# xxayt/MGSV

Hardware: AMD Instinct MI355X
Metric: video-music pairs/s fwd+bwd at B=64 (full training step); sub-objects: retrieval sim-matrix GB/s, eval forward pairs/s (higher is better)
Workload: dtype bf16; 1 GPU; BASELINE.json configs[2]: B=64/GPU, T_v=30, T_a=512, D=512, train mode (dropout on), f32 master weights + Adam, f32 gradient accumulation; global_batch=64, launch=tape

## Files before the change

include/made_hip.h:

```cpp
#ifndef MADE_HIP_H
#define MADE_HIP_H

#include <stdint.h>

#ifdef __cplusplus
extern "C" {
#endif

#define MADE_ABI_VERSION 8

enum MadeDtype { MADE_F32 = 0, MADE_BF16 = 1 };

enum MadeAct {
    MADE_ACT_NONE = 0,
    MADE_ACT_RELU = 1,
    MADE_ACT_GELU = 2,
    MADE_ACT_QUICKGELU = 3,
    MADE_ACT_SIGMOID = 4
};

enum MadeGate {
    MADE_GATE_NONE = 0,
    MADE_GATE_RELU_OUT = 1,
    MADE_GATE_GELU_Z = 2,
// ... 147 lines not shown

int made_splitk_finish(const MadeFinishArgs* args, void* stream);

typedef struct MadeAttnArgs {
    const void* Q; const void* K; const void* V; void* O;
    int32_t dtype; int32_t hd;
    int64_t B, H, Lq, Lk;
    int64_t q_bs, ldq, k_bs, ldk, v_bs, ldv, o_bs, ldo;
    const float* key_mask; const float* q_mask;
    float scale; int32_t _pad;
    const float* q_skip_mask;
    float*      lse;
    MadeDropout drop;
    const int32_t* batch_order;
    uint32_t* keep_bits;
    int64_t ld_bits;
} MadeAttnArgs;

int made_attention(const MadeAttnArgs* args, void* stream);

typedef struct MadeWideAttnArgs {
    const void* Q; const void* K; const void* Kadd; const void* V; void* O;
    const float* key_mask;
    int32_t dtype; int32_t o_dtype;
    int64_t B, NQ1, NQ2, L, D;
    int64_t q_bs, q_s1, q_s2, k_bs, ldk, kadd_bs, ldkadd, v_bs, ldv, o_bs, o_s1, o_s2;
    float scale; int32_t _pad;
    int64_t n_split;
    float*  part_o;
    float*  part_ml;
    MadeDropout drop;
    float*  sum_out;
    float*  lse_out;
} MadeWideAttnArgs;

int made_attention_wide(const MadeWideAttnArgs* args, void* stream);

typedef struct MadeWideAttnBwdArgs {
    const void *Q, *dO, *O, *K, *V;
    const float* key_mask;
    const float *lse, *ssum;
    const float* extra;
    const void* dattc; int64_t ld_dattc; const float* vbias; int64_t hd;
    void *Pd, *dS; int64_t p_bs, ld_p;
    void* dQ; int64_t dq_bs, ld_dq;
    int64_t B, NQ, L, D;
    int64_t q_bs, ld_q, do_bs, ld_do, o_bs, ld_o, k_bs, ldk, v_bs, ldv;
    float scale; int32_t _pad;
    int64_t n_split; float* part_dq;
    MadeDropout drop;
} MadeWideAttnBwdArgs;
int made_attention_wide_bwd(const MadeWideAttnBwdArgs* args, void* stream);

int made_tape_begin(void);
int made_tape_end(uint64_t* handle);
int made_tape_replay(uint64_t handle);
int made_tape_free(uint64_t handle);
int made_tape_interleave(uint64_t handle, int32_t main_weight);
int made_tape_count(uint64_t handle, int64_t* kernels, int64_t* waits, int64_t* others);
int made_tape_replay_range(uint64_t handle, int64_t first, int64_t count);
int made_tape_op(uint64_t handle, int64_t index, int32_t* kind, uint64_t* function, uint64_t* stream, uint32_t* grid3);
int made_stream_wait(void* src_stream, void* dst_stream);
typedef int (*MadeTapeCallback)(void* user);
int made_tape_callback(MadeTapeCallback fn, void* user);
int made_tape_event(int32_t op_kind, int32_t slot, void* stream);
int made_memset_async(void* dst, int32_t value, int64_t nbytes, void* stream);
int made_copy_async(void* dst, const void* src, int64_t nbytes, void* stream);
int made_store_words(void* dst, const uint32_t* words, int32_t n_words, void* stream);


int made_layernorm(const void* x, int32_t x_dtype, int64_t ldx, int64_t x_rows_per_batch, int64_t x_batch_stride,
                   const float* gamma, const float* beta,
                   void* y, int32_t y_dtype, int64_t ldy, int64_t rows, int64_t D, float eps,
                   const float* row_skip , void* stream);

int made_layernorm_add(const void* x, int32_t x_dtype, int64_t ldx, const float* gamma, const float* beta,
                       void* y, int32_t y_dtype, int64_t ldy, const void* add, int32_t add_dtype, int64_t ld_add,
                       void* y2, int64_t ldy2, int64_t rows, int64_t D, float eps, const float* row_skip, void* stream);

int made_pack_music_records(const void* seg, int32_t seg_dtype, int64_t seg_bs, const float* mask, int64_t ld_mask, const float* music, int64_t ld_music,
                            void* out, int32_t pack_dtype, int64_t rec_bytes, int64_t n, int64_t n_pad, int64_t S, int64_t D, void* stream);

int made_cast_mask_rows(const float* x, int64_t ldx, const float* mask, void* y, int32_t y_dtype, int64_t ldy,
                        int64_t rows, int64_t D, void* stream);

int made_masked_mean(const void* x, int32_t x_dtype, int64_t x_bs, int64_t ldx, const float* mask,
                     float* out, int64_t B, int64_t T, int64_t D, void* stream);

int made_l2norm_rows(const void* x, int32_t x_dtype, int64_t ldx, float* y_f32, void* y_alt, int32_t y_alt_dtype,
                     int64_t ldy, int64_t rows, int64_t D, float eps, void* stream);

int made_sine_pe(const float* mask, const float* dim_t, void* out, int32_t out_dtype,
                 int64_t B, int64_t L, int64_t D, void* stream);

int made_masked_softmax(const float* logits, int64_t ld_logits, const float* mask, int64_t ld_mask,
                        void* probs, int32_t out_dtype, int64_t ldp,
                        int64_t M_outer, int64_t R, int64_t S, int64_t S_pad, float scale, void* stream);

typedef struct MadeXpoolFusedArgs {
    const void* Q; int64_t ldq;
    const void* K; const void* U; int64_t k_bs, ldk, u_bs, ldu;
    const float* key_mask;
    const float* ln2_g; const float* ln2_b;
    const void* Wl; int64_t ldw; const float* bl;
    const float* ln3_g; const float* ln3_b;
    const float* vn; int64_t ldvn;
// ... 300 lines not shown
```

mgsv_amd/_lib.py:

```python
from __future__ import annotations

import ctypes as C
import os

_HERE = os.path.dirname(os.path.abspath(__file__))


def variant_env(name: str, default: str = "") -> str:
    if os.environ.get("MADE_DEBUG_VARIANTS", "0") in ("", "0"):
        return default
    return os.environ.get(name, default)


LIB_PATH = os.environ.get("MADE_LIB_PATH") or os.path.join(_HERE, "libmade_hip.so")
ABI_VERSION = 8

F32, BF16 = 0, 1
ACT_NONE, ACT_RELU, ACT_GELU, ACT_QUICKGELU, ACT_SIGMOID = 0, 1, 2, 3, 4
GATE_NONE, GATE_RELU_OUT, GATE_GELU_Z, GATE_QUICKGELU_Z, GATE_SIGMOID_OUT = 0, 1, 2, 3, 4

vp, i64, i32, f32 = C.c_void_p, C.c_int64, C.c_int32, C.c_float


class MadeDropout(C.Structure):
    _fields_ = [("seed", C.c_uint64), ("site", C.c_uint32), ("p", f32), ("seed_device", vp)]


class MadeLinearSeg(C.Structure):
    _fields_ = [("col_begin", i64), ("out", vp), ("out_dtype", i32), ("transposed", i32), ("ldo", i64),
                ("rows_per_batch", i64), ("out_batch_stride", i64), ("out_z_stride", i64),
                ("use_a2", i32), ("_pad", i32)]


class MadeLinearArgs(C.Structure):
    _fields_ = [("A", vp), ("a_dtype", i32), ("w_dtype", i32), ("lda", i64),
                ("A2", vp), ("lda2", i64), ("a2_row_mod", i64),
                ("a2_replace", i32), ("drop_col_div", i32),
                ("a_row_mask", vp),
                ("W", vp), ("ldw", i64),
                ("bias", vp),
                ("M", i64), ("N", i64), ("K", i64),
                ("batch", i64), ("a_z_stride", i64), ("w_z_stride", i64),
                ("act", i32), ("r_dtype", i32),
                ("R", vp), ("ldr", i64), ("r_row_mod", i64),
                ("out_row_mask", vp),
                ("tile_skip_mask", vp),
                ("nseg", i32), ("split_k", i32),
                ("split_ws", vp),
                ("seg", MadeLinearSeg * 4),
                ("G", vp), ("g_dtype", i32), ("gate", i32), ("ldg", i64), ("gate_scale", f32), ("z_dtype", i32),
                ("Zout", vp), ("ldz", i64), ("drop", MadeDropout), ("drop_ld", i64), ("row_index", vp), ("n_rows", vp),
                ("bias_row_scale", vp), ("bias_z_stride", i64)]


class MadeFinishArgs(C.Structure):
    _fields_ = [("ws", vp), ("split_k", i64), ("M", i64), ("N", i64),
                ("bias", vp), ("act", i32), ("r_dtype", i32),
                ("R", vp), ("ldr", i64), ("r_row_mod", i64),
                ("out", vp), ("out_dtype", i32), ("_pad0", i32), ("ldo", i64),
                ("ln1_g", vp), ("ln1_b", vp), ("ln1_out", vp), ("ln1_dtype", i32), ("_pad1", i32), ("ln1_ld", i64),
                ("ln2_g", vp), ("ln2_b", vp), ("ln2_out", vp), ("ln2_dtype", i32), ("_pad2", i32), ("ln2_ld", i64),
                ("eps", f32), ("_pad3", i32)]


class MadeDecStageArgs(C.Structure):
    _fields_ = [("Zin", vp), ("ldz", i64), ("ln_g", vp), ("ln_b", vp),
                ("ln2_g", vp), ("ln2_b", vp), ("x2_out", vp), ("ldx2", i64),
                ("add", vp), ("add_row_mod", i64), ("x_out", vp), ("ldx", i64),
                ("W", vp), ("ldw", i64), ("bias", vp), ("R", vp), ("ldr", i64), ("out", vp), ("ldo", i64),
                ("out_dtype", i32), ("act", i32), ("res_from_x", i32), ("eps", f32),
                ("M", i64), ("N", i64), ("K", i64),
                ("zin_dtype", i32), ("drop_col_div", i32), ("a_out", vp), ("lda_out", i64), ("drop", MadeDropout), ("drop_ld", i64)]


# ... 95 lines not shown

class MadeAdamGroup(C.Structure):
    _fields_ = [("begin", i64), ("end", i64), ("lr", f32), ("max_norm", f32)]


class MadeAdamDeviceState(C.Structure):
    _fields_ = [("step", i64), ("lr", f32 * 4), ("bc1", f32), ("bc2_sqrt", f32)]


class MadeRepackDesc(C.Structure):
    _fields_ = [("src", vp), ("w", vp), ("wt", vp), ("rows", i64), ("cols", i64), ("wt_ld", i64), ("tile_begin", i64),
                ("dtype", i32), ("_pad", i32)]


class MadeFrameDesc(C.Structure):
    _fields_ = [("offset", i64), ("coef", i64), ("H", i32), ("W", i32), ("kh", i32), ("kv", i32)]


class MadeResampleDesc(C.Structure):
    _fields_ = [("offset", i64), ("n", i64), ("taps", i64), ("o", i32), ("m", i32), ("width", i32), ("_pad", i32)]


class MadeAudioSegDesc(C.Structure):
    _fields_ = [("first", i64), ("count", i64)]


SIGNATURES = {
    "made_abi_version": (C.c_int, []),
    "made_set_f32_products": (C.c_int, [C.c_int]),
    "made_get_f32_products": (C.c_int, []),
    "made_last_error": (C.c_char_p, []),
    "made_device_info": (C.c_int, [C.c_char_p, C.c_int, C.POINTER(C.c_int), C.POINTER(C.c_int)]),
    "made_tape_begin": (C.c_int, []),
    "made_tape_end": (C.c_int, [C.POINTER(C.c_uint64)]),
    "made_tape_replay": (C.c_int, [C.c_uint64]),
    "made_tape_free": (C.c_int, [C.c_uint64]),
    "made_tape_interleave": (C.c_int, [C.c_uint64, i32]),
    "made_tape_count": (C.c_int, [C.c_uint64, C.POINTER(i64), C.POINTER(i64), C.POINTER(i64)]),
    "made_tape_replay_range": (C.c_int, [C.c_uint64, i64, i64]),
    "made_tape_op": (C.c_int, [C.c_uint64, i64, C.POINTER(i32), C.POINTER(C.c_uint64), C.POINTER(C.c_uint64), C.POINTER(C.c_uint32)]),
    "made_stream_wait": (C.c_int, [vp, vp]),
    "made_tape_event": (C.c_int, [i32, i32, vp]),
    "made_tape_callback": (C.c_int, [C.CFUNCTYPE(C.c_int, vp), vp]),
    "made_memset_async": (C.c_int, [vp, i32, i64, vp]),
    "made_copy_async": (C.c_int, [vp, vp, i64, vp]),
    "made_store_words": (C.c_int, [vp, vp, i32, vp]),
    "made_linear": (C.c_int, [C.POINTER(MadeLinearArgs), vp]),
    "made_splitk_finish": (C.c_int, [C.POINTER(MadeFinishArgs), vp]),
    "made_dec_stage": (C.c_int, [C.POINTER(MadeDecStageArgs), vp]),
    "made_dec_stage_bwd": (C.c_int, [C.POINTER(MadeDecStageBwdArgs), vp]),
    "made_attention": (C.c_int, [C.POINTER(MadeAttnArgs), vp]),
    "made_attention_wide": (C.c_int, [C.POINTER(MadeWideAttnArgs), vp]),
    "made_attention_wide_bwd": (C.c_int, [C.POINTER(MadeWideAttnBwdArgs), vp]),
    "made_layernorm": (C.c_int, [vp, i32, i64, i64, i64, vp, vp, vp, i32, i64, i64, i64, f32, vp, vp]),
    "made_layernorm_add": (C.c_int, [vp, i32, i64, vp, vp, vp, i32, i64, vp, i32, i64, vp, i64, i64, i64, f32, vp, vp]),
    "made_cast_mask_rows": (C.c_int, [vp, i64, vp, vp, i32, i64, i64, i64, vp]),
    "made_pack_music_records": (C.c_int, [vp, i32, i64, vp, i64, vp, i64, vp, i32, i64, i64, i64, i64, i64, vp]),
    "made_masked_mean": (C.c_int, [vp, i32, i64, i64, vp, vp, i64, i64, i64, vp]),
    "made_l2norm_rows": (C.c_int, [vp, i32, i64, vp, vp, i32, i64, i64, i64, f32, vp]),
    "made_sine_pe": (C.c_int, [vp, vp, vp, i32, i64, i64, i64, vp]),
    "made_masked_softmax": (C.c_int, [vp, i64, vp, i64, vp, i32, i64, i64, i64, i64, i64, f32, vp]),
    "made_xpool_tail": (C.c_int, [vp, i32, i64, vp, vp, vp, i64, vp, vp, i64, i64, i64, i64, f32, vp]),
    "made_clip_loss": (C.c_int, [vp, i64, i64, vp, f32, i32, vp, vp, vp]),
    "made_hungarian_match": (C.c_int, [vp, vp, vp, i64, i64, i64, i64, i32, f32, f32, f32, vp, i32, vp, vp, vp, vp, vp]),
    "made_attention_bwd": (C.c_int, [C.POINTER(MadeAttnBwdArgs), vp]),
    "made_layernorm_bwd": (C.c_int, [vp, i32, i64, i64, i64, vp, vp, i32, i64, vp, i32, i64, vp, i32, i64, vp, i64,
                                     C.POINTER(MadeDropout), i64, vp, vp, i64, i64, f32, vp, vp]),
    "made_layernorm_bwd2": (C.c_int, [vp, vp, i64, vp, vp, i64, vp, i64, vp, i64, vp, i64, vp, i64, C.POINTER(MadeDropout), i64, i32,
                                      vp, vp, vp, vp, i64, i64, f32, vp]),
    "made_pool_bwd": (C.c_int, [vp, vp, vp, vp, i32, i64, i64, vp, i32, i64, i64, vp, i32, i64, i64, i64, i64, i64, f32, vp]),
    "made_l2norm_bwd": (C.c_int, [vp, i32, i64, vp, i64, i64, vp, i64, i32, vp, i32, i64, i64, i64, f32, vp]),
    "made_clip_loss_bwd": (C.c_int, [vp, i64, i64, vp, f32, vp, vp, vp, vp, i32, vp, vp, vp]),
    "made_xpool_tail_bwd": (C.c_int, [vp, i32, i64, vp, vp, vp, i64, vp, i64, vp, i32, i64, vp, C.POINTER(MadeDropout),
                                      vp, vp, vp, i64, vp, i64, f32, i64, i64, i64, f32, vp]),
    "made_softmax_bwd": (C.c_int, [vp, i64, vp, i64, vp, i64, vp, f32, C.POINTER(MadeDropout), vp, vp, vp, i32, i64, i64,
                                   i64, i64, i64, i64, i64, vp]),
    "made_head_bias": (C.c_int, [vp, i32, i64, vp, vp, i64, i64, i64, vp]),
    "made_head_bias_bwd": (C.c_int, [vp, i32, i64, vp, vp, vp, vp, i64, i64, i64, vp]),
    "made_add3": (C.c_int, [vp, i32, vp, i32, vp, i32, vp, i32, i64, i64, vp]),
    "made_colsum": (C.c_int, [vp, i32, i64, i64, i64, vp, vp]),
    "made_posbn_relu_fwd": (C.c_int, [vp, i32, i64, vp, vp, vp, vp, C.c_float, C.c_float, i32, vp, vp, vp, i32, i64, i64, i64, i64, vp]),
    "made_posbn_relu_bwd": (C.c_int, [vp, i32, i64, vp, i32, i64, vp, i32, i64, vp, vp, vp, i32, vp, i32, i64, vp, vp, i64, i64, i64, vp]),
    "made_set_criterion_bwd": (C.c_int, [vp, vp, vp, vp, vp, vp, vp, vp, vp, i64, i64, i64, i64, i64, i32, f32, vp, vp,
                                         vp, vp, i64, i32, vp, vp, vp]),
    "made_adam_step": (C.c_int, [vp, vp, vp, vp, i64, C.POINTER(MadeAdamGroup), i32, f32, f32, f32, i64, f32, vp, vp]),
    "made_adam_step_device": (C.c_int, [vp, vp, vp, vp, i64, C.POINTER(MadeAdamGroup), i32, f32, f32, f32, vp, i32, f32, vp, vp]),
    "made_repack": (C.c_int, [vp, i32, i64, vp]),
    "made_row_groups": (C.c_int, [vp, i64, vp, vp]),
    "made_row_index": (C.c_int, [vp, i64, vp, vp, vp]),
    "made_linear_variant": (C.c_int, [C.POINTER(MadeLinearArgs)]),
    "made_row_affine": (C.c_int, [vp, i32, i64, vp, vp, i64, i32, vp, i32, i64, i64, i64, vp]),
    "made_gate_rows": (C.c_int, [vp, i32, i64, vp, i32, i64, i32, f32, vp, i64, i64, vp, i32, i64, vp, i64, i64, vp]),
    "made_xpool_fused": (C.c_int, [C.POINTER(MadeXpoolFusedArgs), vp]),
    "made_xpool_attention": (C.c_int, [C.POINTER(MadeXpoolAttnArgs), vp]),
    "made_xpool_sims": (C.c_int, [C.POINTER(MadeXpoolSimsArgs), vp]),
    "made_xpool_sims_ws_bytes": (C.c_int64, [i64, i64, i64]),
    "made_xpool_inbatch": (C.c_int, [C.POINTER(MadeXpoolInbatchArgs), vp]),
    "made_xpool_inbatch_ws_bytes": (C.c_int64, [i64, i64]),
    "made_batch_order": (C.c_int, [vp, i64, i64, vp, vp]),
    "made_recall_ranks": (C.c_int, [vp, i64, vp, vp, i64, i64, i64, vp, vp, vp]),
    "made_span_iou": (C.c_int, [vp, vp, vp, vp, i64, i64, i32, f32, vp, vp, vp]),
    "made_gemm_tn": (C.c_int, [C.POINTER(MadeGemmTNArgs), vp]),
    "made_gemm_tn_grouped": (C.c_int, [C.POINTER(MadeGemmTNGroup), vp]),
    "made_gemm_tn_grouped_workspace": (i64, [C.POINTER(MadeGemmTNGroup)]),
    "made_concat_cols": (C.c_int, [vp, i64, vp, i64, vp, i64, vp]),
    "made_pooled_cosine": (C.c_int, [vp, i64, vp, i32, vp, i64, i64, i64, i64, i64, vp]),
# ... 53 lines not shown
```

mgsv_amd/csrc/attention_wide.hip:

```cpp
#include "common.h"

#include <type_traits>

namespace {

constexpr int WQ = 32;
constexpr int WKEY = 32;
constexpr int NTHREADS = 256;

template <typename TC> struct Frag;
template <> struct Frag<float>  { typedef f32x4  type; };
template <> struct Frag<bf16_t> { typedef bf16x8 type; };


template <typename TC, int D, bool DB, int NSL, bool X3 = false>
__global__ __launch_bounds__(NTHREADS) void attention_wide_kernel(const MadeWideAttnArgs a) {
    typedef typename Frag<TC>::type frag_t;
    constexpr int SZ = (int)sizeof(TC);
    constexpr bool IS_BF16 = SZ == 2;
    constexpr int PER16 = 16 / SZ;
    constexpr int DS = D / NSL;
    constexpr int WQB = WQ * (4 / NSL);
    constexpr bool DMA = IS_BF16 && DB;
    constexpr int K_ROW = DMA ? D * SZ : D * SZ + 16;
    constexpr int V_ROW = DMA ? D * SZ : D * SZ + (IS_BF16 ? 64 : 16);
    constexpr int CPR = D * SZ / 16;
    constexpr int NCH = WKEY * CPR / NTHREADS;
    static_assert(WKEY * CPR % NTHREADS == 0, "staging split");
    constexpr int NQF = DS * SZ / 32;
    constexpr int NDT = DS / 32;
    constexpr int KV_STAGE = WKEY * K_ROW + WKEY * V_ROW;
    constexpr int NSTAGE = DB ? 2 : 1;

    extern __shared__ __attribute__((aligned(16))) unsigned char lds[];
    float* lds_s = (float*)(lds + NSTAGE * KV_STAGE);
    float* lds_bias_all = lds_s + 4 * 1024;
    uint32_t* lds_mbits = (uint32_t*)(lds_bias_all + NSTAGE * 32);

    const int tid = threadIdx.x, lane = tid & 63, wave = tid >> 6;
    const int r = lane & 31, hh = lane >> 5;
    const int sl = wave % NSL, qt = wave / NSL;
    const bool batch_fast = gridDim.x == (unsigned)a.B && (a.NQ1 * a.NQ2 + WQB - 1) / WQB != (int64_t)a.B;
    const int64_t b = batch_fast ? blockIdx.x : blockIdx.y;
    const int64_t nq_total = a.NQ1 * a.NQ2;
    const int64_t nq0 = (int64_t)(batch_fast ? blockIdx.y : blockIdx.x) * WQB + qt * WQ;

    const TC* Kg = (const TC*)a.K + b * a.k_bs;
    const TC* Ag = a.Kadd ? (const TC*)a.Kadd + b * a.kadd_bs : nullptr;
    const TC* Vg = (const TC*)a.V + b * a.v_bs;
    const float* maskg = a.key_mask ? a.key_mask + b * a.L : nullptr;

    frag_t qf[NQF];
    int64_t my_q = nq0 + r;
    {
        int64_t q = my_q < nq_total ? my_q : nq_total - 1;
        const TC* qp = (const TC*)a.Q + b * a.q_bs + (q / a.NQ2) * a.q_s1 + (q % a.NQ2) * a.q_s2 + sl * DS;
#pragma unroll
        for (int ks = 0; ks < NQF; ++ks) qf[ks] = *(const frag_t*)(qp + ks * 2 * PER16 + hh * PER16);
    }

    frag_t rk[NCH], rv[NCH];
    int64_t rkey0 = 0;
    auto load_tile = [&](int64_t key0) __attribute__((always_inline)) {
        rkey0 = key0;
#pragma unroll
        for (int i = 0; i < NCH; ++i) {
            int c = tid + i * NTHREADS;
            int row = c / CPR, cc = c % CPR;
            int64_t key = key0 + row;
            const int64_t kcl = key < a.L ? key : a.L - 1;
            rk[i] = *(const frag_t*)(Kg + kcl * a.ldk + cc * PER16);
            rv[i] = *(const frag_t*)(Vg + kcl * a.ldv + cc * PER16);
        }
        if (Ag) {
#pragma unroll
            for (int i = 0; i < NCH; ++i) {
                int c = tid + i * NTHREADS;
                int64_t key = key0 + c / CPR;
                const int64_t kcl = key < a.L ? key : a.L - 1;
                const frag_t av = *(const frag_t*)(Ag + kcl * a.ldkadd + (c % CPR) * PER16);
#pragma unroll
                for (int j = 0; j < PER16; ++j) rk[i][j] = from_f32<TC>(to_f32(rk[i][j]) + to_f32(av[j]));
            }
        }
    };
    auto store_tile = [&](int stage) __attribute__((always_inline)) {
        unsigned char* sk = lds + stage * KV_STAGE;
        unsigned char* sv = sk + WKEY * K_ROW;
        const uint32_t bits = lds_mbits[rkey0 / WKEY];
#pragma unroll
        for (int i = 0; i < NCH; ++i) {
            int c = tid + i * NTHREADS;
            const bool keep = (bits >> (c / CPR)) & 1u;
            *(frag_t*)(sk + (c / CPR) * K_ROW + (c % CPR) * 16) = keep_or_zero(rk[i], keep);
            *(frag_t*)(sv + (c / CPR) * V_ROW + (c % CPR) * 16) = keep_or_zero(rv[i], keep);
        }
        if (tid < WKEY) lds_bias_all[stage * WKEY + tid] = ((bits >> tid) & 1u) ? 0.f : -INFINITY;
    };

    f32x16 o[NDT];
#pragma unroll
    for (int d = 0; d < NDT; ++d)
#pragma unroll
        for (int e = 0; e < 16; ++e) o[d][e] = 0.f;
    float m_run = -INFINITY, l_run = 0.f;
    float sd_run = 0.f;
    const uint32_t drop_thr = made_drop_threshold(a.drop.p);
    const uint64_t drop_seed = a.drop.p > 0.f ? made_drop_seed(a.drop) : 0;
    const float drop_sc = a.drop.p > 0.f ? 1.f / (1.f - a.drop.p) : 1.f;
    const uint64_t drop_base = (uint64_t)(b * nq_total + (my_q < nq_total ? my_q : nq_total - 1)) * (uint64_t)a.L;
    const bool drop_fast = (uint32_t)drop_base <= 0xFFFFFFFFu - (uint32_t)(a.L + 64);
    const uint32_t drop_key = made_rng_key(drop_seed, a.drop.site, (uint32_t)(drop_base >> 32));
    const uint32_t drop_lo = (uint32_t)drop_base;

    int64_t l_eff = a.L;
    int first_valid = 0;
    {
        const int lpad = (int)((a.L + 63) / 64) * 64;
        int last = -1, first = 0x7fffffff;
        for (int j = tid; j < lpad; j += NTHREADS) {
            const bool valid = j < (int)a.L && (maskg == nullptr || maskg[j] != 0.f);
            const unsigned long long bal = __ballot(valid);
            if (lane == 0) { lds_mbits[j / 32] = (uint32_t)bal; lds_mbits[j / 32 + 1] = (uint32_t)(bal >> 32); }
            if (valid) { last = j; first = min(first, j); }
        }
        if (tid == 0) lds_mbits[lpad / 32] = 0u;
        if (maskg) {
#pragma unroll
            for (int o2 = 32; o2 > 0; o2 >>= 1) { last = max(last, __shfl_xor(last, o2)); first = min(first, __shfl_xor(first, o2)); }
            int* red = (int*)lds_s;
            if (lane == 0) { red[wave] = last; red[4 + wave] = first; }
            __syncthreads();
            l_eff = max(max(red[0], red[1]), max(red[2], red[3])) + 1;
            first_valid = min(min(red[4], red[5]), min(red[6], red[7]));
            if (first_valid == 0x7fffffff) first_valid = 0;
        }
        __syncthreads();
    }
    const int64_t nsplit = a.n_split > 1 ? a.n_split : 1;
    const int64_t tiles_all = (l_eff + WKEY - 1) / WKEY;
    const int64_t tiles_per = (tiles_all + nsplit - 1) / nsplit;
    const int64_t tile0 = (int64_t)blockIdx.z * tiles_per;
    const int64_t ntiles = tile0 >= tiles_all ? 0 : (tile0 + tiles_per <= tiles_all ? tiles_per : tiles_all - tile0);
    typedef __attribute__((address_space(3))) void* lds_ptr_t;
    typedef const __attribute__((address_space(1))) void* glb_ptr_t;
    auto issue_tile = [&](int64_t key0, int stage) __attribute__((always_inline)) {
        constexpr int ROWS_PER_PIECE = DMA ? 1024 / (D * SZ) : 1;
        constexpr int NPIECE = WKEY / ROWS_PER_PIECE;
        constexpr int CPRW = D * SZ / 16;
        const uint32_t bits = lds_mbits[key0 / WKEY];
        unsigned char* st = lds + stage * KV_STAGE;
        const unsigned char* Kb = (const unsigned char*)Kg;
        const unsigned char* Vb = (const unsigned char*)Vg;
        const uint32_t ldk_b = (uint32_t)a.ldk * SZ, ldv_b = (uint32_t)a.ldv * SZ;
#pragma unroll
        for (int i = 0; i < NPIECE / 4; ++i) {
            const int jp = wave + 4 * i;
            const int row = ROWS_PER_PIECE == 1 ? jp : 2 * jp + (lane >> 5);
            const uint32_t cl = ROWS_PER_PIECE == 1 ? (uint32_t)lane : (uint32_t)(lane & 31);
            const uint32_t srow = ((bits >> row) & 1u) ? (uint32_t)(key0 + row) : (uint32_t)first_valid;
            const uint32_t ck = cl ^ ((uint32_t)(row & 31) & (uint32_t)(CPRW - 1));
            const uint32_t cu = ((((cl >> 2) ^ (uint32_t)(row & 7)) << 2) | (cl & 3));
            __builtin_amdgcn_global_load_lds((glb_ptr_t)(Kb + (size_t)(srow * ldk_b + ck * 16u)), (lds_ptr_t)(st + jp * 1024), 16, 0, 0);
            __builtin_amdgcn_global_load_lds((glb_ptr_t)(Vb + (size_t)(srow * ldv_b + cu * 16u)), (lds_ptr_t)(st + WKEY * K_ROW + jp * 1024), 16, 0, 0);
        }
    };
    if constexpr (DMA) {
        __builtin_amdgcn_s_waitcnt(0x0070);
        if (ntiles > 0) issue_tile(tile0 * WKEY, 0);
    } else if (NSTAGE == 2 && ntiles > 0) {
        load_tile(tile0 * WKEY);
        store_tile(0);
        __syncthreads();
    }
    for (int64_t tt = 0; tt < ntiles; ++tt) {
        const int64_t t = tile0 + tt;
        const int cur = NSTAGE == 2 ? (int)(tt & 1) : 0;
        uint32_t tbits = 0xffffffffu;
        if constexpr (DMA) {
            asm volatile("s_waitcnt vmcnt(0) lgkmcnt(0)\n\ts_barrier" ::: "memory");
            tbits = lds_mbits[t];
        } else if (NSTAGE == 2) {
            if (tt + 1 < ntiles) load_tile((t + 1) * WKEY);
        } else {
            load_tile(t * WKEY);
            __syncthreads();
            store_tile(0);
            __syncthreads();
        }
        const unsigned char* lds_k = lds + cur * KV_STAGE;
        const unsigned char* lds_v = lds_k + WKEY * K_ROW;
        const float* lds_bias = lds_bias_all + cur * WKEY;

        f32x16 s;
#pragma unroll
        for (int e = 0; e < 16; ++e) s[e] = 0.f;
        if constexpr (X3) {
            static_assert(!X3 || (NQF % 2 == 0 && !DMA), "f32 slices of 16 columns or more");
#pragma unroll
            for (int ks = 0; ks < NQF; ks += 2) {
                const SplitF32x4 k0 = made_split4(*(const f32x4*)(lds_k + r * K_ROW + sl * DS * SZ + ks * 32 + hh * 16));
                const SplitF32x4 k1 = made_split4(*(const f32x4*)(lds_k + r * K_ROW + sl * DS * SZ + (ks + 1) * 32 + hh * 16));
                s = made_mfma_x3_16(k0, k1, made_split4(qf[ks]), made_split4(qf[ks + 1]), s);
            }
        } else {
#pragma unroll
        for (int ks = 0; ks < NQF; ++ks) {
            frag_t kf;
            if constexpr (DMA) kf = *(const frag_t*)(lds_k + r * K_ROW + ((((sl * DS * SZ) / 16 + ks * 2 + hh) ^ r) << 4));
            else kf = *(const frag_t*)(lds_k + r * K_ROW + sl * DS * SZ + ks * 32 + hh * 16);
            if constexpr (IS_BF16) {
                s = __builtin_amdgcn_mfma_f32_32x32x16_bf16(kf, qf[ks], s, 0, 0, 0);
            } else {
#pragma unroll
                for (int e = 0; e < 4; ++e) s = __builtin_amdgcn_mfma_f32_32x32x2f32(kf[e], qf[ks][e], s, 0, 0, 0);
            }
        }
        }
        if constexpr (DMA) {
            if (tt + 1 < ntiles) issue_tile((t + 1) * WKEY, cur ^ 1);
        }
#pragma unroll
        for (int e = 0; e < 16; ++e) lds_s[wave * 1024 + acc_row(e, hh) * 32 + r] = s[e];
        asm volatile("s_waitcnt lgkmcnt(0)\n\ts_barrier" ::: "memory");
        float mx = -INFINITY;
#pragma unroll
        for (int e = 0; e < 16; ++e) {
            const int idx = acc_row(e, hh) * 32 + r;
            float v;
            if constexpr (NSL == 4) v = (lds_s[idx] + lds_s[1024 + idx]) + (lds_s[2048 + idx] + lds_s[3072 + idx]);
            else v = lds_s[qt * 2048 + idx] + lds_s[qt * 2048 + 1024 + idx];
            if constexpr (DMA) v = ((tbits >> acc_row(e, hh)) & 1u) ? v * a.scale : -INFINITY;
            else v = v * a.scale + lds_bias[acc_row(e, hh)];
            s[e] = v;
// ... 54 lines not shown
                    for (int d = 0; d < NDT; ++d) {
                        asm volatile("" : "+v"(lo[d]), "+v"(hi[d]));
                        o[d] = __builtin_amdgcn_mfma_f32_32x32x16_bf16(__builtin_shufflevector(lo[d], hi[d], 0, 1, 2, 3, 4, 5, 6, 7), pf, o[d], 0, 0, 0);
                    }
                } else {
#pragma unroll
                for (int d = 0; d < NDT; ++d) {
                    const int dcol = sl * DS + d * 32 + (g & 1) * 16 + 4 * (i & 3);
                    const unsigned char* vp = lds_v + (kb + (i >> 2)) * V_ROW + dcol * 2;
                    bf16x4 lo = __builtin_amdgcn_ds_read_tr16_b64_v4bf16((__attribute__((address_space(3))) bf16x4*)vp);
                    bf16x4 hi = __builtin_amdgcn_ds_read_tr16_b64_v4bf16((__attribute__((address_space(3))) bf16x4*)(vp + 8 * V_ROW));
                    bf16x8 vf = __builtin_shufflevector(lo, hi, 0, 1, 2, 3, 4, 5, 6, 7);
                    o[d] = __builtin_amdgcn_mfma_f32_32x32x16_bf16(vf, pf, o[d], 0, 0, 0);
                }
                }
            }
        } else if constexpr (X3) {
#pragma unroll
            for (int g4 = 0; g4 < 4; g4 += 2) {
                const SplitF32x4 pb0 = made_split4(f32x4{s[4 * g4], s[4 * g4 + 1], s[4 * g4 + 2], s[4 * g4 + 3]});
                const SplitF32x4 pb1 = made_split4(f32x4{s[4 * g4 + 4], s[4 * g4 + 5], s[4 * g4 + 6], s[4 * g4 + 7]});
#pragma unroll
                for (int d = 0; d < NDT; ++d) {
                    f32x4 v0, v1;
#pragma unroll
                    for (int j = 0; j < 4; ++j) {
                        v0[j] = *(const float*)(lds_v + (8 * g4 + 4 * hh + j) * V_ROW + (sl * DS + d * 32 + r) * 4);
                        v1[j] = *(const float*)(lds_v + (8 * g4 + 8 + 4 * hh + j) * V_ROW + (sl * DS + d * 32 + r) * 4);
                    }
                    o[d] = made_mfma_x3_16(made_split4(v0), made_split4(v1), pb0, pb1, o[d]);
                }
            }
        } else {
#pragma unroll
            for (int e = 0; e < 16; ++e) {
                const int key = acc_row(e, hh);
#pragma unroll
                for (int d = 0; d < NDT; ++d) {
                    float vv = *(const float*)(lds_v + key * V_ROW + (sl * DS + d * 32 + r) * 4);
                    o[d] = __builtin_amdgcn_mfma_f32_32x32x2f32(vv, s[e], o[d], 0, 0, 0);
                }
            }
        }
        if (NSTAGE == 2 && !DMA) {
            if (tt + 1 < ntiles) store_tile(cur ^ 1);
            __syncthreads();
        }
    }

    const float l_tot = l_run + __shfl_xor(l_run, 32);
    const float inv = 1.f / l_tot;
    const float sd_tot = sd_run + __shfl_xor(sd_run, 32);
    const bool live_q = my_q < nq_total;
    if (nsplit == 1 && !live_q) return;
    if (nsplit == 1 && sl == 0 && hh == 0) {
        if (a.sum_out) a.sum_out[b * nq_total + my_q] = a.drop.p > 0.f ? sd_tot * inv : 1.f;
        if (a.lse_out) a.lse_out[b * nq_total + my_q] = m_run + logf(l_tot);
    }
    if (nsplit > 1) {
        const int64_t prow = (b * nsplit + blockIdx.z) * nq_total + (live_q ? my_q : 0);
        if (live_q) {
            float* po = a.part_o + prow * D + sl * DS;
#pragma unroll
            for (int d = 0; d < NDT; ++d)
#pragma unroll
                for (int g4 = 0; g4 < 4; ++g4) {
                    f32x4 pk; pk[0] = o[d][4 * g4]; pk[1] = o[d][4 * g4 + 1]; pk[2] = o[d][4 * g4 + 2]; pk[3] = o[d][4 * g4 + 3];
                    *(f32x4*)(po + d * 32 + 8 * g4 + 4 * hh) = pk;
                }
            if (sl == 0 && hh == 0) {
                a.part_ml[prow * 4] = m_run; a.part_ml[prow * 4 + 1] = l_tot; a.part_ml[prow * 4 + 2] = a.drop.p > 0.f ? sd_tot : l_tot;
            }
        }
        return;
    }
    const int64_t obase = b * a.o_bs + (my_q / a.NQ2) * a.o_s1 + (my_q % a.NQ2) * a.o_s2 + sl * DS;
#pragma unroll
    for (int d = 0; d < NDT; ++d)
#pragma unroll
        for (int g4 = 0; g4 < 4; ++g4) {
            const int64_t off = obase + d * 32 + 8 * g4 + 4 * hh;
            float v0 = o[d][4 * g4] * inv, v1 = o[d][4 * g4 + 1] * inv, v2 = o[d][4 * g4 + 2] * inv, v3 = o[d][4 * g4 + 3] * inv;
            if (a.o_dtype == MADE_F32) {
                f32x4 pk; pk[0] = v0; pk[1] = v1; pk[2] = v2; pk[3] = v3;
                *(f32x4*)((float*)a.O + off) = pk;
            } else {
                bf16x4 pk; pk[0] = (bf16_t)v0; pk[1] = (bf16_t)v1; pk[2] = (bf16_t)v2; pk[3] = (bf16_t)v3;
                *(bf16x4*)((bf16_t*)a.O + off) = pk;
            }
        }
}

__global__ __launch_bounds__(NTHREADS) void attention_wide_combine_kernel(const MadeWideAttnArgs a) {
    const int lane = threadIdx.x & 63;
    const int64_t nq_total = a.NQ1 * a.NQ2;
    const int64_t row = (int64_t)blockIdx.x * (NTHREADS / 64) + (threadIdx.x >> 6);
    if (row >= a.B * nq_total) return;
    const int64_t b = row / nq_total, q = row % nq_total;
    const int D = (int)a.D;
    const int ns = (int)a.n_split;
    float Lsum = 0.f, Dsum = 0.f, Muse = 0.f;
    f32x4 acc[2];
#pragma unroll
    for (int i = 0; i < 2; ++i) { acc[i][0] = acc[i][1] = acc[i][2] = acc[i][3] = 0.f; }
    if (ns <= 4) {
        f32x4 t[4][2];
        float ml[4][3];
#pragma unroll
        for (int sp = 0; sp < 4; ++sp) {
            const int64_t pr = (b * ns + (sp < ns ? sp : ns - 1)) * nq_total + q;
            ml[sp][0] = a.part_ml[pr * 4]; ml[sp][1] = a.part_ml[pr * 4 + 1]; ml[sp][2] = a.part_ml[pr * 4 + 2];
#pragma unroll
            for (int i = 0; i < 2; ++i) {
// ... 37 lines not shown
            }
        }
    }
    const float inv = 1.f / Lsum;
    if (a.sum_out && lane == 0) a.sum_out[b * nq_total + q] = Dsum * inv;
    if (a.lse_out && lane == 0) a.lse_out[b * nq_total + q] = Muse + logf(Lsum);
    const int64_t obase = b * a.o_bs + (q / a.NQ2) * a.o_s1 + (q % a.NQ2) * a.o_s2;
#pragma unroll
    for (int i = 0; i < 2; ++i) {
        int c = (i * 64 + lane) * 4;
        if (c < D) {
            if (a.o_dtype == MADE_F32) {
                f32x4 pk; pk[0] = acc[i][0] * inv; pk[1] = acc[i][1] * inv; pk[2] = acc[i][2] * inv; pk[3] = acc[i][3] * inv;
                *(f32x4*)((float*)a.O + obase + c) = pk;
            } else {
                bf16x4 pk; pk[0] = (bf16_t)(acc[i][0] * inv); pk[1] = (bf16_t)(acc[i][1] * inv);
                pk[2] = (bf16_t)(acc[i][2] * inv); pk[3] = (bf16_t)(acc[i][3] * inv);
                *(bf16x4*)((bf16_t*)a.O + obase + c) = pk;
            }
        }
    }
}

template <typename TC, int D, bool DB, int NSL>
int launch_wide(const MadeWideAttnArgs& a, hipStream_t st) {
    constexpr int SZ = (int)sizeof(TC);
    constexpr bool DMA = SZ == 2 && DB;
    constexpr int K_ROW = DMA ? D * SZ : D * SZ + 16, V_ROW = DMA ? D * SZ : D * SZ + (SZ == 2 ? 64 : 16);
    constexpr int NSTAGE = DB ? 2 : 1;
    constexpr size_t kBase = (size_t)NSTAGE * (WKEY * K_ROW + WKEY * V_ROW) + 4 * 1024 * 4 + NSTAGE * 32 * 4;
    constexpr size_t kCap = kBase + 8192 < 160 * 1024 ? kBase + 8192 : 160 * 1024;
    const size_t lds_bytes = kBase + (size_t)((a.L + 63) / 64 * 2 + 2) * 4;
    if (lds_bytes > kCap) {
        made_set_error("made_attention_wide: L=%lld keys: the mask bit row does not fit in LDS beside the K / V stages", (long long)a.L);
        return MADE_ERR_UNSUPPORTED;
    }
    static bool attr_done = false;
    if (!attr_done) {
        hipError_t e = hipFuncSetAttribute((const void*)attention_wide_kernel<TC, D, DB, NSL>, hipFuncAttributeMaxDynamicSharedMemorySize, (int)kCap);
        if (e == hipSuccess && SZ == 4)
            e = hipFuncSetAttribute((const void*)attention_wide_kernel<TC, D, DB, NSL, SZ == 4>, hipFuncAttributeMaxDynamicSharedMemorySize, (int)kCap);
        if (e != hipSuccess) {
            made_set_error("made_attention_wide: cannot reserve %zu bytes of LDS: %s", kCap, hipGetErrorString(e));
            return MADE_ERR_HIP;
        }
        attr_done = true;
    }
    const int64_t nq = a.NQ1 * a.NQ2;
    const int64_t nsplit = a.n_split > 1 ? a.n_split : 1;
    constexpr int WQB = WQ * (4 / NSL);
    const int64_t qtiles = (nq + WQB - 1) / WQB;
    const bool batch_fast = qtiles > 1 && qtiles <= 8 && qtiles != a.B;
    dim3 grid((unsigned)(batch_fast ? a.B : qtiles), (unsigned)(batch_fast ? qtiles : a.B), (unsigned)nsplit), block(NTHREADS);
    if (SZ == 4 && g_made_f32_products) hipLaunchKernelGGL((attention_wide_kernel<TC, D, DB, NSL, SZ == 4>), grid, block, lds_bytes, st, a);
    else hipLaunchKernelGGL((attention_wide_kernel<TC, D, DB, NSL>), grid, block, lds_bytes, st, a);
    int rc = made_check_launch("made_attention_wide");
    if (rc != MADE_OK || nsplit == 1) return rc;
    const int64_t rows = a.B * nq;
    hipLaunchKernelGGL(attention_wide_combine_kernel, dim3((unsigned)((rows + 3) / 4)), dim3(NTHREADS), 0, st, a);
    return made_check_launch("made_attention_wide(combine)");
}

}

extern "C" int made_attention_wide(const MadeWideAttnArgs* args, void* stream) {
    MADE_REQUIRE(args != nullptr, "made_attention_wide: null args");
    const MadeWideAttnArgs& a = *args;
    MADE_REQUIRE(a.Q && a.K && a.V && a.O, "made_attention_wide: null tensor");
    MADE_REQUIRE(a.B >= 0 && a.NQ1 >= 0 && a.NQ2 > 0 && a.L > 0, "made_attention_wide: bad dims");
    MADE_REQUIRE(a.dtype == MADE_F32 || a.dtype == MADE_BF16, "made_attention_wide: bad dtype %d", a.dtype);
    MADE_REQUIRE(a.o_dtype == MADE_F32 || a.o_dtype == MADE_BF16, "made_attention_wide: bad o_dtype %d", a.o_dtype);
    MADE_UNSUPPORTED(a.D == 128 || a.D == 256 || a.D == 512, "made_attention_wide: D=%lld not in {128, 256, 512}", (long long)a.D);
    MADE_UNSUPPORTED(a.B <= 65535, "made_attention_wide: B too large for the grid");
    const int per16 = a.dtype == MADE_F32 ? 4 : 8;
    MADE_UNSUPPORTED(a.q_bs % per16 == 0 && a.q_s1 % per16 == 0 && a.q_s2 % per16 == 0 && a.k_bs % per16 == 0 && a.ldk % per16 == 0 &&
                     a.v_bs % per16 == 0 && a.ldv % per16 == 0 && a.kadd_bs % per16 == 0 && a.ldkadd % per16 == 0 &&
                     a.o_bs % 4 == 0 && a.o_s1 % 4 == 0 && a.o_s2 % 4 == 0,
                     "made_attention_wide: strides must keep 16-byte alignment");
    MADE_UNSUPPORTED(((uintptr_t)a.Q % 16) == 0 && ((uintptr_t)a.K % 16) == 0 && ((uintptr_t)a.V % 16) == 0 && ((uintptr_t)a.O % 16) == 0 &&
                     ((uintptr_t)a.Kadd % 16) == 0, "made_attention_wide: base pointers must be 16-byte aligned");
    MADE_REQUIRE(a.drop.p >= 0.f && a.drop.p < 1.f, "made_attention_wide: dropout p out of [0,1)");
    if (a.n_split > 1) {
        MADE_REQUIRE(a.part_o != nullptr && a.part_ml != nullptr, "made_attention_wide: n_split > 1 needs part_o / part_ml");
        MADE_UNSUPPORTED(a.n_split <= 64, "made_attention_wide: n_split <= 64");
    }
    if (a.B == 0 || a.NQ1 == 0) return MADE_OK;
    hipStream_t st = (hipStream_t)stream;
    if (a.dtype == MADE_BF16) {
        const int64_t nq = a.NQ1 * a.NQ2;
        const bool few = nq <= 64 && a.Kadd == nullptr;
        const bool pair = nq > 32 && nq <= 64 && a.Kadd == nullptr;
        if (a.D == 128) return launch_wide<bf16_t, 128, false, 4>(a, st);
        if (a.D == 512) {
            if (pair) return launch_wide<bf16_t, 512, true, 2>(a, st);
            return few ? launch_wide<bf16_t, 512, true, 4>(a, st) : launch_wide<bf16_t, 512, false, 4>(a, st);
        }
        if (pair) return launch_wide<bf16_t, 256, true, 2>(a, st);
        return few ? launch_wide<bf16_t, 256, true, 4>(a, st) : launch_wide<bf16_t, 256, false, 4>(a, st);
    }
    if (a.D == 128) return launch_wide<float, 128, false, 4>(a, st);
    return a.D == 512 ? launch_wide<float, 512, false, 4>(a, st) : launch_wide<float, 256, false, 4>(a, st);
}
```

mgsv_amd/csrc/attention_wide_bwd.hip:

```cpp
#include "common.h"

namespace {

constexpr int BK = 32;
constexpr int NT = 256;
constexpr int MAXQ = 8;

typedef __attribute__((address_space(3))) void* lds_ptr_t;
typedef const __attribute__((address_space(1))) void* glb_ptr_t;

template <int D>
__global__ __launch_bounds__(NT) void attention_wide_bwd_kernel(const MadeWideAttnBwdArgs a) {
    constexpr int DS = D / 4;
    constexpr int NQF = DS / 16;
    constexpr int NDT = DS / 32;
    constexpr int ROWB = D * 2;
    constexpr int CPR = ROWB / 16;
    constexpr int STAGE = 2 * BK * ROWB;
    extern __shared__ __attribute__((aligned(16))) unsigned char lds[];
    float* lds_x = (float*)(lds + 2 * STAGE);
    float* lds_q = lds_x + 4 * 2 * BK * MAXQ;
    uint32_t* lds_mbits = (uint32_t*)(lds_q + 8 + 4 * MAXQ);

    const int tid = threadIdx.x, lane = tid & 63, wave = __builtin_amdgcn_readfirstlane(tid >> 6);
    const int r = lane & 31, hh = lane >> 5;
    const int sl = wave;
    const int64_t b = blockIdx.y;
    const int NQ = (int)a.NQ;
    const int rq = (r & 7) < NQ ? (r & 7) : NQ - 1;
    const bool live = r < NQ;

    const bf16_t* Kg = (const bf16_t*)a.K + b * a.k_bs;
    const bf16_t* Vg = (const bf16_t*)a.V + b * a.v_bs;
    const float* maskg = a.key_mask ? a.key_mask + b * a.L : nullptr;

    bf16x8 qf[NQF], dof[NQF];
    float dpart = 0.f;
    {
        const bf16_t* qp = (const bf16_t*)a.Q + b * a.q_bs + (int64_t)rq * a.ld_q + sl * DS + hh * 8;
        const bf16_t* gp = (const bf16_t*)a.dO + b * a.do_bs + (int64_t)rq * a.ld_do + sl * DS + hh * 8;
        const bf16_t* op = (const bf16_t*)a.O + b * a.o_bs + (int64_t)rq * a.ld_o + sl * DS + hh * 8;
        bf16x8 of[NQF];
#pragma unroll
        for (int ks = 0; ks < NQF; ++ks) { qf[ks] = *(const bf16x8*)(qp + ks * 16); dof[ks] = *(const bf16x8*)(gp + ks * 16); of[ks] = *(const bf16x8*)(op + ks * 16); }
#pragma unroll
        for (int ks = 0; ks < NQF; ++ks)
#pragma unroll
            for (int j = 0; j < 8; ++j) dpart += (float)dof[ks][j] * (float)of[ks][j];
    }
    dpart += __shfl_xor(dpart, 32);
    if (r < MAXQ && hh == 0) lds_q[8 + wave * MAXQ + r] = dpart;
    const float lse = a.lse[b * NQ + rq];
    const float ssum = a.ssum ? a.ssum[b * NQ + rq] : 1.f;
    if (wave == 0) {
        float ex = 0.f;
        if (a.extra) {
            ex = a.extra[b * NQ + ((lane >> 3) < NQ ? (lane >> 3) : NQ - 1)];
        } else if (a.dattc) {
            const int h = lane >> 3, per = (int)a.hd / 8;
            const bf16_t* dp_ = (const bf16_t*)a.dattc + b * a.ld_dattc + h * a.hd + (lane & 7) * per;
            const float* bp = a.vbias + h * a.hd + (lane & 7) * per;
            if (h < NQ)
                for (int e = 0; e < per; ++e) ex += (float)dp_[e] * bp[e];
            ex += __shfl_xor(ex, 1); ex += __shfl_xor(ex, 2); ex += __shfl_xor(ex, 4);
        }
        if ((lane & 7) == 0) lds_q[lane >> 3] = ex;
    }

    int64_t l_eff = a.L;
    int first_valid = 0;
    {
        const int lpad = (int)((a.L + 63) / 64) * 64;
        int last = -1, first = 0x7fffffff;
        for (int j = tid; j < lpad; j += NT) {
            const bool valid = j < (int)a.L && (maskg == nullptr || maskg[j] != 0.f);
            const unsigned long long bal = __ballot(valid);
            if (lane == 0) { lds_mbits[j / 32] = (uint32_t)bal; lds_mbits[j / 32 + 1] = (uint32_t)(bal >> 32); }
            if (valid) { last = j; first = min(first, j); }
        }
        if (tid == 0) lds_mbits[lpad / 32] = 0u;
#pragma unroll
        for (int o2 = 32; o2 > 0; o2 >>= 1) { last = max(last, __shfl_xor(last, o2)); first = min(first, __shfl_xor(first, o2)); }
        int* red = (int*)lds_x;
        if (lane == 0) { red[wave] = last; red[4 + wave] = first; }
        __syncthreads();
        l_eff = max(max(red[0], red[1]), max(red[2], red[3])) + 1;
        first_valid = min(min(red[4], red[5]), min(red[6], red[7]));
        if (first_valid == 0x7fffffff) first_valid = 0;
        __syncthreads();
    }
    const float extra = lds_q[rq];
    const float delta = ((lds_q[8 + rq] + lds_q[8 + MAXQ + rq]) + (lds_q[8 + 2 * MAXQ + rq] + lds_q[8 + 3 * MAXQ + rq])) + extra * ssum;

    const int64_t nsplit = a.n_split > 1 ? a.n_split : 1;
    const int64_t tiles_all = (l_eff + BK - 1) / BK;
    const int64_t tiles_L = (a.L + BK - 1) / BK;
    const int64_t tiles_per = (tiles_all + nsplit - 1) / nsplit;
    const int64_t tile0 = (int64_t)blockIdx.z * tiles_per;
    const int64_t ntiles = tile0 >= tiles_all ? 0 : (tile0 + tiles_per <= tiles_all ? tiles_per : tiles_all - tile0);

    auto issue_tile = [&](int64_t key0, int stage) __attribute__((always_inline)) {
        constexpr int ROWS_PER_PIECE = 1024 / ROWB;
        constexpr int NPIECE = BK / ROWS_PER_PIECE;
        const uint32_t bits = lds_mbits[key0 / BK];
        unsigned char* st = lds + stage * STAGE;
        const unsigned char* Kb = (const unsigned char*)Kg;
        const unsigned char* Vb = (const unsigned char*)Vg;
        const uint32_t ldk_b = (uint32_t)a.ldk * 2, ldv_b = (uint32_t)a.ldv * 2;
#pragma unroll
        for (int i = 0; i < NPIECE / 4; ++i) {
            const int jp = wave + 4 * i;
            const int row = ROWS_PER_PIECE == 1 ? jp : 2 * jp + (lane >> 5);
            const uint32_t cl = ROWS_PER_PIECE == 1 ? (uint32_t)lane : (uint32_t)(lane & 31);
            const uint32_t srow = ((bits >> row) & 1u) ? (uint32_t)(key0 + row) : (uint32_t)first_valid;
            const uint32_t c_row = cl ^ ((uint32_t)(row & 31) & (uint32_t)(CPR - 1));
            const uint32_t c_tr = ((((cl >> 2) ^ (uint32_t)(row & 7)) << 2) | (cl & 3));
            __builtin_amdgcn_global_load_lds((glb_ptr_t)(Kb + (size_t)(srow * ldk_b + c_tr * 16u)), (lds_ptr_t)(st + jp * 1024), 16, 0, 0);
            __builtin_amdgcn_global_load_lds((glb_ptr_t)(Vb + (size_t)(srow * ldv_b + c_row * 16u)), (lds_ptr_t)(st + BK * ROWB + jp * 1024), 16, 0, 0);
        }
    };

    f32x16 o[NDT];
#pragma unroll
    for (int d = 0; d < NDT; ++d)
#pragma unroll
        for (int e = 0; e < 16; ++e) o[d][e] = 0.f;
    const uint32_t drop_thr = made_drop_threshold(a.drop.p);
    const uint64_t drop_seed = a.drop.p > 0.f ? made_drop_seed(a.drop) : 0;
    const float drop_sc = a.drop.p > 0.f ? 1.f / (1.f - a.drop.p) : 1.f;
    const uint64_t drop_base = (uint64_t)(b * NQ + rq) * (uint64_t)a.L;
    const bool drop_fast = (uint32_t)drop_base <= 0xFFFFFFFFu - (uint32_t)(a.L + 64);
    const uint32_t drop_key = made_rng_key(drop_seed, a.drop.site, (uint32_t)(drop_base >> 32));
    const uint32_t drop_lo = (uint32_t)drop_base;
    bf16_t* out_row = (wave == 0 ? (bf16_t*)a.Pd : (bf16_t*)a.dS) + b * a.p_bs + (int64_t)rq * a.ld_p;

    __builtin_amdgcn_s_waitcnt(0x0070);
    if (ntiles > 0) issue_tile(tile0 * BK, 0);
    for (int64_t tt = 0; tt < ntiles; ++tt) {
        const int64_t t = tile0 + tt;
        const int cur = (int)(tt & 1);
        asm volatile("s_waitcnt vmcnt(0) lgkmcnt(0)\n\ts_barrier" ::: "memory");
        const uint32_t tbits = lds_mbits[t];
        const unsigned char* lds_k = lds + cur * STAGE;
        const unsigned char* lds_v = lds_k + BK * ROWB;

        f32x16 s, dp;
#pragma unroll
        for (int e = 0; e < 16; ++e) { s[e] = 0.f; dp[e] = 0.f; }
#pragma unroll
        for (int ks = 0; ks < NQF; ++ks) {
            const int c = (sl * DS * 2) / 16 + ks * 2 + hh;
            const bf16x8 kf = *(const bf16x8*)(lds_k + r * ROWB + ((((c >> 2) ^ (r & 7)) << 6) | ((c & 3) << 4)));
            const bf16x8 vf = *(const bf16x8*)(lds_v + r * ROWB + (((c ^ r) & (CPR - 1)) << 4));
            s = __builtin_amdgcn_mfma_f32_32x32x16_bf16(kf, qf[ks], s, 0, 0, 0);
            dp = __builtin_amdgcn_mfma_f32_32x32x16_bf16(vf, dof[ks], dp, 0, 0, 0);
        }
        if (tt + 1 < ntiles) issue_tile((t + 1) * BK, cur ^ 1);
        if (r < MAXQ) {
#pragma unroll
            for (int e = 0; e < 16; ++e) {
                lds_x[((wave * 2 + 0) * BK + acc_row(e, hh)) * MAXQ + r] = s[e];
                lds_x[((wave * 2 + 1) * BK + acc_row(e, hh)) * MAXQ + r] = dp[e];
            }
        }
        asm volatile("s_waitcnt lgkmcnt(0)\n\ts_barrier" ::: "memory");
        float pd[16];
#pragma unroll
        for (int e = 0; e < 16; ++e) {
            const int kr = acc_row(e, hh);
            const float* xs = lds_x + kr * MAXQ + (r & 7);
            const float S = (xs[0] + xs[2 * BK * MAXQ]) + (xs[4 * BK * MAXQ] + xs[6 * BK * MAXQ]);
            const float dP = (xs[BK * MAXQ] + xs[3 * BK * MAXQ]) + (xs[5 * BK * MAXQ] + xs[7 * BK * MAXQ]);
            const bool valid = (tbits >> kr) & 1u;
            const float p = valid ? __expf(S * a.scale - lse) : 0.f;
            bool kp = true;
            if (a.drop.p > 0.f) {
                const uint32_t kidx = (uint32_t)(t * BK + kr);
                const uint32_t hsh = drop_fast ? made_rng_fmix32((drop_lo + kidx) ^ drop_key) : made_rng_mix(drop_seed, a.drop.site, drop_base + (uint64_t)kidx);
                kp = (hsh >> 8) >= drop_thr;
            }
            pd[e] = kp ? p * drop_sc : 0.f;
            const float dpd = valid ? dP + extra : 0.f;
            const float dpu = kp ? dpd * drop_sc : 0.f;
            s[e] = p * (dpu - delta) * a.scale;
        }
        if (wave < 2 && live) {
#pragma unroll
            for (int g4 = 0; g4 < 4; ++g4) {
                const int64_t key0 = t * BK + 8 * g4 + 4 * hh;
                if (key0 < a.ld_p) {
                    bf16x4 pk;
#pragma unroll
                    for (int j = 0; j < 4; ++j) pk[j] = (bf16_t)(wave == 0 ? pd[4 * g4 + j] : s[4 * g4 + j]);
                    *(bf16x4*)(out_row + key0) = pk;
                }
            }
        }
        {
            const int g = lane >> 4, i = lane & 15;
#pragma unroll
            for (int s2 = 0; s2 < 2; ++s2) {
                bf16x8 pf;
#pragma unroll
                for (int j = 0; j < 8; ++j) pf[j] = (bf16_t)s[8 * s2 + j];
                const int kb = 16 * s2 + 4 * (g >> 1);
                const int row = kb + (i >> 2);
                const uint32_t vb = (uint32_t)(uintptr_t)(__attribute__((address_space(3))) unsigned char*)lds_k + row * ROWB + (g & 1) * 32 + (i & 3) * 8;
                bf16x4 lo[NDT], hi[NDT];
#pragma unroll
                for (int d = 0; d < NDT; ++d) {
                    const uint32_t va = vb + ((((sl * DS) / 32 + d) ^ (row & 7)) << 6);
                    asm volatile("ds_read_b64_tr_b16 %0, %1" : "=v"(lo[d]) : "v"(va));
                    asm volatile("ds_read_b64_tr_b16 %0, %1 offset:%2" : "=v"(hi[d]) : "v"(va), "n"(8 * ROWB));
                }
#pragma unroll
                for (int d = 0; d < NDT; ++d) asm volatile("" : "+v"(lo[d]), "+v"(hi[d]));
                asm volatile("s_waitcnt lgkmcnt(0)" ::: "memory");
#pragma unroll
                for (int d = 0; d < NDT; ++d) {
                    asm volatile("" : "+v"(lo[d]), "+v"(hi[d]));
                    o[d] = __builtin_amdgcn_mfma_f32_32x32x16_bf16(__builtin_shufflevector(lo[d], hi[d], 0, 1, 2, 3, 4, 5, 6, 7), pf, o[d], 0, 0, 0);
                }
            }
        }
    }
    if (wave < 2 && live) {
        for (int64_t tz = tiles_all + blockIdx.z; tz < tiles_L; tz += nsplit) {
#pragma unroll
            for (int g4 = 0; g4 < 4; ++g4) {
                const int64_t key0 = tz * BK + 8 * g4 + 4 * hh;
                if (key0 < a.ld_p) {
                    bf16x4 z4; z4[0] = z4[1] = z4[2] = z4[3] = (bf16_t)0.f;
                    *(bf16x4*)(out_row + key0) = z4;
                }
            }
        }
    }

    if (nsplit == 1) {
        if (live) {
            bf16_t* dq = (bf16_t*)a.dQ + b * a.dq_bs + (int64_t)r * a.ld_dq + sl * DS;
#pragma unroll
            for (int d = 0; d < NDT; ++d)
#pragma unroll
                for (int g4 = 0; g4 < 4; ++g4) {
                    bf16x4 pk;
#pragma unroll
                    for (int j = 0; j < 4; ++j) pk[j] = (bf16_t)o[d][4 * g4 + j];
                    *(bf16x4*)(dq + d * 32 + 8 * g4 + 4 * hh) = pk;
                }
        }
        return;
    }
    if (live) {
        float* po = a.part_dq + ((b * nsplit + blockIdx.z) * NQ + r) * D + sl * DS;
#pragma unroll
        for (int d = 0; d < NDT; ++d)
#pragma unroll
            for (int g4 = 0; g4 < 4; ++g4) {
                f32x4 pk; pk[0] = o[d][4 * g4]; pk[1] = o[d][4 * g4 + 1]; pk[2] = o[d][4 * g4 + 2]; pk[3] = o[d][4 * g4 + 3];
                *(f32x4*)(po + d * 32 + 8 * g4 + 4 * hh) = pk;
            }
    }
}

__global__ __launch_bounds__(NT) void wide_bwd_merge_kernel(const MadeWideAttnBwdArgs a) {
    const int lane = threadIdx.x & 63;
    const int64_t row = (int64_t)blockIdx.x * 4 + (threadIdx.x >> 6);
    if (row >= a.B * a.NQ) return;
    const int64_t b = row / a.NQ, q = row % a.NQ;
    const int D = (int)a.D;
    const int per = D / 64;
    float acc[8];
#pragma unroll
    for (int j = 0; j < 8; ++j) acc[j] = 0.f;
    for (int64_t sp = 0; sp < a.n_split; ++sp) {
        const float* pp = a.part_dq + ((b * a.n_split + sp) * a.NQ + q) * D + lane * per;
        const f32x4 t0 = *(const f32x4*)pp;
        acc[0] += t0[0]; acc[1] += t0[1]; acc[2] += t0[2]; acc[3] += t0[3];
        if (per == 8) {
            const f32x4 t1 = *(const f32x4*)(pp + 4);
            acc[4] += t1[0]; acc[5] += t1[1]; acc[6] += t1[2]; acc[7] += t1[3];
        }
    }
    bf16_t* dq = (bf16_t*)a.dQ + b * a.dq_bs + q * a.ld_dq + lane * per;
    bf16x4 p0; p0[0] = (bf16_t)acc[0]; p0[1] = (bf16_t)acc[1]; p0[2] = (bf16_t)acc[2]; p0[3] = (bf16_t)acc[3];
    *(bf16x4*)dq = p0;
    if (per == 8) {
        bf16x4 p1; p1[0] = (bf16_t)acc[4]; p1[1] = (bf16_t)acc[5]; p1[2] = (bf16_t)acc[6]; p1[3] = (bf16_t)acc[7];
        *(bf16x4*)(dq + 4) = p1;
    }
}

template <int D>
int launch_wide_bwd(const MadeWideAttnBwdArgs& a, hipStream_t st) {
    constexpr size_t kBase = (size_t)2 * 2 * BK * D * 2 + (size_t)(4 * 2 * BK * MAXQ + 8 + 4 * MAXQ) * 4;
    const size_t lds_bytes = kBase + (size_t)((a.L + 63) / 64 * 2 + 2) * 4;
    if (lds_bytes > 160 * 1024) {
        made_set_error("made_attention_wide_bwd: L=%lld keys: the mask bit row does not fit in LDS beside the K / V stages", (long long)a.L);
        return MADE_ERR_UNSUPPORTED;
    }
    static bool attr_done = false;
    if (!attr_done) {
        hipError_t e = hipFuncSetAttribute((const void*)attention_wide_bwd_kernel<D>, hipFuncAttributeMaxDynamicSharedMemorySize, 160 * 1024);
        if (e != hipSuccess) {
            made_set_error("made_attention_wide_bwd: cannot reserve LDS: %s", hipGetErrorString(e));
            return MADE_ERR_HIP;
        }
        attr_done = true;
    }
    const int64_t nsplit = a.n_split > 1 ? a.n_split : 1;
    hipLaunchKernelGGL((attention_wide_bwd_kernel<D>), dim3(1, (unsigned)a.B, (unsigned)nsplit), dim3(NT), lds_bytes, st, a);
    int rc = made_check_launch("made_attention_wide_bwd");
    if (rc != MADE_OK || nsplit == 1) return rc;
    hipLaunchKernelGGL(wide_bwd_merge_kernel, dim3((unsigned)((a.B * a.NQ + 3) / 4)), dim3(NT), 0, st, a);
    return made_check_launch("made_attention_wide_bwd(merge)");
}

}

extern "C" int made_attention_wide_bwd(const MadeWideAttnBwdArgs* args, void* stream) {
    MADE_REQUIRE(args != nullptr, "made_attention_wide_bwd: null args");
    const MadeWideAttnBwdArgs& a = *args;
    MADE_REQUIRE(a.Q && a.dO && a.O && a.K && a.V && a.lse && a.Pd && a.dS && a.dQ, "made_attention_wide_bwd: null tensor");
    MADE_REQUIRE(a.B >= 0 && a.NQ > 0 && a.L > 0, "made_attention_wide_bwd: bad dims");
    MADE_UNSUPPORTED(a.NQ <= MAXQ, "made_attention_wide_bwd: NQ=%lld query rows per sample (at most %d: one moment query)", (long long)a.NQ, MAXQ);
    MADE_UNSUPPORTED(a.D == 256 || a.D == 512, "made_attention_wide_bwd: D=%lld not in {256, 512}", (long long)a.D);
    MADE_UNSUPPORTED(a.B <= 65535, "made_attention_wide_bwd: B too large for the grid");
    MADE_UNSUPPORTED(a.q_bs % 8 == 0 && a.ld_q % 8 == 0 && a.do_bs % 8 == 0 && a.ld_do % 8 == 0 && a.o_bs % 8 == 0 && a.ld_o % 8 == 0 &&
                     a.k_bs % 8 == 0 && a.ldk % 8 == 0 && a.v_bs % 8 == 0 && a.ldv % 8 == 0 && a.p_bs % 4 == 0 && a.ld_p % 4 == 0 &&
                     a.dq_bs % 4 == 0 && a.ld_dq % 4 == 0, "made_attention_wide_bwd: strides must keep the rows aligned (16 bytes in, 8 bytes out)");
    MADE_UNSUPPORTED(((uintptr_t)a.Q % 16) == 0 && ((uintptr_t)a.dO % 16) == 0 && ((uintptr_t)a.O % 16) == 0 && ((uintptr_t)a.K % 16) == 0 &&
                     ((uintptr_t)a.V % 16) == 0 && ((uintptr_t)a.Pd % 8) == 0 && ((uintptr_t)a.dS % 8) == 0 && ((uintptr_t)a.dQ % 8) == 0,
                     "made_attention_wide_bwd: base pointers must be aligned");
    MADE_REQUIRE(a.ld_p >= a.L, "made_attention_wide_bwd: ld_p < L");
    MADE_REQUIRE(a.drop.p >= 0.f && a.drop.p < 1.f, "made_attention_wide_bwd: dropout p out of [0,1)");
    if (a.dattc && !a.extra) {
        MADE_REQUIRE(a.vbias != nullptr && a.hd > 0 && a.hd % 8 == 0, "made_attention_wide_bwd: dattc needs vbias and hd (a multiple of 8)");
        MADE_UNSUPPORTED(a.hd * a.NQ == a.D, "made_attention_wide_bwd: dattc needs the one-query layout NQ * hd == D (NQ=%lld hd=%lld D=%lld); pass `extra` otherwise",
                         (long long)a.NQ, (long long)a.hd, (long long)a.D);
    }
    if (a.n_split > 1) {
        MADE_REQUIRE(a.part_dq != nullptr, "made_attention_wide_bwd: n_split > 1 needs part_dq");
        MADE_UNSUPPORTED(a.n_split <= 64, "made_attention_wide_bwd: n_split <= 64");
    }
    if (a.B == 0) return MADE_OK;
    hipStream_t st = (hipStream_t)stream;
    return a.D == 512 ? launch_wide_bwd<512>(a, st) : launch_wide_bwd<256>(a, st);
}
```

mgsv_amd/ops.py:

```python
from __future__ import annotations

import ctypes as C
import math
from dataclasses import dataclass
from typing import Optional, Sequence

import torch

from . import _lib, tape as _tape
from ._lib import (ACT_GELU, ACT_NONE, ACT_QUICKGELU, ACT_RELU, ACT_SIGMOID, BF16, F32,
                   MadeAttnArgs, MadeDecStageArgs, MadeFinishArgs, MadeLinearArgs, MadeLinearSeg, MadeWideAttnArgs, check, lib)

Tensor = torch.Tensor


def dt_of(t: Tensor) -> int:
    if t.dtype == torch.float32:
        return F32
    if t.dtype == torch.bfloat16:
        return BF16
    raise TypeError(f"unsupported dtype {t.dtype}")


def torch_dtype(code: int):
    return torch.float32 if code == F32 else torch.bfloat16


def _p(t: Optional[Tensor]):
    if t is None:
        return None
    if not t.is_cuda:
        raise _lib.MadeError("libmade_hip ops need GPU tensors (no CPU fallback)")
    if _tape._recording is not None:
        _tape._recording._keep.append(t)
    return t.data_ptr()


def _stream():
    return torch.cuda.current_stream().cuda_stream


def _f32(t: Optional[Tensor], name: str) -> Optional[Tensor]:
    if t is not None and (t.dtype != torch.float32 or not t.is_contiguous()):
        raise TypeError(f"{name} must be a contiguous float32 tensor")
    return t


def set_drop(d, drop) -> None:
    seed, site, p = drop
    if isinstance(seed, Tensor):
        assert seed.dtype == torch.int64 and seed.numel() == 1 and seed.is_cuda
        d.seed, d.seed_device = 0, seed.data_ptr()
    else:
        d.seed, d.seed_device = int(seed) & 0xFFFFFFFFFFFFFFFF, None
    d.site, d.p = int(site) & 0xFFFFFFFF, float(p)


def round_up(x: int, m: int) -> int:
# ... 283 lines not shown
    assert Q.dim() == 3 and K.dim() == 3 and V.dim() == 3 and O.dim() == 3
    assert Q.stride(2) == 1 and K.stride(2) == 1 and V.stride(2) == 1 and O.stride(2) == 1
    assert Q.dtype == K.dtype == V.dtype == O.dtype
    B, Lq, D = Q.shape
    hd = D // H
    a = MadeAttnArgs()
    a.Q, a.K, a.V, a.O = _p(Q), _p(K), _p(V), _p(O)
    a.dtype, a.hd = dt_of(Q), hd
    a.B, a.H, a.Lq, a.Lk = B, H, Lq, (K.shape[1] if Lk is None else Lk)
    a.q_bs, a.ldq = Q.stride(0), Q.stride(1)
    a.k_bs, a.ldk = K.stride(0), K.stride(1)
    a.v_bs, a.ldv = V.stride(0), V.stride(1)
    a.o_bs, a.ldo = O.stride(0), O.stride(1)
    a.key_mask = _p(_f32(key_mask, "key_mask"))
    a.q_mask = _p(_f32(q_mask, "q_mask"))
    a.q_skip_mask = _p(_f32(q_skip_mask, "q_skip_mask"))
    a.scale = (1.0 / math.sqrt(hd)) if scale is None else scale
    if order is not None:
        assert order.dtype == torch.int32 and order.numel() == B and order.is_contiguous()
        a.batch_order = _p(order)
    if lse is not None:
        assert lse.dtype == torch.float32 and lse.is_contiguous() and lse.numel() == B * H * Lq
        a.lse = _p(lse)
    if drop is not None and drop[2] > 0.0:
        set_drop(a.drop, drop)
        if keep_bits is not None:
            assert keep_bits.dtype == torch.int32 and keep_bits.dim() == 2 and keep_bits.is_contiguous()
            assert keep_bits.shape[0] >= B * H * ((a.Lk + 31) // 32) and keep_bits.shape[1] >= Lq
            a.keep_bits, a.ld_bits = _p(keep_bits), keep_bits.shape[1]
    esz = 4 if a.dtype == F32 else 2
    flops = 4.0 * B * H * Lq * a.Lk * hd
    nbytes = esz * B * D * (2 * Lq + 2 * a.Lk)
    _timed("attention_" + ("f32" if a.dtype == F32 else "bf16"), flops, nbytes,
           lambda: check(lib().made_attention(C.byref(a), _stream()), "made_attention"),
           ("attn", key_mask, q_skip_mask) if (key_mask is not None and key_mask.dim() == 2) else f"B={B} H={H} hd={hd} Lq={Lq} Lk={a.Lk}")
    return O


def attention_bits_shape(B: int, H: int, Lq: int, Lk: int):
    return (B * H * ((Lk + 31) // 32), 32 * ((Lq + 31) // 32))


def attention_bits_decode(bits: Tensor, B: int, H: int, Lq: int, Lk: int) -> Tensor:
    nkt, ldq = (Lk + 31) // 32, bits.shape[1]
    w = bits[:B * H * nkt].view(B, H, nkt, ldq)
    q = torch.arange(Lq, device=bits.device)
    ql = q & 31
    slot = (q & ~31) + 2 * ((ql & 3) + 4 * (ql >> 3)) + ((ql >> 2) & 1)
    w = w[:, :, :, slot]
    b = (w[..., None] >> torch.arange(32, device=bits.device, dtype=torch.int32)) & 1
    return b.permute(0, 1, 3, 2, 4).reshape(B, H, Lq, nkt * 32)[..., :Lk].bool()


def attention_wide(Q: Tensor, K: Tensor, V: Tensor, O: Tensor, *, scale: float, Kadd: Optional[Tensor] = None,
                   key_mask: Optional[Tensor] = None, shared_q: bool = False, n_split: int = 1,
                   part_o: Optional[Tensor] = None, part_ml: Optional[Tensor] = None, drop=None,
                   sum_out: Optional[Tensor] = None, lse_out: Optional[Tensor] = None) -> Tensor:
    assert Q.dim() == 4 and O.dim() == 4 and K.dim() == 3 and V.dim() == 3
    assert Q.stride(3) == 1 and O.stride(3) == 1 and K.stride(2) == 1 and V.stride(2) == 1
    assert Q.dtype == K.dtype == V.dtype
    B, L, D = K.shape
    a = MadeWideAttnArgs()
    a.Q, a.K, a.V, a.O = _p(Q), _p(K), _p(V), _p(O)
    a.key_mask = _p(_f32(key_mask, "key_mask"))
    a.dtype, a.o_dtype = dt_of(Q), dt_of(O)
    a.B, a.NQ1, a.NQ2, a.L, a.D = B, O.shape[1], O.shape[2], L, D
    a.q_bs, a.q_s1, a.q_s2 = (0 if shared_q else Q.stride(0)), Q.stride(1), Q.stride(2)
    a.k_bs, a.ldk = K.stride(0), K.stride(1)
    a.v_bs, a.ldv = V.stride(0), V.stride(1)
    if Kadd is not None:
        assert Kadd.dim() == 3 and Kadd.stride(2) == 1 and Kadd.dtype == K.dtype
        a.Kadd, a.kadd_bs, a.ldkadd = _p(Kadd), Kadd.stride(0), Kadd.stride(1)
    a.o_bs, a.o_s1, a.o_s2 = O.stride(0), O.stride(1), O.stride(2)
    a.scale = scale
    nq = a.NQ1 * a.NQ2
    if n_split > 1:
        if part_o is None:
            part_o = torch.empty(B * n_split * nq * D, device=Q.device, dtype=torch.float32)
            part_ml = torch.empty(B * n_split * nq * 4, device=Q.device, dtype=torch.float32)
        assert part_o.numel() >= B * n_split * nq * D and part_ml.numel() >= B * n_split * nq * 4
        a.n_split, a.part_o, a.part_ml = n_split, _p(_f32(part_o, "part_o")), _p(_f32(part_ml, "part_ml"))
    if drop is not None and drop[2] > 0.0:
        set_drop(a.drop, drop)
    if lse_out is not None:
        assert lse_out.dtype == torch.float32 and lse_out.is_contiguous() and lse_out.numel() >= B * nq
        a.lse_out = _p(lse_out)
    if sum_out is not None:
        assert sum_out.dtype == torch.float32 and sum_out.is_contiguous() and sum_out.numel() >= B * nq
        a.sum_out = _p(sum_out)
    esz = 4 if a.dtype == F32 else 2
    _timed("attention_wide_" + ("f32" if a.dtype == F32 else "bf16"), 4.0 * B * nq * L * D,
           esz * B * (2 * L * D + 2 * nq * D),
           lambda: check(lib().made_attention_wide(C.byref(a), _stream()), "made_attention_wide"),
           f"B={B} NQ={nq} L={L} D={D} kadd={int(Kadd is not None)}")
    return O


def layernorm(x: Tensor, gamma: Tensor, beta: Tensor, out: Optional[Tensor] = None, eps: float = 1e-5,
              out_dtype: Optional[torch.dtype] = None, row_skip: Optional[Tensor] = None) -> Tensor:
    assert x.dim() in (2, 3) and x.stride(-1) == 1
    if x.dim() == 3:
        rows, D = x.shape[0] * x.shape[1], x.shape[2]
        ldx, rpb, xbs = x.stride(1), x.shape[1], x.stride(0)
    else:
        rows, D = x.shape
        ldx, rpb, xbs = x.stride(0), 0, 0
    if out is None:
        out = torch.empty((rows, D), device=x.device, dtype=out_dtype or x.dtype)
    assert out.dim() == 2 and out.stride(1) == 1 and out.shape[0] >= rows
    check(lib().made_layernorm(_p(x), dt_of(x), ldx, rpb, xbs, _p(_f32(gamma, "gamma")), _p(_f32(beta, "beta")),
                               _p(out), dt_of(out), out.stride(0), rows, D, eps, _p(_f32(row_skip, "row_skip")), _stream()),
          "made_layernorm")
    return out


def layernorm_add(x: Tensor, gamma: Optional[Tensor], beta: Optional[Tensor], add: Tensor, out: Optional[Tensor], out2: Tensor,
                  eps: float = 1e-5, row_skip: Optional[Tensor] = None) -> Tensor:
    assert x.dim() == 2 and add.dim() == 2 and out2.dim() == 2 and x.stride(1) == 1 and add.stride(1) == 1 and out2.stride(1) == 1
    rows, D = x.shape
    ydt = dt_of(out2)
    if out is not None:
        assert out.dtype == out2.dtype and out.stride(1) == 1
    check(lib().made_layernorm_add(_p(x), dt_of(x), x.stride(0), _p(_f32(gamma, "gamma")), _p(_f32(beta, "beta")),
                                   _p(out), ydt, out.stride(0) if out is not None else 0, _p(add), dt_of(add), add.stride(0),
                                   _p(out2), out2.stride(0), rows, D, eps, _p(_f32(row_skip, "row_skip")), _stream()), "made_layernorm_add")
    return out2


def cast_mask_rows(x: Tensor, mask: Optional[Tensor], out: Tensor) -> Tensor:
    assert x.dim() == 2 and out.dim() == 2 and x.dtype == torch.float32 and x.stride(1) == 1 and out.stride(1) == 1
    check(lib().made_cast_mask_rows(_p(x), x.stride(0), _p(_f32(mask, "mask")), _p(out), dt_of(out), out.stride(0),
                                    x.shape[0], x.shape[1], _stream()), "made_cast_mask_rows")
    return out


def pack_music_records(seg: Tensor, mask: Tensor, music: Tensor, out: Tensor, pack_dtype: torch.dtype) -> Tensor:
    n, S, D = seg.shape
    assert seg.stride(2) == 1 and seg.stride(1) == D and out.dtype == torch.uint8 and out.dim() == 2 and out.is_contiguous() and out.shape[0] >= n
    mask, music = _f32(mask.contiguous(), "mask"), _f32(music.contiguous(), "music")
    check(lib().made_pack_music_records(_p(seg), dt_of(seg), seg.stride(0) if n > 0 else S * D, _p(mask), S, _p(music), D, _p(out),
                                        F32 if pack_dtype == torch.float32 else BF16, out.shape[1], n, out.shape[0], S, D, _stream()),
          "made_pack_music_records")
    return out


def row_affine(x: Tensor, scale: Tensor, shift: Tensor, act: int = ACT_NONE, out: Optional[Tensor] = None) -> Tensor:
    assert x.dim() == 2 and x.stride(1) == 1 and scale.numel() == shift.numel()
# ... 339 lines not shown
```

mgsv_amd/ops_train.py:

```python
from __future__ import annotations

import ctypes as C
from typing import Optional, Tuple

import torch

from . import _lib
from ._lib import BF16, F32, MadeAttnBwdArgs, MadeDropout, MadeGemmTNArgs, MadeGemmTNGroup, check, lib
from .ops import _f32, _p, _stream, _timed, dt_of, set_drop

Tensor = torch.Tensor
Pair = Tuple[int, int]


_TN_SLAB_US = 1.3


def _tn_splits(tiles: int, nslab: int, gathered: bool, cap: int) -> int:
    if _lib.variant_env("MADE_TN_SPLIT_MODEL", "1") == "0":
        sp = max(8, (512 // max(tiles, 1)) // 8 * 8) if cap == 64 and tiles < 64 else max(1, 2048 // max(tiles, 1))
        while (nslab + sp - 1) // sp > 64:
            sp += 8
        return min(sp, max(1, nslab))
    live = max(1, (nslab * 9) // 16 if gathered else nslab)
# ... 242 lines not shown
    B, T, D = out.shape
    def bs(t): return (t.stride(0), t.stride(1)) if t is not None else (0, 0)
    check(lib().made_pool_bwd(_p(_f32(mean, "mean")), _p(_f32(dvec, "dvec")), _p(_f32(mask, "mask")),
                              _p(in1), _dt(in1), *bs(in1), _p(in2), _dt(in2), *bs(in2),
                              _p(out), dt_of(out), *bs(out), B, T, D, eps, _stream()), "made_pool_bwd")
    return out


def l2norm_bwd(x: Tensor, dy: Tensor, dx: Optional[Tensor] = None, *, accumulate: bool = False, dx_alt: Optional[Tensor] = None,
               eps: float = 1e-12, dy_rows_per: int = 1) -> None:
    rows, D = x.shape
    check(lib().made_l2norm_bwd(_p(x), dt_of(x), x.stride(0), _p(_f32(dy, "dy")), dy.stride(0), dy_rows_per,
                                _p(dx), dx.stride(0) if dx is not None else 0, int(accumulate),
                                _p(dx_alt), _dt(dx_alt), dx_alt.stride(0) if dx_alt is not None else 0,
                                rows, D, eps, _stream()), "made_l2norm_bwd")


def clip_loss_bwd(sims: Tensor, logit_scale: Tensor, weight: float, upstream: Optional[Tensor], lse_ws: Tensor, dsims: Tensor,
                  dsims_t: Optional[Tensor], d_logit_scale: Optional[Tensor], accumulate: bool = False,
                  row_exclude: Optional[Tensor] = None) -> None:
    n = sims.shape[0]
    assert lse_ws.numel() >= 2 * n and dsims.is_contiguous()
    assert row_exclude is None or (row_exclude.shape == sims.shape and row_exclude.is_contiguous())
    check(lib().made_clip_loss_bwd(_p(_f32(sims, "sims")), sims.stride(0), n, _p(logit_scale), float(weight), _p(upstream),
                                   _p(lse_ws), _p(dsims), _p(dsims_t), int(accumulate), _p(d_logit_scale),
                                   _p(_f32(row_exclude, "row_exclude")), _stream()),
          "made_clip_loss_bwd")


def xpool_tail_bwd(y: Tensor, gamma: Tensor, beta: Tensor, video: Tensor, dsims: Tensor, dy: Tensor, Nm: int, Nv: int, *,
                   dy_drop: Optional[Tensor] = None, drop=None, dgamma: Optional[Tensor] = None, dbeta: Optional[Tensor] = None,
                   dvideo: Optional[Tensor] = None, dpool: Optional[Tensor] = None, dpool_scale: float = 1.0, eps: float = 1e-5) -> None:
    D = y.shape[1]
    check(lib().made_xpool_tail_bwd(_p(y), dt_of(y), y.stride(0), _p(gamma), _p(beta), _p(_f32(video, "video")), video.stride(0),
                                    _p(_f32(dsims, "dsims")), dsims.stride(0), _p(dy), dt_of(dy), dy.stride(0), _p(dy_drop),
                                    _drop_ptr(drop), _p(dgamma), _p(dbeta), _p(dvideo), dvideo.stride(0) if dvideo is not None else 0,
                                    _p(_f32(dpool, "dpool")), dpool.stride(0) if dpool is not None else 0, float(dpool_scale),
                                    Nm, Nv, D, eps, _stream()), "made_xpool_tail_bwd")


def softmax_bwd(S: Tensor, dP: Tensor, mask: Optional[Tensor], rows_per_mask: int, scale: float, Pd: Tensor, dS: Tensor,
                dSt: Optional[Tensor], rows_per_batch: int, L: int, *, extra: Optional[Tensor] = None, drop=None,
                ldo: Optional[int] = None, ldt: int = 0, out_batch_stride: int = 0, t_batch_stride: int = 0) -> None:
    rows = S.shape[0]
    check(lib().made_softmax_bwd(_p(_f32(S, "S")), S.stride(0), _p(dP), dP.stride(0), _p(mask), rows_per_mask,
                                 _p(extra), float(scale), _drop_ptr(drop), _p(Pd), _p(dS), _p(dSt), dt_of(Pd),
                                 Pd.stride(-2) if ldo is None else ldo, ldt, out_batch_stride, t_batch_stride,
                                 rows, rows_per_batch, L, _stream()), "made_softmax_bwd")


def attention_wide_bwd(Q: Tensor, dO: Tensor, O: Tensor, K: Tensor, V: Tensor, lse: Tensor, Pd: Tensor, dS: Tensor, dQ: Tensor, *, scale: float,
                       key_mask: Optional[Tensor] = None, ssum: Optional[Tensor] = None, extra: Optional[Tensor] = None,
                       dattc: Optional[Tensor] = None, vbias: Optional[Tensor] = None, hd: int = 0, drop=None, n_split: int = 1,
                       part_dq: Optional[Tensor] = None) -> Tensor:
    assert Q.dim() == 3 and dO.shape == Q.shape and O.shape == Q.shape and dQ.shape == Q.shape and K.dim() == 3 and V.shape == K.shape
    B, NQ, D = Q.shape
    L = K.shape[1]
    for t in (Q, dO, O, K, V, Pd, dS, dQ):
        assert t.dtype == torch.bfloat16 and t.stride(-1) == 1
    assert Pd.dim() == 3 and dS.dim() == 3 and Pd.stride() == dS.stride() and Pd.shape[0] == B and Pd.shape[1] == NQ
    a = _lib.MadeWideAttnBwdArgs()
    a.Q, a.dO, a.O, a.K, a.V = _p(Q), _p(dO), _p(O), _p(K), _p(V)
    a.key_mask, a.lse, a.ssum, a.extra = _p(_f32(key_mask, "key_mask")), _p(_f32(lse, "lse")), _p(_f32(ssum, "ssum")), _p(_f32(extra, "extra"))
    if dattc is not None:
        assert dattc.dim() == 2 and dattc.dtype == torch.bfloat16 and dattc.stride(1) == 1 and vbias is not None
        a.dattc, a.ld_dattc, a.vbias, a.hd = _p(dattc), dattc.stride(0), _p(_f32(vbias, "vbias")), hd
    a.Pd, a.dS, a.p_bs, a.ld_p = _p(Pd), _p(dS), Pd.stride(0), Pd.stride(1)
    a.dQ, a.dq_bs, a.ld_dq = _p(dQ), dQ.stride(0), dQ.stride(1)
    a.B, a.NQ, a.L, a.D = B, NQ, L, D
    a.q_bs, a.ld_q, a.do_bs, a.ld_do, a.o_bs, a.ld_o = Q.stride(0), Q.stride(1), dO.stride(0), dO.stride(1), O.stride(0), O.stride(1)
    a.k_bs, a.ldk, a.v_bs, a.ldv = K.stride(0), K.stride(1), V.stride(0), V.stride(1)
    a.scale = float(scale)
    if n_split > 1:
        assert part_dq is not None and part_dq.dtype == torch.float32 and part_dq.numel() >= B * n_split * NQ * D
        a.n_split, a.part_dq = n_split, _p(part_dq)
    if drop is not None and drop[2] > 0.0:
        set_drop(a.drop, drop)
    _timed("made_attention_wide_bwd", 6.0 * B * NQ * L * D, 2.0 * B * (2 * L * D + 4 * NQ * D + 2 * NQ * L),
                lambda: check(lib().made_attention_wide_bwd(C.byref(a), _stream()), "made_attention_wide_bwd"), f"B={B} NQ={NQ} L={L} D={D}")
    return dQ


def head_bias(x: Tensor, s: Tensor, bias: Tensor, H: int) -> None:
    rows, D = x.shape
    check(lib().made_head_bias(_p(x), dt_of(x), x.stride(0), _p(_f32(s, "s")), _p(bias), rows, H, D // H, _stream()), "made_head_bias")


def head_bias_bwd(dy: Tensor, s: Tensor, bias: Tensor, dbias: Tensor, ds: Tensor, H: int) -> None:
    rows, D = dy.shape
    check(lib().made_head_bias_bwd(_p(dy), dt_of(dy), dy.stride(0), _p(_f32(s, "s")), _p(bias), _p(dbias), _p(ds), rows, H, D // H,
                                   _stream()), "made_head_bias_bwd")


def add3(out: Tensor, a: Tensor, b: Optional[Tensor] = None, c: Optional[Tensor] = None, b_mod: int = 0) -> Tensor:
    for t in (out, a, b, c):
        assert t is None or t.is_contiguous()
    check(lib().made_add3(_p(out), dt_of(out), _p(a), dt_of(a), _p(b), _dt(b), _p(c), _dt(c), out.numel(), b_mod, _stream()), "made_add3")
    return out


def gate_rows(x: Tensor, out: Tensor, *, G: Optional[Tensor] = None, gate: int = 0, scale: float = 1.0, drop=None, drop_ld: int = 0,
              drop_col_div: int = 1, row_skip: Optional[Tensor] = None) -> Tensor:
    rows, cols = x.shape
    assert x.stride(1) == 1 and out.stride(1) == 1 and out.shape == x.shape and (G is None or (G.shape == x.shape and G.stride(1) == 1))
    check(lib().made_gate_rows(_p(x), dt_of(x), x.stride(0), _p(G), _dt(G), G.stride(0) if G is not None else 0, gate, scale,
                               _drop_ptr(drop), drop_ld, drop_col_div, _p(out), dt_of(out), out.stride(0), _p(_f32(row_skip, "row_skip")), rows, cols,
                               _stream()), "made_gate_rows")
    return out


def colsum(x: Tensor, out: Tensor) -> None:
    rows, cols = x.shape
    check(lib().made_colsum(_p(x), dt_of(x), x.stride(0), rows, cols, _p(_f32(out, "out")), _stream()), "made_colsum")


def posbn_relu(x: Tensor, weight: Tensor, bias: Tensor, running_mean: Optional[Tensor], running_var: Optional[Tensor], momentum: float,
               batch_stats: bool, save_mean: Tensor, save_rstd: Tensor, out: Tensor, eps: float = 1e-5) -> Tensor:
    B, T, F = x.shape
    assert x.is_contiguous() and out.is_contiguous() and out.shape == x.shape
    check(lib().made_posbn_relu_fwd(_p(x), dt_of(x), F, _p(_f32(weight, "weight")), _p(_f32(bias, "bias")), _p(_f32(running_mean, "running_mean")),
                                    _p(_f32(running_var, "running_var")), float(momentum), float(eps), int(bool(batch_stats)),
                                    _p(_f32(save_mean, "save_mean")), _p(_f32(save_rstd, "save_rstd")), _p(out), dt_of(out), F, B, T, F, _stream()),
          "made_posbn_relu_fwd")
    return out


def posbn_relu_bwd(x: Tensor, y: Tensor, dy: Tensor, weight: Tensor, save_mean: Tensor, save_rstd: Tensor, batch_stats: bool, dx: Tensor,
                   dweight: Optional[Tensor], dbias: Optional[Tensor]) -> Tensor:
    B, T, F = x.shape
    for t in (x, y, dy, dx):
        assert t.is_contiguous() and tuple(t.shape) == (B, T, F)
    check(lib().made_posbn_relu_bwd(_p(x), dt_of(x), F, _p(y), dt_of(y), F, _p(dy), dt_of(dy), F, _p(_f32(weight, "weight")),
# ... 18 lines not shown
```

mgsv_amd/trainer.py:

```python
from __future__ import annotations

import math
import os
from typing import Dict, List, Optional, Tuple

import numpy as np
import torch

from . import _lib, dropout as dr, ops, ops_train as tr, tape as _tape
from .config import MadeConfig
from .engine import MadeEngine
from .ops import Seg, round_up

Tensor = torch.Tensor
XA = "video_guided_to_music_pooling_cross_transformer"


HEAD_PAD = 64


class MadeTrainer(MadeEngine):
    def __init__(self, cfg: MadeConfig, state_dict: Dict[str, object], device="cuda:0", dtype: str = "f32"):
        if dtype == "f32x3":
            raise ValueError('dtype "f32x3" (split-bf16 products) is an inference mode: it meets the forward\'s 1e-4 gate, its gradients do not meet '
                             'the f32 training path\'s (measured up to 3e-2 relative per tensor); train in "f32" or "bf16"')
        super().__init__(cfg, state_dict, device, dtype)
        self._check_train_supported()
        self._init_master(state_dict)
        self.repack()
        self._tws: Dict[tuple, Dict[str, Tensor]] = {}
        self.generation = 0
        self.seed = 0
        self.training_dropout = True
        self._bits = dtype == "bf16" and _lib.variant_env("MADE_ATTN_BITS", "1") != "0"

    def _check_train_supported(self):
        c = self.cfg
        bad = []
        if "concat" not in c.mml_fusion and "CA" not in c.mml_fusion:
            bad.append(f"mml_fusion={c.mml_fusion}")
        if c.moment_query_type not in ("video", "music", "zero", "random", "xpool"):
            bad.append(f"moment_query_type={c.moment_query_type}")
        if c.moment_query_type == "xpool" and "music" not in c.vmr_fusion:
            bad.append("moment_query_type=xpool without the music-pooling tower (the reference fails there too)")
        if c.vmr_fusion not in ("XA-music", "XA-video", "XA-video-music", "XA-music-video"):
            bad.append(f"vmr_fusion={c.vmr_fusion}")
        if c.vmr_loss == "dual_single_feature_fuse" and "music" not in c.vmr_fusion:
            bad.append("vmr_loss=dual_single_feature_fuse without the music-pooling tower (the reference fails there too)")
        if c.agg_module != "mlp" and c.with_cls_token and (c.video_transformer_depth < 1 or c.audio_transformer_depth < 1):
            bad.append("with_cls_token without a temporal block")
        if "detr" not in c.mml_localization and "regression" not in c.mml_localization:
            bad.append(f"mml_localization={c.mml_localization}")
        if c.audio_short_cut and c.contrastive_align_loss and c.contrastive_hdim != c.D:
            bad.append("audio_short_cut with contrastive_dim != D (the reference's own add would not broadcast)")
        if c.D not in (128, 256, 512):
            bad.append(f"dim_input={c.D} (the kernels are built for 128, 256 and 512; 128 trains through the chain of separate launches)")
        if bad:
            raise NotImplementedError("MadeTrainer (HIP training path) does not cover yet: " + "; ".join(bad))

    def _towers(self) -> List[Tuple[str, str]]:
        t = []
        if "music" in self.cfg.vmr_fusion:
            t.append(("xa", XA))
        if "video" in self.cfg.vmr_fusion:
            t.append(("xav", "music_guided_to_video_pooling_cross_transformer"))
# ... 346 lines not shown
        rows = B * L
        Lp = round_up(L, 8)
        Sp = round_up(Ta, 8)
        HQ = H * Q
        ws.update(
            xv1=E(B, D), xq=E(B, D), xs1=E(B * Ta, D), xk=E(B * Ta, D), xu=E(B * Ta, D), xo=E(B * B, D), xa2=E(B * B, D),
            xa3=E(B * B, D), xy=E(B * B, D), xg1=E(B * B, D), xg2=E(B * B, D), xg3=E(B * B, D),
            xS=E(B * B, Sp, dtype=f32), xdP=E(B * B, Sp, dtype=f32), xP=E(B * B, Sp), xdS=E(B * B, Sp), xdSt=E(B, Ta, B),
            xdkv=E(B * Ta, 2 * D), xds1=E(B * Ta, D), xdseg=E(B * Ta, D), xdq32=E(B, D, dtype=f32), xdq=E(B, D), xdv1=E(B, D),
            vn=E(B, D, dtype=f32), mn=E(B, D, dtype=f32), dvn=E(B, D, dtype=f32), dmn=E(B, D, dtype=f32),
            sims_vp_t=E(B, B, dtype=f32), dsims_st=E(B, B, dtype=f32),
            xpooled=E(B * B, D, dtype=f32), xpool_q=E(B, D, dtype=f32), dxpool_q=E(B, D, dtype=f32),
            ones_bb=torch.ones(B, B, device=self.device, dtype=f32),
            dsims_s=E(B, B, dtype=f32), dsims_d=E(B, B, dtype=f32), dsims_dt=E(B, B, dtype=f32), clip_ws=E(2 * B, dtype=f32),
            sims_both=E(B, B, dtype=f32), sd_ws=E(16 * B * B, dtype=f32),
            dclip=E(2 * B * D + B * max(c.contrastive_hdim, 1), dtype=f32),
            e_delta=E(B * H * L, dtype=f32), eg1=E(rows, D), eg2=E(rows, D), eg2b=E(rows, D), eg3=E(rows, D), eg3b=E(rows, D), eg3c=E(rows, D),
            egqkv=E(rows, 3 * D), egffn=E(rows, Fd),
            eg2b_2=E(rows, D), eg3_2=E(rows, D), egqkv_2=E(rows, 3 * D), egffn_2=E(rows, Fd),
            dfus=E(rows, D),
            s_raw=E(B * HQ, dtype=f32), dds_raw=E(B * HQ, dtype=f32), gq_raw=E(B, HQ, D),
            d_tq0=E(B * Q, D), GQ=Z(B, 2, nd, HQ, D), PdS=Z(B, 2, nd, HQ, Lp), dS_S=E(nd, B * HQ, Lp, dtype=f32), dS_dP=E(B * HQ, Lp, dtype=f32),
            dSt=E(B, L, HQ), d_ds=E(B * Q, H, dtype=f32), d_delta=E(B * H * Q, dtype=f32),
            dg1=E(B * Q, D), dg2=E(B * Q, D), dg3=E(B * Q, D), dg4=E(B * Q, D), dgqkv=E(B * Q, 3 * D), dgffn=E(B * Q, Fd),
            dgq=E(B, HQ, D), dtgt=E(B * Q, D), dhs=E(nd * B * Q, D), dgN=E(nd * B * Q, D),
            dchain=E(nd, 6, B * Q, D),
            h1=E(nd * B * Q, D), h2=E(nd * B * Q, D), hg1=E(nd * B * Q, D), hg2=E(nd * B * Q, D),
            dlogsp=Z(2, nd * B * Q, HEAD_PAD, dtype=f32), dlogsp_c=Z(2, nd * B * Q, HEAD_PAD),
        )
        ws["dlog"], ws["dsp"], ws["dlog_c"], ws["dsp_c"] = ws["dlogsp"][0], ws["dlogsp"][1], ws["dlogsp_c"][0], ws["dlogsp_c"][1]
        ws["dvideo"], ws["dmusic"] = ws["dclip"][:B * D].view(B, D), ws["dclip"][B * D:2 * B * D].view(B, D)
        if "video" in c.vmr_fusion:
            Svp = round_up(Tv, 8)
            ws.update(
                yv1=E(B, D), yq=E(B, D), ys1=E(B * Tv, D), yk=E(B * Tv, D), yu=E(B * Tv, D), yo=E(B * B, D), ya2=E(B * B, D),
                ya3=E(B * B, D), yy=E(B * B, D), yg1=E(B * B, D), yg2=E(B * B, D), yg3=E(B * B, D),
                yS=E(B * B, Svp, dtype=f32), ydP=E(B * B, Svp, dtype=f32), yP=E(B * B, Svp), ydS=E(B * B, Svp), ydSt=E(B, Tv, B),
                ydkv=E(B * Tv, 2 * D), yds1=E(B * Tv, D), ydseg=E(B * Tv, D), ydq32=E(B, D, dtype=f32), ydq=E(B, D), ydv1=E(B, D),
                dframe_sum=E(B * Tv, D))
        for l in range(ne):
            ws.update({f"e.{l}.src": E(rows, D), f"e.{l}.srcpos": E(rows, D), f"e.{l}.qkv": E(rows, 3 * D), f"e.{l}.att": E(rows, D),
                       f"e.{l}.lse": E(B * H * L, dtype=f32), f"e.{l}.kbits": E(*ops.attention_bits_shape(B, H, L, L), dtype=torch.int32), f"e.{l}.x": E(rows, D), f"e.{l}.s1": E(rows, D), f"e.{l}.h": E(rows, Fd),
                       f"e.{l}.x2": E(rows, D)})
        ws.update(mem=E(rows, D), mempos=E(rows, D))
        if not concat:
            inner, ra, rv = c.ca_heads * c.ca_dim_head, B * Ta, B * Tv
            ws.update(c_nx=E(ra, D), c_nc=E(rv, D), c_q=E(ra, inner), c_kv=E(rv, 2 * inner), c_att=E(ra, inner), c_lse=E(B * c.ca_heads * Ta, dtype=f32),
                      c_ax=E(ra, D), c_nf=E(ra, D), c_z1=E(ra, c.ca_ffn_dim), c_h=E(ra, c.ca_ffn_dim), c_y=E(ra, D),
                      c_g1=E(ra, D), c_g2=E(ra, D), c_g3=E(ra, D), c_gf=E(ra, c.ca_ffn_dim), c_gq=E(ra, inner), c_gkv=E(rv, 2 * inner),
                      c_gatt=E(ra, inner), c_delta=E(B * c.ca_heads * Ta, dtype=f32), c_dseg=E(ra, D), c_dframe=E(rv, D), c_gnc=E(rv, D))
        i32 = torch.int32
        ws.update(rows_v=(E(B * Tv, dtype=i32), E(1, dtype=i32)), rows_a=(E(B * Ta, dtype=i32), E(1, dtype=i32)), rows_f=(E(rows, dtype=i32), E(1, dtype=i32)),
                  order_v=E(B, dtype=i32), order_a=E(B, dtype=i32), order_f=E(B, dtype=i32))
        BQ = B * Q
        stacks = dict(tgt=E(nd + 1, BQ, D), tq=E(nd + 1, BQ, D), qkv=E(nd, BQ, 3 * D), att=E(nd, BQ, D), t_a=E(nd, BQ, D), t1=E(nd, BQ, D),
                      t1q=E(nd, BQ, D), qc=E(nd, BQ, D), pooled=E(nd, BQ, H * D), attc=E(nd, BQ, D), t_b=E(nd, BQ, D), t2=E(nd, BQ, D),
                      h=E(nd, BQ, Fd), t_c=E(nd, BQ, D),
                      **({"n1": E(nd, BQ, D)} if c.detr_pre_norm else {}),
                      g_ffn=E(nd, BQ, D), g_z=E(nd, BQ, Fd), g_ca=E(nd, BQ, D), g_attc=E(nd, BQ, D), g_q=E(nd, B, HQ, D), g_qc=E(nd, BQ, D),
                      g_sa=E(nd, BQ, D), g_qkv=E(nd, BQ, 3 * D), dt1q=E(nd, BQ, D))
        ws["dstack"] = stacks
        ws["s_stack"] = E(nd, BQ, H, dtype=f32)
        ws["ca_lse"] = E(nd, B * HQ, dtype=f32)
        for l in range(nd):
            ws.update({f"d.{l}.{k}": v[l] for k, v in stacks.items() if not k.startswith("g_")})
            ws.update({f"d.{l}.lse": E(B * H * Q, dtype=f32), f"d.{l}.s": ws["s_stack"][l], f"d.{l}.t3": stacks["tgt"][l + 1]})
        if c.contrastive_align_loss:
            Dc = c.contrastive_hdim
            if c.audio_short_cut:
                ws.update(pq_n0=E(nd * B * Q, Dc, dtype=f32), pq_s1=E(nd * B * Q, Dc, dtype=f32), pq_s2=E(nd * B * Q, Dc, dtype=f32),
                          dpq_s=E(nd * B * Q, Dc, dtype=f32), dpq_s2=E(nd * B * Q, Dc, dtype=f32))
            ws.update(dpq=E(nd * B * Q, Dc, dtype=f32), dvid_sum=ws["dclip"][2 * B * D:2 * B * D + B * Dc].view(B, Dc), dpq_raw=E(nd * B * Q, Dc), dpv_raw=E(B * Tv, Dc),
                      dframe_x=E(B * Tv, D))
        self._tws[key] = ws
        return ws

    @torch.no_grad()
    def same_music_exclusion(self, music_ids) -> Optional[Tensor]:
        c = self.cfg
        if music_ids is None or c.vmr_loss != "dual_single_loss_fuse":
            return None
        ids = list(music_ids)
        code = {}
        idx = torch.tensor([code.setdefault(str(i), len(code)) for i in ids])
        ex = (idx[:, None] == idx[None, :]).float()
        ex.fill_diagonal_(0.0)
        return ex.to(self.device)

    def forward_train(self, frame_feats: Tensor, segment_feats: Tensor, frame_masks: Tensor, segment_masks: Tensor,
                      spans_target: Tensor, seed: int = 0, music_ids=None, v_duration: Optional[Tensor] = None) -> Dict[str, Tensor]:
        c, P = self.cfg, self.P
        self._set_products()
        if c.predict_center == 1 and v_duration is None:
            raise ValueError("predict_center=1 needs v_duration (reference model/model_Uni.py:280-282)")
        self.seed = int(seed)
        B, Tv, _ = frame_feats.shape
        Ta = segment_feats.shape[1]
        concat = "concat" in c.mml_fusion
        D, L, Q, nd, H = c.D, (Tv + Ta if concat else Ta), c.num_moment_queries, c.detr_dec_layers, c.detr_nheads
        ws, tw = self._buffers(B, Tv, Ta), self._train_buffers(B, Tv, Ta)
        fm, sm = frame_masks.contiguous(), segment_masks.contiguous()
        pd = float(c.detr_dropout)
        self._shape = (B, Tv, Ta)
        self._inputs = (frame_feats.contiguous(), segment_feats.contiguous(), fm, sm, spans_target.contiguous())

        fus, fus_mask = ws["fus"], ws["fus_mask"]
        self._groups = {}
        cur, side = torch.cuda.current_stream(), self._side_stream()
        side.wait_stream(cur)
        self._rows = {sm.data_ptr(): ops.row_index(sm, out=tw["rows_a"])}
        self._order = {sm.data_ptr(): ops.batch_order(sm, out=tw["order_a"])}
        with torch.cuda.stream(side):
            ops.concat_cols(fm if concat else None, sm, fus_mask)
            self._rows[fm.data_ptr()] = ops.row_index(fm, out=tw["rows_v"])
            self._order[fm.data_ptr()] = ops.batch_order(fm, out=tw["order_v"])
            self._rows[fus_mask.data_ptr()] = ops.row_index(fus_mask, out=tw["rows_f"])
            self._order[fus_mask.data_ptr()] = ops.batch_order(fus_mask, out=tw["order_f"])
            pos = ops.sine_pe(fus_mask, P["dim_t"], out=ws["pos"])
            self._encode_train(self._inputs[0], fm, "video", ws, tw, 0)
        self._encode_train(self._inputs[1], sm, "audio", ws, tw, Tv)
        cur.wait_stream(side)
        rows_f = self._rows[fus_mask.data_ptr()]
        if concat:
            frame, seg = fus[:, :Tv], fus[:, Tv:]
        else:
            frame, seg = ws["frame_buf"], ws["seg_buf"]
            self._ca_fusion_train(ws, tw, frame, seg, fm, sm, B, Tv, Ta)
        self._views = (frame, seg)
        video, music = ws["video"], ws["music"]
        out: Dict[str, Tensor] = dict(video_feats=video, music_feats=music, frame_feats=frame, segment_feats=seg)

        qp = P["query_embed"]
        hd = D // H
        ca_scale = 1.0 / math.sqrt(hd)
        GQ = tw.get("GQ")
        regression = "regression" in c.mml_localization

        def dec_fill_tgt() -> None:
            tgt = tw["d.0.tgt"]
            if c.moment_query_type in ("video", "music", "xpool"):
                if c.moment_query_type == "xpool":
                    cur.wait_stream(side)
                src_vec = video if c.moment_query_type == "video" else (music if c.moment_query_type == "music" else tw["xpool_q"])
                if Q == 1:
                    tr.add3(tgt, src_vec)
                else:
                    tgt.view(B, Q, D).copy_(src_vec[:, None, :].expand(B, Q, D))
            else:
                _tape.zero_(tgt)
            if Q > 1 and not c.detr_pre_norm:
                tr.add3(tw["d.0.tq"], tgt, qp, b_mod=Q * D)

        stage = self._dec_stage_chain()

        def dec_query_side(l: int) -> None:
            p, d = f"detr_transformer.decoder.layers.{l}", f"d.{l}"
            tgt, tq = tw[d + ".tgt"], tw[d + ".tq"]
            qkv = tw[d + ".qkv"]
            Win, bin_ = P[p + ".ca.in.w"], P[p + ".ca.in.b"]
            Wt = P[p + ".ca.in.wt"]
            if c.detr_pre_norm:
                n1 = tw[d + ".n1"]
                qp_rows = qp.expand(B * Q, D) if Q == 1 else qp.repeat(B, 1)
                if Q == 1:
                    Wsa, bsa = P[p + ".sa.in.w"], P[p + ".sa.in.b"]
                    ops.layernorm(tgt, P[p + ".ln1.g"], P[p + ".ln1.b"], out=n1)
                    ops.linear(n1, Wsa[2 * D:], bsa[2 * D:], out=tw[d + ".att"], drop=self._drop(f"dec.{l}" + ".sa_attn", pd), drop_ld=H, drop_col_div=hd)
                else:
                    ops.layernorm_add(tgt, P[p + ".ln1.g"], P[p + ".ln1.b"], qp_rows, n1, tq)
                    ops.linear(n1, P[p + ".sa.in.w"], P[p + ".sa.in.b"], A2=tq, a2_replace=True,
# ... 76 lines not shown
            fskip = qskip = rows_f = None
        pos2 = pos.view(rows, D)
        src = fus.view(rows, D)
        if c.detr_enc_layers == 0:
            ops.layernorm_add(src, None, None, pos2, tw["mem"], tw["mempos"], row_skip=fskip)
        else:
            srcpos = tw["e.0.srcpos"]
            if not c.detr_pre_norm:
                ops.layernorm_add(src, None, None, pos2, None, srcpos, row_skip=fskip)
        pre = bool(c.detr_pre_norm)
        xin = src
        for l in range(c.detr_enc_layers):
            p, e = f"detr_transformer.encoder.layers.{l}", f"e.{l}"
            if pre:
                src, srcpos = tw[e + ".src"], tw[e + ".srcpos"]
                ops.layernorm_add(xin, P[p + ".ln1.g"], P[p + ".ln1.b"], pos2, src, srcpos, row_skip=fskip)
            elif l > 0:
                src, srcpos = tw[e + ".src"], tw[e + ".srcpos"]
            qkv = tw[e + ".qkv"]
            ops.linear(src, P[p + ".in.w"], P[p + ".in.b"], A2=srcpos, a2_replace=True, rows=rows_f,
                       segs=[Seg(out=qkv, col_begin=0, use_a2=True), Seg(out=qkv[:, 2 * D:], col_begin=2 * D, ldo=qkv.stride(0))])
            q3 = qkv.view(B, L, 3 * D)
            att = tw[e + ".att"]
            ops.attention(q3[:, :, :D], q3[:, :, D:2 * D], q3[:, :, 2 * D:], att.view(B, L, D), H, key_mask=fus_mask,
                          q_skip_mask=qskip, lse=tw[e + ".lse"], drop=self._drop(f"enc.{l}" + ".attn", pd),
                          order=self._order[fus_mask.data_ptr()], keep_bits=tw[e + ".kbits"] if self._bits else None)
            x = ops.linear(att, P[p + ".out.w"], P[p + ".out.b"], R=xin if pre else src, out=tw[e + ".x"], rows=rows_f,
                           drop=self._drop(f"enc.{l}" + ".drop1", pd))
            s1 = ops.layernorm(x, P[p + (".ln2.g" if pre else ".ln1.g")], P[p + (".ln2.b" if pre else ".ln1.b")], out=tw[e + ".s1"], row_skip=fskip)
            h = ops.linear(s1, P[p + ".ff1.w"], P[p + ".ff1.b"], act=ops.ACT_RELU, out=tw[e + ".h"], rows=rows_f,
                           drop=self._drop(f"enc.{l}" + ".ffn_act", pd))
            x2 = ops.linear(h, P[p + ".ff2.w"], P[p + ".ff2.b"], R=x if pre else s1, out=tw[e + ".x2"], rows=rows_f,
                            drop=self._drop(f"enc.{l}" + ".drop2", pd))
            last = l == c.detr_enc_layers - 1
            if pre:
                xin = x2
                if last:
                    ops.layernorm_add(x2, P["enc.norm.g"], P["enc.norm.b"], pos2, tw["mem"], tw["mempos"], row_skip=fskip)
                continue
            nsrc, nsp = (tw["mem"], tw["mempos"]) if last else (tw[f"e.{l + 1}.src"], tw[f"e.{l + 1}.srcpos"])
            ops.layernorm_add(x2, P[p + ".ln2.g"], P[p + ".ln2.b"], pos2, nsrc, nsp, row_skip=fskip)
        memory, mempos = tw["mem"], tw["mempos"]
        out["memory"] = memory.view(B, L, D)

        if regression:
            return self._regression_train(out, ws, tw, memory.view(B, L, D), fus_mask, v_duration, cur, side)

        mem3, mempos3 = memory.view(B, L, D), mempos.view(B, L, D)
        if dec_early is None:
            dec_fill_tgt()
        hs = ws["hs"]
        GQ = tw["GQ"]
        n_split = int(_lib.variant_env("MADE_WIDE_NSPLIT", "0")) or max(1, min(8, 256 // max(B, 1)))
        t3_stack = tw["dstack"]["tgt"][1:]
        for l in range(nd):
            p, d = f"detr_transformer.decoder.layers.{l}", f"d.{l}"
            tgt, tq = tw[d + ".tgt"], tw[d + ".tq"]
            qkv = tw[d + ".qkv"]
            if l == 0 and dec_early is not None:
                cur.wait_event(dec_early)
            else:
                dec_query_side(l)
            Win, bin_ = P[p + ".ca.in.w"], P[p + ".ca.in.b"]
            qprime, t1 = GQ[:, 1, l], tw[d + ".t1"]
            pooled = tw[d + ".pooled"]
            s_out = tw[d + ".s"] if Q == 1 else tw["s_raw"]
            ops.attention_wide(qprime.view(B, H, Q, D), mempos3, mem3, pooled.view(B, Q, H, D).permute(0, 2, 1, 3), scale=ca_scale,
                               key_mask=fus_mask, drop=self._drop(f"dec.{l}" + ".ca_attn", pd), sum_out=s_out,
                               n_split=n_split, part_o=ws["part_o"], part_ml=ws["part_ml"],
                               lse_out=tw["ca_lse"][l] if stage else None)
            if Q > 1:
                tw[d + ".s"].view(B, Q, H).copy_(s_out.view(B, H, Q).permute(0, 2, 1))
            attc = tw[d + ".attc"]
            if stage:
                ops.linear(pooled[:, :D], Win[2 * D:2 * D + hd], bin_[2 * D:], M=B * Q, N=hd, K=D, batch=H, a_z_stride=D, w_z_stride=hd * D,
                           segs=[Seg(out=attc, ldo=D, out_z_stride=hd)], bias_row_scale=tw[d + ".s"], bias_z_stride=hd)
            else:
                ops.linear(pooled[:, :D], Win[2 * D:2 * D + hd], None, M=B * Q, N=hd, K=D, batch=H, a_z_stride=D, w_z_stride=hd * D,
                           segs=[Seg(out=attc, ldo=D, out_z_stride=hd)])
                tr.head_bias(attc, tw[d + ".s"], bin_[2 * D:], H)
            if c.detr_pre_norm:
                tb = ops.linear(attc, P[p + ".ca.out.w"], P[p + ".ca.out.b"], R=tw[d + ".t_a"], out=tw[d + ".t_b"], drop=self._drop(f"dec.{l}" + ".drop2", pd))
                t2 = ops.layernorm(tb, P[p + ".ln3.g"], P[p + ".ln3.b"], out=tw[d + ".t2"])
                h = ops.linear(t2, P[p + ".ff1.w"], P[p + ".ff1.b"], act=ops.ACT_RELU, out=tw[d + ".h"], drop=self._drop(f"dec.{l}" + ".ffn_act", pd))
                ops.linear(h, P[p + ".ff2.w"], P[p + ".ff2.b"], R=tb, out=tw[d + ".t3"], drop=self._drop(f"dec.{l}" + ".drop3", pd))
                continue
            tb = ops.linear(attc, P[p + ".ca.out.w"], P[p + ".ca.out.b"], R=t1, out=tw[d + ".t_b"], drop=self._drop(f"dec.{l}" + ".drop2", pd))
            if stage:
                h = ops.dec_stage(tb, P[p + ".ff1.w"], P[p + ".ff1.b"], tw[d + ".h"], ln=(P[p + ".ln2.g"], P[p + ".ln2.b"]), x_out=tw[d + ".t2"],
                                  act=ops.ACT_RELU, drop=self._drop(f"dec.{l}" + ".ffn_act", pd))
                t2 = tw[d + ".t2"]
            else:
                t2 = ops.layernorm(tb, P[p + ".ln2.g"], P[p + ".ln2.b"], out=tw[d + ".t2"])
                h = ops.linear(t2, P[p + ".ff1.w"], P[p + ".ff1.b"], act=ops.ACT_RELU, out=tw[d + ".h"], drop=self._drop(f"dec.{l}" + ".ffn_act", pd))
            tcx = ops.linear(h, P[p + ".ff2.w"], P[p + ".ff2.b"], R=t2, out=tw[d + ".t_c"], drop=self._drop(f"dec.{l}" + ".drop3", pd))
            t3 = tw[d + ".t3"]
            if stage:
                if l + 1 == nd:
                    ops.layernorm(tcx, P[p + ".ln3.g"], P[p + ".ln3.b"], out=t3)
            elif l + 1 < nd:
                ops.layernorm_add(tcx, P[p + ".ln3.g"], P[p + ".ln3.b"], qp.expand(B * Q, D) if Q == 1 else qp.repeat(B, 1), t3, tw[f"d.{l + 1}.tq"])
            else:
                ops.layernorm(tcx, P[p + ".ln3.g"], P[p + ".ln3.b"], out=t3)
        ops.layernorm(t3_stack.reshape(nd * B * Q, D), P["dec.norm.g"], P["dec.norm.b"], out=hs.view(nd * B * Q, D))
        out["hs"] = hs.view(nd, B, Q, D)

        hs2 = hs.view(nd * B * Q, D)
        logits, spans = ws["logits"], ws["spans"]
        ops.linear(hs2, P["class_embed.w"], P["class_embed.b"], out=logits.view(-1, 2))
        h1 = ops.linear(hs2, P["span_embed.0.w"], P["span_embed.0.b"], act=ops.ACT_RELU, out=tw["h1"])
        h2 = ops.linear(h1, P["span_embed.1.w"], P["span_embed.1.b"], act=ops.ACT_RELU, out=tw["h2"])
        if c.predict_center == 1:
            ops.linear(h2, P["span_embed.2.w"], P["span_embed.2.b"], act=ops.ACT_SIGMOID, segs=[Seg(out=spans.view(-1, 2), ldo=2)])
            spans[..., 1] = (v_duration.to(self.device, torch.float32) / c.max_m_duration).view(1, B, 1)
        else:
            ops.linear(h2, P["span_embed.2.w"], P["span_embed.2.b"], act=ops.ACT_SIGMOID, out=spans.view(-1, 2))
        out.update(pred_logits=logits[-1], pred_spans=spans[-1], logits_all=logits, spans_all=spans)
        if c.moment_loss:
            last = hs[nd - 1]
            m1 = ops.linear(last, P["moment_embed.0.w"], P["moment_embed.0.b"], act=ops.ACT_RELU)
            m2 = ops.linear(m1, P["moment_embed.1.w"], P["moment_embed.1.b"], act=ops.ACT_RELU)
            m3 = ops.linear(m2, P["moment_embed.2.w"], P["moment_embed.2.b"], out_dtype=torch.float32)
            mf = ops.l2norm_rows(m3)
            if c.audio_short_cut:
                mq = music if Q == 1 else music[:, None, :].expand(B, Q, D).contiguous()
                tr.add3(m3, mf, mq, b_mod=B * Q * D)
                mf = ops.l2norm_rows(m3)
            out["moment_feats"] = mf.view(B, Q, D)
        pq = vid_sum = None
        if c.contrastive_align_loss:
            ops.linear(hs2, P["proj_q.w"], P["proj_q.b"], out=ws["pq_raw"])
            pq = ws["pq"]
            pq2 = pq.view(nd * B * Q, -1)
            if c.audio_short_cut:
                mq = music if Q == 1 else music[:, None, :].expand(B, Q, D).contiguous()
                ops.l2norm_rows(ws["pq_raw"], out_f32=tw["pq_n0"])
                tr.add3(tw["pq_s1"], tw["pq_n0"], mq, b_mod=B * Q * D)
                ops.l2norm_rows(tw["pq_s1"], out_f32=pq2)
                if c.aux_loss and nd > 1:
                    n_aux = (nd - 1) * B * Q
                    tr.add3(tw["pq_s2"][:n_aux], pq2[:n_aux], mq, b_mod=B * Q * D)
                    ops.l2norm_rows(tw["pq_s2"][:n_aux], out_f32=pq2[:n_aux])
            else:
                ops.l2norm_rows(ws["pq_raw"], out_f32=pq2)
            self._frame_rows_linear(frame, P["proj_v.w"], P["proj_v.b"], ws["pv_raw"], B, Tv)
            pv = ws["pv"]
            ops.l2norm_rows(ws["pv_raw"], out_f32=pv.view(B * Tv, pq.shape[-1]))
            vid_sum = ops.masked_mean(pv, None, out=ws["vid_sum"])
            out.update(proj_queries=pq[-1], proj_vid_mem=pv, proj_queries_all=pq)
        tg = self._inputs[4]
        pi, ti, cnt, status, cost = ops.hungarian_match(logits.view(nd * B, Q, 2), spans.view(nd * B, Q, 2), tg, c.foreground_label)
        losses, total = ops.set_criterion(logits, spans, tg, pi, ti, cnt, pq, vid_sum, P["empty_weight"], c.foreground_label, P["crit_weights"])
        self._match = (pi, ti, cnt)
        out.update(matcher_pred_idx=pi.view(nd, B, -1), matcher_tgt_idx=ti.view(nd, B, -1), matcher_count=cnt.view(nd, B),
                   matcher_status=status, criterion_losses=losses, localization_loss=total)
        cur.wait_stream(side)
        return out

    def _opt_stream(self):
        st = getattr(self, "_opt_st", None)
        if st is None:
            st = self._opt_st = torch.cuda.Stream(device=self.device)
        return st

    def _dec_stage_chain(self) -> bool:
        c = self.cfg
        return (self.tc == torch.bfloat16 and c.num_moment_queries == 1 and c.D in (256, 512) and not c.detr_pre_norm
                and _lib.variant_env("MADE_DEC_STAGE", "1") != "0")

    def _encode_train(self, feats: Tensor, mask: Tensor, which: str, ws, tw, row_off: int) -> None:
        c, P = self.cfg, self.P
        if c.agg_module == "mlp":
            return self._encode_train_mlp(feats, mask, which, ws, tw, row_off)
        B, T, Kin = feats.shape
        D, Hh = c.D, c.SA_temporal_heads
        proj, mod, pe, depth, tag = (("vit_proj", "video_transformer", "pe_video", c.video_transformer_depth, "v") if which == "video"
                                     else ("ast_proj", "audio_transformer", "pe_audio", c.audio_transformer_depth, "a"))
        cls = bool(c.with_cls_token)
        T1 = T + 1 if cls else T
        if P[pe].shape[0] < T1:
            raise ValueError(f"{which} position table holds {P[pe].shape[0]} positions < {T1}")
        nrow = B * T
        mflat = mask.reshape(-1)
        pt = dr.P_TEMPORAL
        name = "video" if which == "video" else "audio"
        act = ops.ACT_QUICKGELU if c.with_act_after_proj else ops.ACT_NONE
        zp = tw[tag + ".zproj"] if c.with_act_after_proj else None
        x = tw[f"{tag}.0.x0"]
        if cls:
            mask1 = tw[tag + ".mask1"]
            mask1[:, 0] = 1.0; mask1[:, 1:] = mask
            self._rows[mask1.data_ptr()] = ops.row_index(mask1, out=tw[tag + ".rows1"])
            self._order[mask1.data_ptr()] = ops.batch_order(mask1, out=tw[tag + ".order1"])
            x3 = x.view(B, T1, D)
            x3[:, 0] = (P["cls_" + name].float() + P[pe][0].float()).to(self.tc)
            lin_out = dict(segs=[Seg(out=x3[:, 1:], ldo=D, rows_per_batch=T, out_batch_stride=T1 * D)])
            pe_rows = P[pe][1:T1]
        else:
            mask1 = mask
            lin_out = dict(out=x, rows=self._rw(mflat))
            pe_rows = P[pe][:T]
        mflat1 = mask1.reshape(-1)
        rws = self._rw(mflat1)
        if self.tc == torch.bfloat16:
            xin = ops.cast_mask_rows(feats.view(nrow, Kin), mflat, tw[tag + ".xin"])
            ops.linear(xin, P[proj + ".w"], P[proj + ".b"], act=act, Zout=zp, R=pe_rows, r_row_mod=T, **lin_out)
        else:
            ops.linear(feats.view(nrow, Kin), P[proj + ".w"], P[proj + ".b"], a_row_mask=mflat, act=act, Zout=zp, R=pe_rows, r_row_mod=T, **lin_out)
        for l in range(depth):
            p, t = f"{mod}.layers.{l}", f"{tag}.{l}"
            x1 = ops.layernorm(x, P[p + ".ln1.g"], P[p + ".ln1.b"], out=tw[t + ".x1"], row_skip=mflat1)
            qkv = ops.linear(x1, P[p + ".in.w"], P[p + ".in.b"], out=tw[t + ".qkv"], rows=rws)
            q3 = qkv.view(B, T1, 3 * D)
            att = tw[t + ".att"]
            ops.attention(q3[:, :, :D], q3[:, :, D:2 * D], q3[:, :, 2 * D:], att.view(B, T1, D), Hh, key_mask=mask1, q_skip_mask=mask1,
                          lse=tw[t + ".lse"], drop=self._drop(f"{name}.{l}.attn", pt), order=self._order[mask1.data_ptr()],
# ... 205 lines not shown
            pq = ws["pq"] if c.contrastive_align_loss else None
            vid_sum = ws["vid_sum"] if c.contrastive_align_loss else None
            tr.set_criterion_bwd(logits, spans, tg, pi, ti, cnt, pq, vid_sum, P["empty_weight"], c.foreground_label, P["crit_weights"], g_loc,
                                 tw["dlog"], tw["dsp"], tw["dpq"] if pq is not None else None, tw["dvid_sum"] if pq is not None else None,
                                 ld_out=HEAD_PAD, through_sigmoid=True)
            hs2 = ws["hs"].view(nd * B * Q, D)
            dhs = tw["dhs"]
            dlog, dsp = tw["dlog"], tw["dsp"]
            if self.tc != torch.float32:
                tr.add3(tw["dlogsp_c"], tw["dlogsp"])
                dlog, dsp = tw["dlog_c"], tw["dsp_c"]
            heads_dw: list = []
            heads_dw.append(lambda: tr.gemm_tn(dlog[:, :2], hs2, G["class_embed.w"], accumulate=True, colsum=G["class_embed.b"]))
            ops.linear(dlog, P["class_embed.wt"], None, out=dhs)
            n_span = 1 if c.predict_center == 1 else 2
            heads_dw.append(lambda: tr.gemm_tn(dsp[:, :n_span], tw["h2"], G["span_embed.2.w"], accumulate=True, colsum=G["span_embed.2.b"]))
            dz2 = ops.linear(dsp, P["span_embed.2.wt"], None, out=tw["hg1"], gate=_lib.GATE_RELU_OUT, G=tw["h2"])
            dz1 = self._lin_bwd(dz2, tw["h1"], "span_embed.1", dx_out=tw["hg2"], gate=_lib.GATE_RELU_OUT, G=tw["h1"], later=heads_dw)
            self._lin_bwd(dz1, hs2, "span_embed.0", dx_out=dhs, R=dhs, later=heads_dw)
            if c.contrastive_align_loss:
                Dc = pq.shape[-1]
                dn = tw["dpq"]
                if c.audio_short_cut:
                    if c.aux_loss and nd > 1:
                        n_aux = (nd - 1) * B * Q
                        ds2 = tw["dpq_s2"][:n_aux]
                        tr.l2norm_bwd(tw["pq_s2"][:n_aux], dn[:n_aux], dx=ds2)
                        dmusic.add_(ds2.view(nd - 1, B, Q, D).sum((0, 2)))
                        dn[:n_aux].copy_(ds2)
                    tr.l2norm_bwd(tw["pq_s1"], dn, dx=tw["dpq_s"])
                    dmusic.add_(tw["dpq_s"].view(nd, B, Q, D).sum((0, 2)))
                    dn = tw["dpq_s"]
                tr.l2norm_bwd(ws["pq_raw"], dn, dx_alt=tw["dpq_raw"])
                self._lin_bwd(tw["dpq_raw"], hs2, "proj_q", dx_out=dhs, R=dhs, later=heads_dw)
                tr.l2norm_bwd(ws["pv_raw"], tw["dvid_sum"], dx_alt=tw["dpv_raw"], dy_rows_per=Tv)
                heads_dw.append(lambda: tr.gemm_tn(tw["dpv_raw"][:Tv], frame[0], G["proj_v.w"], accumulate=True, colsum=G["proj_v.b"], batch=(B, 1),
                                                   a_zs=(Tv * Dc, 0), b_zs=(frame.stride(0), 0), colsum_zs=(0, 0)))
                ops.linear(tw["dpv_raw"], P["proj_v.wt"], None, out=tw["dframe_x"])

            qp = P["query_embed"]
            mem3, mempos3 = tw["mem"].view(B, L, D), tw["mempos"].view(B, L, D)
            Lp = tw["PdS"].shape[-1]
            GQ, PdS = tw["GQ"], tw["PdS"]
            ca_scale = 1.0 / math.sqrt(hd)
            st = tw["dstack"]
            dtgt = None
            stage = self._dec_stage_chain()
            pre = bool(c.detr_pre_norm)
            S_all = tw["dS_S"]
            if not stage:
                ops.linear(GQ[0, 1].reshape(nd * HQ, D), mempos3[0], None, M=nd * HQ, N=L, K=D, batch=B, a_z_stride=GQ.stride(0), w_z_stride=L * D,
                           segs=[Seg(out=S_all, ldo=Lp, rows_per_batch=HQ, out_batch_stride=B * HQ * Lp, out_z_stride=HQ * Lp)])
            n_split_b = int(_lib.variant_env("MADE_WIDE_NSPLIT", "0")) or max(1, min(8, 256 // max(B, 1)))
            if stage:
                gN = tw["dgN"]
                tr.layernorm_bwd(tw["dstack"]["tgt"][1:].reshape(nd * B * Q, D), P["dec.norm.g"], dhs, gN, dgamma=G["dec.norm.g"], dbeta=G["dec.norm.b"])
            for l in range(nd - 1, -1, -1):
                p, d = f"detr_transformer.decoder.layers.{l}", f"d.{l}"
                g1, g2, g4 = tw["dg1"], tw["dg2"], tw["dg4"]
                if stage and _lib.variant_env("MADE_CHAIN_BUFS", "1") != "0":
                    ch = tw["dchain"][l]
                    g1a, g1b, g2a, g2b, g2c, dt_out = ch[0], ch[1], ch[2], ch[3], ch[4], ch[5]
                else:
                    g1a = g1b = g1
                    g2a = g2b = g2c = g2
                    dt_out = tw["dtgt"]
                Win, Wt = P[p + ".ca.in.w"], P[p + ".ca.in.wt"]
                g_ffn, g_z, g_ca, g_attc, g_q, g_qc, g_sa, gqkv = (st[k][l] for k in ("g_ffn", "g_z", "g_ca", "g_attc", "g_q", "g_qc", "g_sa", "g_qkv"))
                if stage:
                    tr.dec_stage_bwd(tw[d + ".t_c"], P[p + ".ln3.g"], gN[l * B * Q:(l + 1) * B * Q], P[p + ".ff2.wt"], g_z,
                                     dgamma_a=G[p + ".ln3.g"], dbeta_a=G[p + ".ln3.b"], add=dtgt, dx_out=g2a, a_out=g_ffn,
                                     drop_a=self._drop(f"dec.{l}" + ".drop3", pd), G=tw[d + ".h"], gate_scale=inv_keep)
                elif pre:
                    tr.layernorm_bwd(tw[d + ".t3"], P["dec.norm.g"], dhs[l * B * Q:(l + 1) * B * Q], g1, dgamma=G["dec.norm.g"], dbeta=G["dec.norm.b"], add=dtgt)
                    tr.gate_rows(g1, g_ffn, drop=self._drop(f"dec.{l}" + ".drop3", pd))
                else:
                    tr.layernorm_bwd(tw[d + ".t3"], P["dec.norm.g"], dhs[l * B * Q:(l + 1) * B * Q], g1, dgamma=G["dec.norm.g"], dbeta=G["dec.norm.b"], add=dtgt)
                    tr.layernorm_bwd(tw[d + ".t_c"], P[p + ".ln3.g"], g1, g2, dgamma=G[p + ".ln3.g"], dbeta=G[p + ".ln3.b"],
                                     dx_drop=g_ffn, drop=self._drop(f"dec.{l}" + ".drop3", pd))
                if not stage:
                    ops.linear(g_ffn, P[p + ".ff2.wt"], None, out=g_z, gate=_lib.GATE_RELU_OUT, G=tw[d + ".h"], gate_scale=inv_keep)
                if pre:
                    dn3 = ops.linear(g_z, P[p + ".ff1.wt"], None, out=g4)
                    tr.layernorm_bwd(tw[d + ".t_b"], P[p + ".ln3.g"], dn3, g2, dgamma=G[p + ".ln3.g"], dbeta=G[p + ".ln3.b"], add=g1,
                                     dx_drop=g_ca, drop=self._drop(f"dec.{l}" + ".drop2", pd))
                    dattc = ops.linear(g_ca, P[p + ".ca.out.wt"], None, out=g_attc)
                else:
                    dt2 = ops.linear(g_z, P[p + ".ff1.wt"], None, out=g1a, R=g2a)
                if pre:
                    pass
                elif stage:
                    dattc = tr.dec_stage_bwd(tw[d + ".t_b"], P[p + ".ln2.g"], dt2, P[p + ".ca.out.wt"], g_attc, dgamma_a=G[p + ".ln2.g"],
                                             dbeta_a=G[p + ".ln2.b"], dx_out=g2b, a_out=g_ca, drop_a=self._drop(f"dec.{l}" + ".drop2", pd))
                else:
                    tr.layernorm_bwd(tw[d + ".t_b"], P[p + ".ln2.g"], dt2, g2, dgamma=G[p + ".ln2.g"], dbeta=G[p + ".ln2.b"],
                                     dx_drop=g_ca, drop=self._drop(f"dec.{l}" + ".drop2", pd))
                    dattc = ops.linear(g_ca, P[p + ".ca.out.wt"], None, out=g_attc)
                dpooled = GQ[:, 0, l]
                qprime = GQ[:, 1, l]
                if stage:
                    ops.linear(dattc[:, :hd], Wt[:, 2 * D:2 * D + hd], None, M=B * Q, N=D, K=hd, batch=H, a_z_stride=hd, w_z_stride=hd,
                               segs=[Seg(out=dpooled, ldo=D, rows_per_batch=Q, out_batch_stride=dpooled.stride(0), out_z_stride=Q * D)])
                    tr.attention_wide_bwd(qprime, dpooled, tw[d + ".pooled"].view(B, HQ, D), mempos3, mem3, tw["ca_lse"][l].view(B, HQ),
                                          PdS[:, 0, l], PdS[:, 1, l], g_q, scale=ca_scale, key_mask=fus_mask, ssum=tw[d + ".s"].view(B, HQ),
                                          dattc=dattc, vbias=P[p + ".ca.in.b"][2 * D:], hd=hd, drop=self._drop(f"dec.{l}" + ".ca_attn", pd),
                                          n_split=n_split_b, part_dq=ws["part_o"])
                else:
                    tr.head_bias_bwd(dattc, tw[d + ".s"], P[p + ".ca.in.b"][2 * D:], G[p + ".ca.in.b"][2 * D:], tw["d_ds"], H)
                    d_ds = tw["d_ds"]
                    if Q > 1:
                        tw["dds_raw"].view(B, H, Q).copy_(d_ds.view(B, Q, H).permute(0, 2, 1))
                        d_ds = tw["dds_raw"]
                    ops.linear(dattc[:, :hd], Wt[:, 2 * D:2 * D + hd], None, M=B * Q, N=D, K=hd, batch=H, a_z_stride=hd, w_z_stride=hd,
                               segs=[Seg(out=dpooled, ldo=D, rows_per_batch=Q, out_batch_stride=dpooled.stride(0), out_z_stride=Q * D)])
                    S, dP = S_all[l], tw["dS_dP"]
                    ops.linear(dpooled[0], mem3[0], None, M=HQ, N=L, K=D, batch=B, a_z_stride=dpooled.stride(0), w_z_stride=L * D,
                               segs=[Seg(out=dP, ldo=Lp, out_z_stride=HQ * Lp)])
                    tr.softmax_bwd(S, dP, fus_mask, HQ, ca_scale, PdS[:, 0, l], PdS[:, 1, l], tw["dSt"], HQ, L, extra=d_ds.view(-1),
                                   drop=self._drop(f"dec.{l}" + ".ca_attn", pd), ldo=Lp, ldt=HQ, out_batch_stride=PdS.stride(0))
                    gq_out = g_q if Q == 1 else tw["gq_raw"]
                    tr.gemm_tn(tw["dSt"][0], mempos3[0], gq_out[0], batch=(B, 1), a_zs=(L * HQ, 0), b_zs=(L * D, 0), c_zs=(HQ * D, 0),
                               row_mask=fus_mask, mask_zs=(L, 0))
                    if Q > 1:
                        g_q.view(B, Q, H, D).copy_(gq_out.view(B, H, Q, D).permute(0, 2, 1, 3))
                dq2 = g_q.view(B * Q, H * D)
                ops.linear(dq2[:, :D], Win[D:D + hd], None, M=B * Q, N=hd, K=D, batch=H, a_z_stride=D, w_z_stride=hd * D,
                           segs=[Seg(out=g_qc, ldo=D, out_z_stride=hd)])
                dt1q = st["dt1q"][l]
                if pre:
                    ops.linear(g_qc, Wt[:, :D], None, out=dt1q)
                    tr.layernorm_bwd(tw[d + ".t_a"], P[p + ".ln2.g"], dt1q, g1, dgamma=G[p + ".ln2.g"], dbeta=G[p + ".ln2.b"], add=g2,
                                     dx_drop=g_sa, drop=self._drop(f"dec.{l}" + ".drop1", pd))
                    if Q == 1:
                        ops.linear(g_sa, P[p + ".sa.out.wt"], None, segs=[Seg(out=gqkv[:, 2 * D:], ldo=gqkv.stride(0))],
                                   drop=self._drop(f"dec.{l}" + ".sa_attn", pd), drop_ld=H, drop_col_div=hd)
                        dn1 = ops.linear(gqkv[:, 2 * D:], P[p + ".sa.in.wt"][:, 2 * D:], None, out=g4)
                    else:
                        datt = ops.linear(g_sa, P[p + ".sa.out.wt"], None, out=g4)
                        qkv = tw[d + ".qkv"]
                        q3, g3v = qkv.view(B, Q, 3 * D), gqkv.view(B, Q, 3 * D)
                        tr.attention_bwd(q3[:, :, :D], q3[:, :, D:2 * D], q3[:, :, 2 * D:], tw[d + ".att"].view(B, Q, D), datt.view(B, Q, D),
                                         g3v[:, :, :D], g3v[:, :, D:2 * D], g3v[:, :, 2 * D:], tw[d + ".lse"], tw["d_delta"], H,
                                         drop=self._drop(f"dec.{l}" + ".sa_attn", pd))
                        dn1 = ops.linear(gqkv, P[p + ".sa.in.wt"], None, out=g2)
                        dqk = ops.linear(gqkv[:, :2 * D], P[p + ".sa.in.wt"][:, :2 * D], None, out=g4)
                        tr.colsum(dqk.view(B, Q * D), G["query_embed"].view(-1))
                    dtgt = tr.layernorm_bwd(tw[d + ".tgt"], P[p + ".ln1.g"], dn1, tw["dtgt"], dgamma=G[p + ".ln1.g"], dbeta=G[p + ".ln1.b"], add=g1)
                    continue
                ops.linear(g_qc, Wt[:, :D], None, out=g1b, R=g2b, Zout=dt1q)
                if stage:
                    tr.dec_stage_bwd(tw[d + ".t_a"], P[p + ".ln1.g"], g1b, P[p + ".sa.out.wt"], gqkv[:, 2 * D:], dgamma_a=G[p + ".ln1.g"],
                                     dbeta_a=G[p + ".ln1.b"], dx_out=g2c, a_out=g_sa, drop_a=self._drop(f"dec.{l}" + ".drop1", pd),
                                     drop_o=self._drop(f"dec.{l}" + ".sa_attn", pd), drop_o_ld=H, drop_o_col_div=hd)
                    dtgt = ops.linear(gqkv[:, 2 * D:], P[p + ".sa.in.wt"][:, 2 * D:], None, R=g2c, out=dt_out)
                    continue
                tr.layernorm_bwd(tw[d + ".t_a"], P[p + ".ln1.g"], g1, g2, dgamma=G[p + ".ln1.g"], dbeta=G[p + ".ln1.b"],
                                 dx_drop=g_sa, drop=self._drop(f"dec.{l}" + ".drop1", pd))
                if Q == 1:
                    ops.linear(g_sa, P[p + ".sa.out.wt"], None, segs=[Seg(out=gqkv[:, 2 * D:], ldo=gqkv.stride(0))],
# ... 707 lines not shown
```

Before: 13790 pairs/s.

## Plan variable-length key slices per sample for wide cross-attention fwd/bwd

Adds a device-side planning kernel that scans the key mask once per step, works out each sample's valid key-tile count, and picks a slice cap so all samples' slices fit within a fixed number of workgroup slots (about the CU count). The wide attention forward and backward then launch a 1-D grid where each block reads its sample, tile range and precomputed mask bits from the plan, and a planned combine kernel merges only that sample's slices. This is meant to balance work across CUs when samples have very different valid lengths, and to skip each block's own full-mask scan and empty trailing tiles. The cost is an extra plan kernel per step, a larger partial-output buffer, and a fixed n_split of 8.

```diff
diff --git a/include/made_hip.h b/include/made_hip.h
--- a/include/made_hip.h
+++ b/include/made_hip.h
@@ -223,6 +223,42 @@
 } MadeWideAttnBwdArgs;
 int made_attention_wide_bwd(const MadeWideAttnBwdArgs* args, void* stream);
 
+#define MADE_WIDE_PLAN_HEAD 4
+#define MADE_WIDE_PLAN_SAMPLE 4
+#define MADE_WIDE_PLAN_SLOT 16
+#define MADE_WIDE_PLAN_SLOT_BITS 8
+MADE_HOST_DEVICE static inline int64_t made_wide_plan_words(int64_t B, int64_t n_slots) {
+    return MADE_WIDE_PLAN_HEAD + MADE_WIDE_PLAN_SAMPLE * B + MADE_WIDE_PLAN_SLOT * n_slots;
+}
+MADE_HOST_DEVICE static inline int32_t made_wide_slice_count(const int32_t* tiles, int32_t stride, int32_t B, int32_t c, int32_t max_slices) {
+    int32_t total = 0;
+    for (int32_t b = 0; b < B; ++b) {
+        const int32_t t = tiles[b * stride];
+        const int32_t n = t > c ? (t + c - 1) / c : 1;
+        if (n > max_slices) return -1;
+        total += n;
+    }
+    return total;
+}
+MADE_HOST_DEVICE static inline int32_t made_wide_slice_cap(const int32_t* tiles, int32_t stride, int32_t B, int32_t n_slots, int32_t max_slices) {
+    int32_t tmax = 1;
+    for (int32_t b = 0; b < B; ++b) tmax = tiles[b * stride] > tmax ? tiles[b * stride] : tmax;
+    for (int32_t c = 1; c <= tmax; ++c) {
+        const int32_t n = made_wide_slice_count(tiles, stride, B, c, max_slices);
+        if (n >= 0 && n <= n_slots) return c;
+    }
+    return 0;
+}
+MADE_HOST_DEVICE static inline int32_t made_wide_slice_first(int32_t tiles, int32_t n, int32_t s) {
+    return s * (tiles / n) + (s < tiles % n ? s : tiles % n);
+}
+MADE_HOST_DEVICE static inline int32_t made_wide_slice_len(int32_t tiles, int32_t n, int32_t s) { return tiles / n + (s < tiles % n ? 1 : 0); }
+
+int made_wide_slice_plan(const float* key_mask, int64_t B, int64_t L, int32_t n_slots, int32_t max_slices,
+                         const int32_t* batch_order, void* plan, int64_t plan_bytes, void* stream);
+int made_attention_wide_planned(const MadeWideAttnArgs* args, const void* plan, int32_t n_slots, void* stream);
+int made_attention_wide_bwd_planned(const MadeWideAttnBwdArgs* args, const void* plan, int32_t n_slots, void* stream);
+
 int made_tape_begin(void);
 int made_tape_end(uint64_t* handle);
 int made_tape_replay(uint64_t handle);
diff --git a/mgsv_amd/_lib.py b/mgsv_amd/_lib.py
--- a/mgsv_amd/_lib.py
+++ b/mgsv_amd/_lib.py
@@ -20,6 +20,12 @@
 GATE_NONE, GATE_RELU_OUT, GATE_GELU_Z, GATE_QUICKGELU_Z, GATE_SIGMOID_OUT = 0, 1, 2, 3, 4
 
 vp, i64, i32, f32 = C.c_void_p, C.c_int64, C.c_int32, C.c_float
+
+WIDE_PLAN_HEAD, WIDE_PLAN_SAMPLE, WIDE_PLAN_SLOT, WIDE_PLAN_SLOT_BITS = 4, 4, 16, 8
+
+
+def wide_plan_words(B: int, n_slots: int) -> int:
+    return WIDE_PLAN_HEAD + WIDE_PLAN_SAMPLE * B + WIDE_PLAN_SLOT * n_slots
 
 
 class MadeDropout(C.Structure):
@@ -221,6 +227,9 @@
     "made_attention": (C.c_int, [C.POINTER(MadeAttnArgs), vp]),
     "made_attention_wide": (C.c_int, [C.POINTER(MadeWideAttnArgs), vp]),
     "made_attention_wide_bwd": (C.c_int, [C.POINTER(MadeWideAttnBwdArgs), vp]),
+    "made_wide_slice_plan": (C.c_int, [vp, i64, i64, i32, i32, vp, vp, i64, vp]),
+    "made_attention_wide_planned": (C.c_int, [C.POINTER(MadeWideAttnArgs), vp, i32, vp]),
+    "made_attention_wide_bwd_planned": (C.c_int, [C.POINTER(MadeWideAttnBwdArgs), vp, i32, vp]),
     "made_layernorm": (C.c_int, [vp, i32, i64, i64, i64, vp, vp, vp, i32, i64, i64, i64, f32, vp, vp]),
     "made_layernorm_add": (C.c_int, [vp, i32, i64, vp, vp, vp, i32, i64, vp, i32, i64, vp, i64, i64, i64, f32, vp, vp]),
     "made_cast_mask_rows": (C.c_int, [vp, i64, vp, vp, i32, i64, i64, i64, vp]),
diff --git a/mgsv_amd/csrc/attention_wide.hip b/mgsv_amd/csrc/attention_wide.hip
--- a/mgsv_amd/csrc/attention_wide.hip
+++ b/mgsv_amd/csrc/attention_wide.hip
@@ -13,8 +13,9 @@
 template <> struct Frag<bf16_t> { typedef bf16x8 type; };
 
 
-template <typename TC, int D, bool DB, int NSL, bool X3 = false>
-__global__ __launch_bounds__(NTHREADS) void attention_wide_kernel(const MadeWideAttnArgs a) {
+template <typename TC, int D, bool DB, int NSL, bool X3 = false, bool PLAN = false>
+__global__ __launch_bounds__(NTHREADS) void attention_wide_kernel(const MadeWideAttnArgs a, const int32_t* __restrict__ plan) {
+    static_assert(!PLAN || (DB && sizeof(TC) == 2 && NSL == 4 && !X3), "the planned launch: LDS-DMA variant, one query tile");
     typedef typename Frag<TC>::type frag_t;
     constexpr int SZ = (int)sizeof(TC);
     constexpr bool IS_BF16 = SZ == 2;
@@ -40,10 +41,21 @@
     const int tid = threadIdx.x, lane = tid & 63, wave = tid >> 6;
     const int r = lane & 31, hh = lane >> 5;
     const int sl = wave % NSL, qt = wave / NSL;
+    int32_t pl[MADE_WIDE_PLAN_SLOT] = {};
+    if constexpr (PLAN) {
+        const u32x4* sp = (const u32x4*)(plan + MADE_WIDE_PLAN_HEAD + MADE_WIDE_PLAN_SAMPLE * a.B + (int64_t)MADE_WIDE_PLAN_SLOT * blockIdx.x);
+#pragma unroll
+        for (int i = 0; i < 4; ++i) {
+            const u32x4 v = sp[i];
+            pl[4 * i] = (int32_t)v[0]; pl[4 * i + 1] = (int32_t)v[1]; pl[4 * i + 2] = (int32_t)v[2]; pl[4 * i + 3] = (int32_t)v[3];
+        }
+        if (pl[0] < 0 || pl[0] >= a.B || pl[3] < 0 || pl[3] >= a.n_split || pl[1] < 0 || pl[2] < 0 || (int64_t)(pl[1] + pl[2]) * WKEY >= a.L + WKEY ||
+            pl[4] < 0 || pl[4] >= a.L) return;
+    }
     const bool batch_fast = gridDim.x == (unsigned)a.B && (a.NQ1 * a.NQ2 + WQB - 1) / WQB != (int64_t)a.B;
-    const int64_t b = batch_fast ? blockIdx.x : blockIdx.y;
+    const int64_t b = PLAN ? (int64_t)pl[0] : (batch_fast ? blockIdx.x : blockIdx.y);
     const int64_t nq_total = a.NQ1 * a.NQ2;
-    const int64_t nq0 = (int64_t)(batch_fast ? blockIdx.y : blockIdx.x) * WQB + qt * WQ;
+    const int64_t nq0 = PLAN ? (int64_t)qt * WQ : (int64_t)(batch_fast ? blockIdx.y : blockIdx.x) * WQB + qt * WQ;
 
     const TC* Kg = (const TC*)a.K + b * a.k_bs;
     const TC* Ag = a.Kadd ? (const TC*)a.Kadd + b * a.kadd_bs : nullptr;
@@ -115,7 +127,25 @@
 
     int64_t l_eff = a.L;
     int first_valid = 0;
-    {
+    if constexpr (PLAN) {
+        first_valid = pl[4];
+        const int nt = pl[2];
+        if (nt <= MADE_WIDE_PLAN_SLOT_BITS) {
+            uint32_t w = (uint32_t)pl[8];
+#pragma unroll
+            for (int i = 1; i < MADE_WIDE_PLAN_SLOT_BITS; ++i) w = tid == i ? (uint32_t)pl[8 + i] : w;
+            if (tid < MADE_WIDE_PLAN_SLOT_BITS) lds_mbits[tid] = w;
+        } else {
+            const int nk = nt * WKEY, k0 = pl[1] * WKEY;
+            for (int j = tid; j < ((nk + 63) & ~63); j += NTHREADS) {
+                const int key = k0 + j;
+                const float mv = maskg[key < (int)a.L ? key : (int)a.L - 1];
+                const unsigned long long bal = __ballot(j < nk && key < (int)a.L && mv != 0.f);
+                if (lane == 0) { lds_mbits[j / 32] = (uint32_t)bal; lds_mbits[j / 32 + 1] = (uint32_t)(bal >> 32); }
+            }
+        }
+        __syncthreads();
+    } else {
         const int lpad = (int)((a.L + 63) / 64) * 64;
         int last = -1, first = 0x7fffffff;
         for (int j = tid; j < lpad; j += NTHREADS) {
@@ -140,15 +170,17 @@
     const int64_t nsplit = a.n_split > 1 ? a.n_split : 1;
     const int64_t tiles_all = (l_eff + WKEY - 1) / WKEY;
     const int64_t tiles_per = (tiles_all + nsplit - 1) / nsplit;
-    const int64_t tile0 = (int64_t)blockIdx.z * tiles_per;
-    const int64_t ntiles = tile0 >= tiles_all ? 0 : (tile0 + tiles_per <= tiles_all ? tiles_per : tiles_all - tile0);
+    const int64_t tile0 = PLAN ? (int64_t)pl[1] : (int64_t)blockIdx.z * tiles_per;
+    const int64_t ntiles = PLAN ? (int64_t)pl[2] : (tile0 >= tiles_all ? 0 : (tile0 + tiles_per <= tiles_all ? tiles_per : tiles_all - tile0));
+    const int64_t mb0 = PLAN ? tile0 : 0;
+    const int64_t zslice = PLAN ? (int64_t)pl[3] : (int64_t)blockIdx.z;
     typedef __attribute__((address_space(3))) void* lds_ptr_t;
     typedef const __attribute__((address_space(1))) void* glb_ptr_t;
     auto issue_tile = [&](int64_t key0, int stage) __attribute__((always_inline)) {
         constexpr int ROWS_PER_PIECE = DMA ? 1024 / (D * SZ) : 1;
         constexpr int NPIECE = WKEY / ROWS_PER_PIECE;
         constexpr int CPRW = D * SZ / 16;
-        const uint32_t bits = lds_mbits[key0 / WKEY];
+        const uint32_t bits = lds_mbits[key0 / WKEY - mb0];
         unsigned char* st = lds + stage * KV_STAGE;
         const unsigned char* Kb = (const unsigned char*)Kg;
         const unsigned char* Vb = (const unsigned char*)Vg;
@@ -179,7 +211,7 @@
         uint32_t tbits = 0xffffffffu;
         if constexpr (DMA) {
             asm volatile("s_waitcnt vmcnt(0) lgkmcnt(0)\n\ts_barrier" ::: "memory");
-            tbits = lds_mbits[t];
+            tbits = lds_mbits[t - mb0];
         } else if (NSTAGE == 2) {
             if (tt + 1 < ntiles) load_tile((t + 1) * WKEY);
         } else {
@@ -340,13 +372,13 @@
     const float inv = 1.f / l_tot;
     const float sd_tot = sd_run + __shfl_xor(sd_run, 32);
     const bool live_q = my_q < nq_total;
-    if (nsplit == 1 && !live_q) return;
-    if (nsplit == 1 && sl == 0 && hh == 0) {
+    if (!PLAN && nsplit == 1 && !live_q) return;
+    if (!PLAN && nsplit == 1 && sl == 0 && hh == 0) {
         if (a.sum_out) a.sum_out[b * nq_total + my_q] = a.drop.p > 0.f ? sd_tot * inv : 1.f;
         if (a.lse_out) a.lse_out[b * nq_total + my_q] = m_run + logf(l_tot);
     }
-    if (nsplit > 1) {
-        const int64_t prow = (b * nsplit + blockIdx.z) * nq_total + (live_q ? my_q : 0);
+    if (PLAN || nsplit > 1) {
+        const int64_t prow = (b * nsplit + zslice) * nq_total + (live_q ? my_q : 0);
         if (live_q) {
             float* po = a.part_o + prow * D + sl * DS;
 #pragma unroll
@@ -490,8 +522,8 @@
     const int64_t qtiles = (nq + WQB - 1) / WQB;
     const bool batch_fast = qtiles > 1 && qtiles <= 8 && qtiles != a.B;
     dim3 grid((unsigned)(batch_fast ? a.B : qtiles), (unsigned)(batch_fast ? qtiles : a.B), (unsigned)nsplit), block(NTHREADS);
-    if (SZ == 4 && g_made_f32_products) hipLaunchKernelGGL((attention_wide_kernel<TC, D, DB, NSL, SZ == 4>), grid, block, lds_bytes, st, a);
-    else hipLaunchKernelGGL((attention_wide_kernel<TC, D, DB, NSL>), grid, block, lds_bytes, st, a);
+    if (SZ == 4 && g_made_f32_products) hipLaunchKernelGGL((attention_wide_kernel<TC, D, DB, NSL, SZ == 4>), grid, block, lds_bytes, st, a, (const int32_t*)nullptr);
+    else hipLaunchKernelGGL((attention_wide_kernel<TC, D, DB, NSL>), grid, block, lds_bytes, st, a, (const int32_t*)nullptr);
     int rc = made_check_launch("made_attention_wide");
     if (rc != MADE_OK || nsplit == 1) return rc;
     const int64_t rows = a.B * nq;
@@ -499,6 +531,205 @@
     return made_check_launch("made_attention_wide(combine)");
 }
 
+constexpr int PLAN_T = 1024;
+__global__ __launch_bounds__(PLAN_T) void wide_slice_plan_kernel(const float* __restrict__ mask, int B, int L, int n_slots, int max_slices,
+                                                                 const int32_t* __restrict__ order, int32_t* __restrict__ plan) {
+    __shared__ int32_t s_tiles[PLAN_T], s_first[PLAN_T], s_ord[PLAN_T];
+    __shared__ int32_t s_cap;
+    extern __shared__ __attribute__((aligned(16))) unsigned char lds[];
+    uint32_t* s_bits = (uint32_t*)lds;
+    const int tid = threadIdx.x, lane = tid & 63, wave = tid >> 6;
+    const int nch = (L + 63) / 64, wpr = 2 * nch;
+    if (tid == 0) s_cap = 0x7fffffff;
+    for (int b = wave; b < B; b += PLAN_T / 64) {
+        const float* m = mask + (int64_t)b * L;
+        int last = -1, first = -1;
+        for (int c0 = 0; c0 < nch; c0 += 8) {
+            float v[8];
+#pragma unroll
+            for (int j = 0; j < 8; ++j) {
+                const int i = (c0 + j) * 64 + lane;
+                v[j] = m[i < L ? i : L - 1];
+            }
+#pragma unroll
+            for (int j = 0; j < 8; ++j) {
+                const int i = (c0 + j) * 64 + lane;
+                const unsigned long long bal = __ballot(i < L && v[j] != 0.f);
+                if (c0 + j < nch) {
+                    if (lane == 0) { s_bits[b * wpr + 2 * (c0 + j)] = (uint32_t)bal; s_bits[b * wpr + 2 * (c0 + j) + 1] = (uint32_t)(bal >> 32); }
+                    if (bal) {
+                        last = (c0 + j) * 64 + 63 - __clzll(bal);
+                        if (first < 0) first = (c0 + j) * 64 + __ffsll(bal) - 1;
+                    }
+                }
+            }
+        }
+        if (lane == 0) { s_tiles[b] = (last + 1 + 31) / 32; s_first[b] = first < 0 ? 0 : first; }
+    }
+    if (tid < B) {
+        const int o = order ? order[tid] : tid;
+        s_ord[tid] = o >= 0 && o < B ? o : tid;
+    }
+    __syncthreads();
+    int tmax = 1;
+    for (int b = 0; b < B; ++b) tmax = max(tmax, s_tiles[b]);
+    for (int c = tid + 1; c <= tmax; c += PLAN_T) {
+        const int n = made_wide_slice_count(s_tiles, 1, B, c, max_slices);
+        if (n >= 0 && n <= n_slots) atomicMin(&s_cap, c);
+    }
+    __syncthreads();
+    const int cap = s_cap <= tmax ? s_cap : tmax;
+    int used = 0;
+    for (int r = 0; r < B; ++r) { const int t = s_tiles[s_ord[r]]; used += t > cap ? (t + cap - 1) / cap : 1; }
+    if (tid == 0) { plan[0] = cap; plan[1] = used; plan[2] = n_slots; plan[3] = max_slices; }
+    int32_t* slots = plan + MADE_WIDE_PLAN_HEAD + MADE_WIDE_PLAN_SAMPLE * B;
+    if (tid < B) {
+        int slot0 = 0;
+        for (int r = 0; r < tid; ++r) { const int t = s_tiles[s_ord[r]]; slot0 += t > cap ? (t + cap - 1) / cap : 1; }
+        const int b = s_ord[tid], t = s_tiles[b], fv = s_first[b];
+        const int n = t > cap ? (t + cap - 1) / cap : 1;
+        int32_t* sm = plan + MADE_WIDE_PLAN_HEAD + MADE_WIDE_PLAN_SAMPLE * b;
+        sm[0] = t; sm[1] = slot0; sm[2] = n; sm[3] = fv;
+        for (int s = 0; s < n && slot0 + s < n_slots; ++s) {
+            int32_t* sp = slots + (int64_t)MADE_WIDE_PLAN_SLOT * (slot0 + s);
+            const int t0 = made_wide_slice_first(t, n, s), tn = made_wide_slice_len(t, n, s);
+            sp[0] = b; sp[1] = t0; sp[2] = tn; sp[3] = s; sp[4] = fv; sp[5] = n; sp[6] = t; sp[7] = 0;
+            for (int i = 0; i < MADE_WIDE_PLAN_SLOT_BITS; ++i) sp[8 + i] = i < tn ? (int32_t)s_bits[b * wpr + t0 + i] : 0;
+        }
+    }
+    for (int w = used + tid; w < n_slots; w += PLAN_T) {
+        int32_t* sp = slots + (int64_t)MADE_WIDE_PLAN_SLOT * w;
+        sp[0] = -1;
+        for (int i = 1; i < MADE_WIDE_PLAN_SLOT; ++i) sp[i] = 0;
+    }
+}
+
+__global__ __launch_bounds__(NTHREADS) void attention_wide_combine_planned_kernel(const MadeWideAttnArgs a, const int32_t* __restrict__ plan) {
+    constexpr int MAXS = 8;
+    const int lane = threadIdx.x & 63;
+    const int64_t nq_total = a.NQ1 * a.NQ2;
+    const int64_t row = (int64_t)blockIdx.x * (NTHREADS / 64) + (threadIdx.x >> 6);
+    if (row >= a.B * nq_total) return;
+    const int64_t b = row / nq_total, q = row % nq_total;
+    const int D = (int)a.D;
+    const int cap = (int)a.n_split;
+    int ns = plan[MADE_WIDE_PLAN_HEAD + MADE_WIDE_PLAN_SAMPLE * b + 2];
+    ns = ns < 1 ? 1 : (ns > MAXS ? MAXS : ns);
+    ns = ns > cap ? cap : ns;
+    float Lsum = 0.f, Dsum = 0.f;
+    f32x4 acc[2];
+#pragma unroll
+    for (int i = 0; i < 2; ++i) { acc[i][0] = acc[i][1] = acc[i][2] = acc[i][3] = 0.f; }
+    f32x4 t[MAXS][2];
+    float ml[MAXS][3];
+#pragma unroll
+    for (int sp = 0; sp < MAXS; ++sp) {
+        const int64_t pr = (b * cap + (sp < ns ? sp : ns - 1)) * nq_total + q;
+        ml[sp][0] = a.part_ml[pr * 4]; ml[sp][1] = a.part_ml[pr * 4 + 1]; ml[sp][2] = a.part_ml[pr * 4 + 2];
+#pragma unroll
+        for (int i = 0; i < 2; ++i) {
+            const int c = (i * 64 + lane) * 4;
+            t[sp][i] = *(const f32x4*)(a.part_o + pr * D + (c < D ? c : 0));
+        }
+    }
+    float M = -INFINITY;
+#pragma unroll
+    for (int sp = 0; sp < MAXS; ++sp) if (sp < ns) M = fmaxf(M, ml[sp][0]);
+    const float Muse = (M == -INFINITY) ? 0.f : M;
+#pragma unroll
+    for (int sp = 0; sp < MAXS; ++sp) {
+        if (sp < ns) {
+            const float w = expf(ml[sp][0] - Muse);
+            Lsum += ml[sp][1] * w;
+            Dsum += ml[sp][2] * w;
+#pragma unroll
+            for (int i = 0; i < 2; ++i)
+#pragma unroll
+                for (int j = 0; j < 4; ++j) acc[i][j] += t[sp][i][j] * w;
+        }
+    }
+    const float inv = 1.f / Lsum;
+    if (a.sum_out && lane == 0) a.sum_out[b * nq_total + q] = Dsum * inv;
+    if (a.lse_out && lane == 0) a.lse_out[b * nq_total + q] = Muse + logf(Lsum);
+    const int64_t obase = b * a.o_bs + (q / a.NQ2) * a.o_s1 + (q % a.NQ2) * a.o_s2;
+#pragma unroll
+    for (int i = 0; i < 2; ++i) {
+        int c = (i * 64 + lane) * 4;
+        if (c < D) {
+            if (a.o_dtype == MADE_F32) {
+                f32x4 pk; pk[0] = acc[i][0] * inv; pk[1] = acc[i][1] * inv; pk[2] = acc[i][2] * inv; pk[3] = acc[i][3] * inv;
+                *(f32x4*)((float*)a.O + obase + c) = pk;
+            } else {
+                bf16x4 pk; pk[0] = (bf16_t)(acc[i][0] * inv); pk[1] = (bf16_t)(acc[i][1] * inv);
+                pk[2] = (bf16_t)(acc[i][2] * inv); pk[3] = (bf16_t)(acc[i][3] * inv);
+                *(bf16x4*)((bf16_t*)a.O + obase + c) = pk;
+            }
+        }
+    }
+}
+
+template <int D>
+int launch_wide_planned(const MadeWideAttnArgs& a, const int32_t* plan, int n_slots, hipStream_t st) {
+    constexpr size_t kBase = (size_t)2 * (WKEY * D * 2 + WKEY * D * 2) + 4 * 1024 * 4 + 2 * 32 * 4;
+    constexpr size_t kCap = kBase + 8192 < 160 * 1024 ? kBase + 8192 : 160 * 1024;
+    const size_t lds_bytes = kBase + (size_t)((a.L + 63) / 64 * 2 + 2) * 4;
+    if (lds_bytes > kCap) {
+        made_set_error("made_attention_wide_planned: L=%lld keys: the mask bit row does not fit in LDS beside the K / V stages", (long long)a.L);
+        return MADE_ERR_UNSUPPORTED;
+    }
+    static bool attr_done = false;
+    if (!attr_done) {
+        hipError_t e = hipFuncSetAttribute((const void*)attention_wide_kernel<bf16_t, D, true, 4, false, true>, hipFuncAttributeMaxDynamicSharedMemorySize, (int)kCap);
+        if (e != hipSuccess) {
+            made_set_error("made_attention_wide_planned: cannot reserve %zu bytes of LDS: %s", kCap, hipGetErrorString(e));
+            return MADE_ERR_HIP;
+        }
+        attr_done = true;
+    }
+    hipLaunchKernelGGL((attention_wide_kernel<bf16_t, D, true, 4, false, true>), dim3((unsigned)n_slots), dim3(NTHREADS), lds_bytes, st, a, plan);
+    int rc = made_check_launch("made_attention_wide_planned");
+    if (rc != MADE_OK) return rc;
+    const int64_t rows = a.B * a.NQ1 * a.NQ2;
+    hipLaunchKernelGGL(attention_wide_combine_planned_kernel, dim3((unsigned)((rows + 3) / 4)), dim3(NTHREADS), 0, st, a, plan);
+    return made_check_launch("made_attention_wide_planned(combine)");
+}
+
+}
+
+extern "C" int made_wide_slice_plan(const float* key_mask, int64_t B, int64_t L, int32_t n_slots, int32_t max_slices,
+                                    const int32_t* batch_order, void* plan, int64_t plan_bytes, void* stream) {
+    MADE_REQUIRE(key_mask && plan && B > 0 && L > 0 && n_slots > 0 && max_slices > 0, "made_wide_slice_plan: bad arguments");
+    MADE_REQUIRE(plan_bytes >= 4 * made_wide_plan_words(B, n_slots), "made_wide_slice_plan: plan_bytes=%lld < %lld", (long long)plan_bytes,
+                 (long long)(4 * made_wide_plan_words(B, n_slots)));
+    MADE_REQUIRE(((uintptr_t)plan % 16) == 0, "made_wide_slice_plan: the plan must be 16-byte aligned");
+    MADE_UNSUPPORTED(B <= n_slots && n_slots <= PLAN_T, "made_wide_slice_plan: B=%lld samples need B <= n_slots=%d <= %d", (long long)B, n_slots, PLAN_T);
+    MADE_UNSUPPORTED(max_slices <= 8, "made_wide_slice_plan: max_slices=%d (the merges take at most 8 slices)", max_slices);
+    const int64_t bits_bytes = B * ((L + 63) / 64 * 2) * 4;
+    MADE_UNSUPPORTED(L <= 32768 && bits_bytes <= 40 * 1024, "made_wide_slice_plan: B=%lld x L=%lld: the valid-key bits do not fit one workgroup's LDS", (long long)B, (long long)L);
+    hipLaunchKernelGGL(wide_slice_plan_kernel, dim3(1), dim3(PLAN_T), (size_t)bits_bytes, (hipStream_t)stream, key_mask, (int)B, (int)L, (int)n_slots,
+                       (int)max_slices, batch_order, (int32_t*)plan);
+    return made_check_launch("made_wide_slice_plan");
+}
+
+extern "C" int made_attention_wide_planned(const MadeWideAttnArgs* args, const void* plan, int32_t n_slots, void* stream) {
+    MADE_REQUIRE(args != nullptr && plan != nullptr, "made_attention_wide_planned: null args / plan");
+    const MadeWideAttnArgs& a = *args;
+    MADE_REQUIRE(a.Q && a.K && a.V && a.O, "made_attention_wide_planned: null tensor");
+    MADE_REQUIRE(a.B >= 0 && a.NQ1 >= 0 && a.NQ2 > 0 && a.L > 0, "made_attention_wide_planned: bad dims");
+    MADE_REQUIRE(a.o_dtype == MADE_F32 || a.o_dtype == MADE_BF16, "made_attention_wide_planned: bad o_dtype %d", a.o_dtype);
+    MADE_UNSUPPORTED(a.dtype == MADE_BF16 && (a.D == 256 || a.D == 512) && a.Kadd == nullptr && a.key_mask != nullptr && a.NQ1 * a.NQ2 <= WQ,
+                     "made_attention_wide_planned: bf16, D in {256, 512}, no Kadd, a key mask and at most %d query rows per sample", WQ);
+    MADE_UNSUPPORTED(a.B <= n_slots && n_slots <= PLAN_T, "made_attention_wide_planned: B <= n_slots <= %d", PLAN_T);
+    MADE_UNSUPPORTED(a.q_bs % 8 == 0 && a.q_s1 % 8 == 0 && a.q_s2 % 8 == 0 && a.k_bs % 8 == 0 && a.ldk % 8 == 0 && a.v_bs % 8 == 0 && a.ldv % 8 == 0 &&
+                     a.o_bs % 4 == 0 && a.o_s1 % 4 == 0 && a.o_s2 % 4 == 0, "made_attention_wide_planned: strides must keep 16-byte alignment");
+    MADE_UNSUPPORTED(((uintptr_t)a.Q % 16) == 0 && ((uintptr_t)a.K % 16) == 0 && ((uintptr_t)a.V % 16) == 0 && ((uintptr_t)a.O % 16) == 0 &&
+                     ((uintptr_t)plan % 16) == 0, "made_attention_wide_planned: base pointers must be 16-byte aligned");
+    MADE_REQUIRE(a.drop.p >= 0.f && a.drop.p < 1.f, "made_attention_wide_planned: dropout p out of [0,1)");
+    MADE_REQUIRE(a.n_split >= 1 && a.n_split <= 8 && a.part_o != nullptr && a.part_ml != nullptr,
+                 "made_attention_wide_planned: n_split = the slice capacity of part_o / part_ml (1..8)");
+    if (a.B == 0 || a.NQ1 == 0) return MADE_OK;
+    hipStream_t st = (hipStream_t)stream;
+    return a.D == 512 ? launch_wide_planned<512>(a, (const int32_t*)plan, n_slots, st) : launch_wide_planned<256>(a, (const int32_t*)plan, n_slots, st);
 }
 
 extern "C" int made_attention_wide(const MadeWideAttnArgs* args, void* stream) {
diff --git a/mgsv_amd/csrc/attention_wide_bwd.hip b/mgsv_amd/csrc/attention_wide_bwd.hip
--- a/mgsv_amd/csrc/attention_wide_bwd.hip
+++ b/mgsv_amd/csrc/attention_wide_bwd.hip
@@ -9,8 +9,8 @@
 typedef __attribute__((address_space(3))) void* lds_ptr_t;
 typedef const __attribute__((address_space(1))) void* glb_ptr_t;
 
-template <int D>
-__global__ __launch_bounds__(NT) void attention_wide_bwd_kernel(const MadeWideAttnBwdArgs a) {
+template <int D, bool PLAN = false>
+__global__ __launch_bounds__(NT) void attention_wide_bwd_kernel(const MadeWideAttnBwdArgs a, const int32_t* __restrict__ plan) {
     constexpr int DS = D / 4;
     constexpr int NQF = DS / 16;
     constexpr int NDT = DS / 32;
@@ -25,7 +25,18 @@
     const int tid = threadIdx.x, lane = tid & 63, wave = __builtin_amdgcn_readfirstlane(tid >> 6);
     const int r = lane & 31, hh = lane >> 5;
     const int sl = wave;
-    const int64_t b = blockIdx.y;
+    int32_t pl[MADE_WIDE_PLAN_SLOT] = {};
+    if constexpr (PLAN) {
+        const u32x4* sp = (const u32x4*)(plan + MADE_WIDE_PLAN_HEAD + MADE_WIDE_PLAN_SAMPLE * a.B + (int64_t)MADE_WIDE_PLAN_SLOT * blockIdx.x);
+#pragma unroll
+        for (int i = 0; i < 4; ++i) {
+            const u32x4 v = sp[i];
+            pl[4 * i] = (int32_t)v[0]; pl[4 * i + 1] = (int32_t)v[1]; pl[4 * i + 2] = (int32_t)v[2]; pl[4 * i + 3] = (int32_t)v[3];
+        }
+        if (pl[0] < 0 || pl[0] >= a.B || pl[3] < 0 || pl[3] >= a.n_split || pl[1] < 0 || pl[2] < 0 || (int64_t)(pl[1] + pl[2]) * BK >= a.L + BK ||
+            pl[4] < 0 || pl[4] >= a.L) return;
+    }
+    const int64_t b = PLAN ? (int64_t)pl[0] : (int64_t)blockIdx.y;
     const int NQ = (int)a.NQ;
     const int rq = (r & 7) < NQ ? (r & 7) : NQ - 1;
     const bool live = r < NQ;
@@ -69,7 +80,25 @@
 
     int64_t l_eff = a.L;
     int first_valid = 0;
-    {
+    if constexpr (PLAN) {
+        first_valid = pl[4];
+        const int nt = pl[2];
+        if (nt <= MADE_WIDE_PLAN_SLOT_BITS) {
+            uint32_t w = (uint32_t)pl[8];
+#pragma unroll
+            for (int i = 1; i < MADE_WIDE_PLAN_SLOT_BITS; ++i) w = tid == i ? (uint32_t)pl[8 + i] : w;
+            if (tid < MADE_WIDE_PLAN_SLOT_BITS) lds_mbits[tid] = w;
+        } else {
+            const int nk = nt * BK, k0 = pl[1] * BK;
+            for (int j = tid; j < ((nk + 63) & ~63); j += NT) {
+                const int key = k0 + j;
+                const float mv = maskg[key < (int)a.L ? key : (int)a.L - 1];
+                const unsigned long long bal = __ballot(j < nk && key < (int)a.L && mv != 0.f);
+                if (lane == 0) { lds_mbits[j / 32] = (uint32_t)bal; lds_mbits[j / 32 + 1] = (uint32_t)(bal >> 32); }
+            }
+        }
+        __syncthreads();
+    } else {
         const int lpad = (int)((a.L + 63) / 64) * 64;
         int last = -1, first = 0x7fffffff;
         for (int j = tid; j < lpad; j += NT) {
@@ -93,16 +122,19 @@
     const float delta = ((lds_q[8 + rq] + lds_q[8 + MAXQ + rq]) + (lds_q[8 + 2 * MAXQ + rq] + lds_q[8 + 3 * MAXQ + rq])) + extra * ssum;
 
     const int64_t nsplit = a.n_split > 1 ? a.n_split : 1;
-    const int64_t tiles_all = (l_eff + BK - 1) / BK;
+    const int64_t tiles_all = PLAN ? (int64_t)pl[6] : (l_eff + BK - 1) / BK;
     const int64_t tiles_L = (a.L + BK - 1) / BK;
     const int64_t tiles_per = (tiles_all + nsplit - 1) / nsplit;
-    const int64_t tile0 = (int64_t)blockIdx.z * tiles_per;
-    const int64_t ntiles = tile0 >= tiles_all ? 0 : (tile0 + tiles_per <= tiles_all ? tiles_per : tiles_all - tile0);
+    const int64_t tile0 = PLAN ? (int64_t)pl[1] : (int64_t)blockIdx.z * tiles_per;
+    const int64_t ntiles = PLAN ? (int64_t)pl[2] : (tile0 >= tiles_all ? 0 : (tile0 + tiles_per <= tiles_all ? tiles_per : tiles_all - tile0));
+    const int64_t mb0 = PLAN ? tile0 : 0;
+    const int64_t zslice = PLAN ? (int64_t)pl[3] : (int64_t)blockIdx.z;
+    const int64_t zcount = PLAN ? (int64_t)(pl[5] > 0 ? pl[5] : 1) : nsplit;
 
     auto issue_tile = [&](int64_t key0, int stage) __attribute__((always_inline)) {
         constexpr int ROWS_PER_PIECE = 1024 / ROWB;
         constexpr int NPIECE = BK / ROWS_PER_PIECE;
-        const uint32_t bits = lds_mbits[key0 / BK];
+        const uint32_t bits = lds_mbits[key0 / BK - mb0];
         unsigned char* st = lds + stage * STAGE;
         const unsigned char* Kb = (const unsigned char*)Kg;
         const unsigned char* Vb = (const unsigned char*)Vg;
@@ -140,7 +172,7 @@
         const int64_t t = tile0 + tt;
         const int cur = (int)(tt & 1);
         asm volatile("s_waitcnt vmcnt(0) lgkmcnt(0)\n\ts_barrier" ::: "memory");
-        const uint32_t tbits = lds_mbits[t];
+        const uint32_t tbits = lds_mbits[t - mb0];
         const unsigned char* lds_k = lds + cur * STAGE;
         const unsigned char* lds_v = lds_k + BK * ROWB;
 
@@ -225,7 +257,7 @@
         }
     }
     if (wave < 2 && live) {
-        for (int64_t tz = tiles_all + blockIdx.z; tz < tiles_L; tz += nsplit) {
+        for (int64_t tz = tiles_all + zslice; tz < tiles_L; tz += zcount) {
 #pragma unroll
             for (int g4 = 0; g4 < 4; ++g4) {
                 const int64_t key0 = tz * BK + 8 * g4 + 4 * hh;
@@ -237,7 +269,7 @@
         }
     }
 
-    if (nsplit == 1) {
+    if (!PLAN && nsplit == 1) {
         if (live) {
             bf16_t* dq = (bf16_t*)a.dQ + b * a.dq_bs + (int64_t)r * a.ld_dq + sl * DS;
 #pragma unroll
@@ -253,7 +285,7 @@
         return;
     }
     if (live) {
-        float* po = a.part_dq + ((b * nsplit + blockIdx.z) * NQ + r) * D + sl * DS;
+        float* po = a.part_dq + ((b * nsplit + zslice) * NQ + r) * D + sl * DS;
 #pragma unroll
         for (int d = 0; d < NDT; ++d)
 #pragma unroll
@@ -310,13 +342,101 @@
         attr_done = true;
     }
     const int64_t nsplit = a.n_split > 1 ? a.n_split : 1;
-    hipLaunchKernelGGL((attention_wide_bwd_kernel<D>), dim3(1, (unsigned)a.B, (unsigned)nsplit), dim3(NT), lds_bytes, st, a);
+    hipLaunchKernelGGL((attention_wide_bwd_kernel<D>), dim3(1, (unsigned)a.B, (unsigned)nsplit), dim3(NT), lds_bytes, st, a, (const int32_t*)nullptr);
     int rc = made_check_launch("made_attention_wide_bwd");
     if (rc != MADE_OK || nsplit == 1) return rc;
     hipLaunchKernelGGL(wide_bwd_merge_kernel, dim3((unsigned)((a.B * a.NQ + 3) / 4)), dim3(NT), 0, st, a);
     return made_check_launch("made_attention_wide_bwd(merge)");
 }
 
+__global__ __launch_bounds__(NT) void wide_bwd_merge_planned_kernel(const MadeWideAttnBwdArgs a, const int32_t* __restrict__ plan) {
+    constexpr int MAXS = 8;
+    const int lane = threadIdx.x & 63;
+    const int64_t row = (int64_t)blockIdx.x * 4 + (threadIdx.x >> 6);
+    if (row >= a.B * a.NQ) return;
+    const int64_t b = row / a.NQ, q = row % a.NQ;
+    const int D = (int)a.D;
+    const int per = D / 64;
+    const int cap = (int)a.n_split;
+    int ns = plan[MADE_WIDE_PLAN_HEAD + MADE_WIDE_PLAN_SAMPLE * b + 2];
+    ns = ns < 1 ? 1 : (ns > MAXS ? MAXS : ns);
+    ns = ns > cap ? cap : ns;
+    f32x4 t0[MAXS], t1[MAXS];
+#pragma unroll
+    for (int sp = 0; sp < MAXS; ++sp) {
+        const float* pp = a.part_dq + ((b * cap + (sp < ns ? sp : ns - 1)) * a.NQ + q) * D + lane * per;
+        t0[sp] = *(const f32x4*)pp;
+        t1[sp] = *(const f32x4*)(pp + (per == 8 ? 4 : 0));
+    }
+    float acc[8];
+#pragma unroll
+    for (int j = 0; j < 8; ++j) acc[j] = 0.f;
+#pragma unroll
+    for (int sp = 0; sp < MAXS; ++sp) {
+        if (sp < ns) {
+            acc[0] += t0[sp][0]; acc[1] += t0[sp][1]; acc[2] += t0[sp][2]; acc[3] += t0[sp][3];
+            acc[4] += t1[sp][0]; acc[5] += t1[sp][1]; acc[6] += t1[sp][2]; acc[7] += t1[sp][3];
+        }
+    }
+    bf16_t* dq = (bf16_t*)a.dQ + b * a.dq_bs + q * a.ld_dq + lane * per;
+    bf16x4 p0; p0[0] = (bf16_t)acc[0]; p0[1] = (bf16_t)acc[1]; p0[2] = (bf16_t)acc[2]; p0[3] = (bf16_t)acc[3];
+    *(bf16x4*)dq = p0;
+    if (per == 8) {
+        bf16x4 p1; p1[0] = (bf16_t)acc[4]; p1[1] = (bf16_t)acc[5]; p1[2] = (bf16_t)acc[6]; p1[3] = (bf16_t)acc[7];
+        *(bf16x4*)(dq + 4) = p1;
+    }
+}
+
+template <int D>
+int launch_wide_bwd_planned(const MadeWideAttnBwdArgs& a, const int32_t* plan, int n_slots, hipStream_t st) {
+    constexpr size_t kBase = (size_t)2 * 2 * BK * D * 2 + (size_t)(4 * 2 * BK * MAXQ + 8 + 4 * MAXQ) * 4;
+    const size_t lds_bytes = kBase + (size_t)((a.L + 63) / 64 * 2 + 2) * 4;
+    if (lds_bytes > 160 * 1024) {
+        made_set_error("made_attention_wide_bwd_planned: L=%lld keys: the mask bit row does not fit in LDS beside the K / V stages", (long long)a.L);
+        return MADE_ERR_UNSUPPORTED;
+    }
+    static bool attr_done = false;
+    if (!attr_done) {
+        hipError_t e = hipFuncSetAttribute((const void*)attention_wide_bwd_kernel<D, true>, hipFuncAttributeMaxDynamicSharedMemorySize, 160 * 1024);
+        if (e != hipSuccess) {
+            made_set_error("made_attention_wide_bwd_planned: cannot reserve LDS: %s", hipGetErrorString(e));
+            return MADE_ERR_HIP;
+        }
+        attr_done = true;
+    }
+    hipLaunchKernelGGL((attention_wide_bwd_kernel<D, true>), dim3((unsigned)n_slots), dim3(NT), lds_bytes, st, a, plan);
+    int rc = made_check_launch("made_attention_wide_bwd_planned");
+    if (rc != MADE_OK) return rc;
+    hipLaunchKernelGGL(wide_bwd_merge_planned_kernel, dim3((unsigned)((a.B * a.NQ + 3) / 4)), dim3(NT), 0, st, a, plan);
+    return made_check_launch("made_attention_wide_bwd_planned(merge)");
+}
+
+}
+
+extern "C" int made_attention_wide_bwd_planned(const MadeWideAttnBwdArgs* args, const void* plan, int32_t n_slots, void* stream) {
+    MADE_REQUIRE(args != nullptr && plan != nullptr, "made_attention_wide_bwd_planned: null args / plan");
+    const MadeWideAttnBwdArgs& a = *args;
+    MADE_REQUIRE(a.Q && a.dO && a.O && a.K && a.V && a.lse && a.Pd && a.dS && a.dQ, "made_attention_wide_bwd_planned: null tensor");
+    MADE_REQUIRE(a.B >= 0 && a.NQ > 0 && a.L > 0, "made_attention_wide_bwd_planned: bad dims");
+    MADE_UNSUPPORTED(a.NQ <= MAXQ && (a.D == 256 || a.D == 512) && a.key_mask != nullptr,
+                     "made_attention_wide_bwd_planned: NQ <= %d query rows per sample, D in {256, 512} and a key mask", MAXQ);
+    MADE_UNSUPPORTED(a.B <= n_slots && n_slots <= 1024, "made_attention_wide_bwd_planned: B <= n_slots <= 1024");
+    MADE_UNSUPPORTED(a.q_bs % 8 == 0 && a.ld_q % 8 == 0 && a.do_bs % 8 == 0 && a.ld_do % 8 == 0 && a.o_bs % 8 == 0 && a.ld_o % 8 == 0 &&
+                     a.k_bs % 8 == 0 && a.ldk % 8 == 0 && a.v_bs % 8 == 0 && a.ldv % 8 == 0 && a.p_bs % 4 == 0 && a.ld_p % 4 == 0 &&
+                     a.dq_bs % 4 == 0 && a.ld_dq % 4 == 0, "made_attention_wide_bwd_planned: strides must keep the rows aligned (16 bytes in, 8 bytes out)");
+    MADE_UNSUPPORTED(((uintptr_t)a.Q % 16) == 0 && ((uintptr_t)a.dO % 16) == 0 && ((uintptr_t)a.O % 16) == 0 && ((uintptr_t)a.K % 16) == 0 &&
+                     ((uintptr_t)a.V % 16) == 0 && ((uintptr_t)a.Pd % 8) == 0 && ((uintptr_t)a.dS % 8) == 0 && ((uintptr_t)a.dQ % 8) == 0 &&
+                     ((uintptr_t)plan % 16) == 0, "made_attention_wide_bwd_planned: base pointers must be aligned");
+    MADE_REQUIRE(a.ld_p >= a.L, "made_attention_wide_bwd_planned: ld_p < L");
+    MADE_REQUIRE(a.drop.p >= 0.f && a.drop.p < 1.f, "made_attention_wide_bwd_planned: dropout p out of [0,1)");
+    if (a.dattc && !a.extra) {
+        MADE_REQUIRE(a.vbias != nullptr && a.hd > 0 && a.hd % 8 == 0, "made_attention_wide_bwd_planned: dattc needs vbias and hd (a multiple of 8)");
+        MADE_UNSUPPORTED(a.hd * a.NQ == a.D, "made_attention_wide_bwd_planned: dattc needs the one-query layout NQ * hd == D; pass `extra` otherwise");
+    }
+    MADE_REQUIRE(a.n_split >= 1 && a.n_split <= 8 && a.part_dq != nullptr, "made_attention_wide_bwd_planned: n_split = the slice capacity of part_dq (1..8)");
+    if (a.B == 0) return MADE_OK;
+    hipStream_t st = (hipStream_t)stream;
+    return a.D == 512 ? launch_wide_bwd_planned<512>(a, (const int32_t*)plan, n_slots, st) : launch_wide_bwd_planned<256>(a, (const int32_t*)plan, n_slots, st);
 }
 
 extern "C" int made_attention_wide_bwd(const MadeWideAttnBwdArgs* args, void* stream) {
diff --git a/mgsv_amd/ops.py b/mgsv_amd/ops.py
--- a/mgsv_amd/ops.py
+++ b/mgsv_amd/ops.py
@@ -3,7 +3,7 @@
 import ctypes as C
 import math
 from dataclasses import dataclass
-from typing import Optional, Sequence
+from typing import NamedTuple, Optional, Sequence
 
 import torch
 
@@ -393,10 +393,41 @@
     return b.permute(0, 1, 3, 2, 4).reshape(B, H, Lq, nkt * 32)[..., :Lk].bool()
 
 
+class WidePlan(NamedTuple):
+    words: Tensor
+    B: int
+    L: int
+    n_slots: int
+    max_slices: int
+
+    def header(self):
+        return tuple(int(x) for x in self.words[:_lib.WIDE_PLAN_HEAD].tolist())
+
+    def samples(self) -> Tensor:
+        return self.words[_lib.WIDE_PLAN_HEAD:_lib.WIDE_PLAN_HEAD + _lib.WIDE_PLAN_SAMPLE * self.B].view(self.B, _lib.WIDE_PLAN_SAMPLE)
+
+    def slots(self) -> Tensor:
+        return self.words[_lib.WIDE_PLAN_HEAD + _lib.WIDE_PLAN_SAMPLE * self.B:][:_lib.WIDE_PLAN_SLOT * self.n_slots].view(self.n_slots, _lib.WIDE_PLAN_SLOT)
+
+
+def wide_slice_plan(key_mask: Tensor, *, n_slots: int, max_slices: int = 8, order: Optional[Tensor] = None, out: Optional[Tensor] = None) -> WidePlan:
+    assert key_mask.dim() == 2
+    B, L = key_mask.shape
+    words = _lib.wide_plan_words(B, n_slots)
+    if out is None:
+        out = torch.empty(words, device=key_mask.device, dtype=torch.int32)
+    assert out.dtype == torch.int32 and out.is_contiguous() and out.numel() >= words
+    if order is not None:
+        assert order.dtype == torch.int32 and order.numel() == B
+    check(lib().made_wide_slice_plan(_p(_f32(key_mask.contiguous(), "key_mask")), B, L, n_slots, max_slices, _p(order), _p(out), 4 * out.numel(),
+                                     _stream()), "made_wide_slice_plan")
+    return WidePlan(out, B, L, n_slots, max_slices)
+
+
 def attention_wide(Q: Tensor, K: Tensor, V: Tensor, O: Tensor, *, scale: float, Kadd: Optional[Tensor] = None,
                    key_mask: Optional[Tensor] = None, shared_q: bool = False, n_split: int = 1,
                    part_o: Optional[Tensor] = None, part_ml: Optional[Tensor] = None, drop=None,
-                   sum_out: Optional[Tensor] = None, lse_out: Optional[Tensor] = None) -> Tensor:
+                   sum_out: Optional[Tensor] = None, lse_out: Optional[Tensor] = None, plan: Optional[WidePlan] = None) -> Tensor:
     assert Q.dim() == 4 and O.dim() == 4 and K.dim() == 3 and V.dim() == 3
     assert Q.stride(3) == 1 and O.stride(3) == 1 and K.stride(2) == 1 and V.stride(2) == 1
     assert Q.dtype == K.dtype == V.dtype
@@ -415,7 +446,9 @@
     a.o_bs, a.o_s1, a.o_s2 = O.stride(0), O.stride(1), O.stride(2)
     a.scale = scale
     nq = a.NQ1 * a.NQ2
-    if n_split > 1:
+    if plan is not None:
+        assert key_mask is not None and (plan.B, plan.L) == (B, L) and n_split >= plan.max_slices, "the plan is not this call's"
+    if n_split > 1 or plan is not None:
         if part_o is None:
             part_o = torch.empty(B * n_split * nq * D, device=Q.device, dtype=torch.float32)
             part_ml = torch.empty(B * n_split * nq * 4, device=Q.device, dtype=torch.float32)
@@ -432,8 +465,9 @@
     esz = 4 if a.dtype == F32 else 2
     _timed("attention_wide_" + ("f32" if a.dtype == F32 else "bf16"), 4.0 * B * nq * L * D,
            esz * B * (2 * L * D + 2 * nq * D),
-           lambda: check(lib().made_attention_wide(C.byref(a), _stream()), "made_attention_wide"),
-           f"B={B} NQ={nq} L={L} D={D} kadd={int(Kadd is not None)}")
+           (lambda: check(lib().made_attention_wide(C.byref(a), _stream()), "made_attention_wide")) if plan is None else
+           (lambda: check(lib().made_attention_wide_planned(C.byref(a), _p(plan.words), plan.n_slots, _stream()), "made_attention_wide_planned")),
+           f"B={B} NQ={nq} L={L} D={D} kadd={int(Kadd is not None)}" + (" planned" if plan is not None else ""))
     return O
 
 
diff --git a/mgsv_amd/ops_train.py b/mgsv_amd/ops_train.py
--- a/mgsv_amd/ops_train.py
+++ b/mgsv_amd/ops_train.py
@@ -318,7 +318,7 @@
 def attention_wide_bwd(Q: Tensor, dO: Tensor, O: Tensor, K: Tensor, V: Tensor, lse: Tensor, Pd: Tensor, dS: Tensor, dQ: Tensor, *, scale: float,
                        key_mask: Optional[Tensor] = None, ssum: Optional[Tensor] = None, extra: Optional[Tensor] = None,
                        dattc: Optional[Tensor] = None, vbias: Optional[Tensor] = None, hd: int = 0, drop=None, n_split: int = 1,
-                       part_dq: Optional[Tensor] = None) -> Tensor:
+                       part_dq: Optional[Tensor] = None, plan=None) -> Tensor:
     assert Q.dim() == 3 and dO.shape == Q.shape and O.shape == Q.shape and dQ.shape == Q.shape and K.dim() == 3 and V.shape == K.shape
     B, NQ, D = Q.shape
     L = K.shape[1]
@@ -337,13 +337,17 @@
     a.q_bs, a.ld_q, a.do_bs, a.ld_do, a.o_bs, a.ld_o = Q.stride(0), Q.stride(1), dO.stride(0), dO.stride(1), O.stride(0), O.stride(1)
     a.k_bs, a.ldk, a.v_bs, a.ldv = K.stride(0), K.stride(1), V.stride(0), V.stride(1)
     a.scale = float(scale)
-    if n_split > 1:
+    if plan is not None:
+        assert key_mask is not None and (plan.B, plan.L) == (B, L) and n_split >= plan.max_slices, "the plan is not this call's"
+    if n_split > 1 or plan is not None:
         assert part_dq is not None and part_dq.dtype == torch.float32 and part_dq.numel() >= B * n_split * NQ * D
         a.n_split, a.part_dq = n_split, _p(part_dq)
     if drop is not None and drop[2] > 0.0:
         set_drop(a.drop, drop)
     _timed("made_attention_wide_bwd", 6.0 * B * NQ * L * D, 2.0 * B * (2 * L * D + 4 * NQ * D + 2 * NQ * L),
-                lambda: check(lib().made_attention_wide_bwd(C.byref(a), _stream()), "made_attention_wide_bwd"), f"B={B} NQ={NQ} L={L} D={D}")
+                (lambda: check(lib().made_attention_wide_bwd(C.byref(a), _stream()), "made_attention_wide_bwd")) if plan is None else
+                (lambda: check(lib().made_attention_wide_bwd_planned(C.byref(a), _p(plan.words), plan.n_slots, _stream()), "made_attention_wide_bwd_planned")),
+                f"B={B} NQ={NQ} L={L} D={D}" + (" planned" if plan is not None else ""))
     return dQ
 
 
diff --git a/mgsv_amd/trainer.py b/mgsv_amd/trainer.py
--- a/mgsv_amd/trainer.py
+++ b/mgsv_amd/trainer.py
@@ -11,6 +11,8 @@
 from .config import MadeConfig
 from .engine import MadeEngine
 from .ops import Seg, round_up
+
+WIDE_SLICES = 8
 
 Tensor = torch.Tensor
 XA = "video_guided_to_music_pooling_cross_transformer"
@@ -463,6 +465,7 @@
         i32 = torch.int32
         ws.update(rows_v=(E(B * Tv, dtype=i32), E(1, dtype=i32)), rows_a=(E(B * Ta, dtype=i32), E(1, dtype=i32)), rows_f=(E(rows, dtype=i32), E(1, dtype=i32)),
                   order_v=E(B, dtype=i32), order_a=E(B, dtype=i32), order_f=E(B, dtype=i32))
+        ws.update(wide_plan=E(_lib.wide_plan_words(B, self._wide_slots()), dtype=i32))
         BQ = B * Q
         stacks = dict(tgt=E(nd + 1, BQ, D), tq=E(nd + 1, BQ, D), qkv=E(nd, BQ, 3 * D), att=E(nd, BQ, D), t_a=E(nd, BQ, D), t1=E(nd, BQ, D),
                       t1q=E(nd, BQ, D), qc=E(nd, BQ, D), pooled=E(nd, BQ, H * D), attc=E(nd, BQ, D), t_b=E(nd, BQ, D), t2=E(nd, BQ, D),
@@ -527,6 +530,9 @@
             self._order[fm.data_ptr()] = ops.batch_order(fm, out=tw["order_v"])
             self._rows[fus_mask.data_ptr()] = ops.row_index(fus_mask, out=tw["rows_f"])
             self._order[fus_mask.data_ptr()] = ops.batch_order(fus_mask, out=tw["order_f"])
+            self._wide_plan = (ops.wide_slice_plan(fus_mask, n_slots=self._wide_slots(), max_slices=WIDE_SLICES,
+                                                   order=self._order[fus_mask.data_ptr()], out=tw["wide_plan"])
+                               if "regression" not in c.mml_localization and self._wide_planned_ok(B, H * Q, D) else None)
             pos = ops.sine_pe(fus_mask, P["dim_t"], out=ws["pos"])
             self._encode_train(self._inputs[0], fm, "video", ws, tw, 0)
         self._encode_train(self._inputs[1], sm, "audio", ws, tw, Tv)
@@ -709,6 +715,9 @@
         hs = ws["hs"]
         GQ = tw["GQ"]
         n_split = int(_lib.variant_env("MADE_WIDE_NSPLIT", "0")) or max(1, min(8, 256 // max(B, 1)))
+        wplan = self._wide_plan if _lib.variant_env("MADE_WIDE_PLANNED", "1") != "0" else None
+        if wplan is not None:
+            n_split = WIDE_SLICES
         t3_stack = tw["dstack"]["tgt"][1:]
         for l in range(nd):
             p, d = f"detr_transformer.decoder.layers.{l}", f"d.{l}"
@@ -725,7 +734,7 @@
             ops.attention_wide(qprime.view(B, H, Q, D), mempos3, mem3, pooled.view(B, Q, H, D).permute(0, 2, 1, 3), scale=ca_scale,
                                key_mask=fus_mask, drop=self._drop(f"dec.{l}" + ".ca_attn", pd), sum_out=s_out,
                                n_split=n_split, part_o=ws["part_o"], part_ml=ws["part_ml"],
-                               lse_out=tw["ca_lse"][l] if stage else None)
+                               lse_out=tw["ca_lse"][l] if stage else None, plan=wplan)
             if Q > 1:
                 tw[d + ".s"].view(B, Q, H).copy_(s_out.view(B, H, Q).permute(0, 2, 1))
             attc = tw[d + ".attc"]
@@ -819,6 +828,14 @@
         if st is None:
             st = self._opt_st = torch.cuda.Stream(device=self.device)
         return st
+
+    def _wide_slots(self) -> int:
+        if getattr(self, "_wide_slots_n", None) is None:
+            self._wide_slots_n = max(8, min(1024, _lib.device_info()[1]))
+        return self._wide_slots_n
+
+    def _wide_planned_ok(self, B: int, HQ: int, D: int) -> bool:
+        return self.tc == torch.bfloat16 and D in (256, 512) and HQ <= 32 and B <= self._wide_slots()
 
     def _dec_stage_chain(self) -> bool:
         c = self.cfg
@@ -1130,6 +1147,9 @@
                 ops.linear(GQ[0, 1].reshape(nd * HQ, D), mempos3[0], None, M=nd * HQ, N=L, K=D, batch=B, a_z_stride=GQ.stride(0), w_z_stride=L * D,
                            segs=[Seg(out=S_all, ldo=Lp, rows_per_batch=HQ, out_batch_stride=B * HQ * Lp, out_z_stride=HQ * Lp)])
             n_split_b = int(_lib.variant_env("MADE_WIDE_NSPLIT", "0")) or max(1, min(8, 256 // max(B, 1)))
+            wplan = self._wide_plan if HQ <= 8 and _lib.variant_env("MADE_WIDE_PLANNED", "1") != "0" else None
+            if wplan is not None:
+                n_split_b = WIDE_SLICES
             if stage:
                 gN = tw["dgN"]
                 tr.layernorm_bwd(tw["dstack"]["tgt"][1:].reshape(nd * B * Q, D), P["dec.norm.g"], dhs, gN, dgamma=G["dec.norm.g"], dbeta=G["dec.norm.b"])
@@ -1182,7 +1202,7 @@
                     tr.attention_wide_bwd(qprime, dpooled, tw[d + ".pooled"].view(B, HQ, D), mempos3, mem3, tw["ca_lse"][l].view(B, HQ),
                                           PdS[:, 0, l], PdS[:, 1, l], g_q, scale=ca_scale, key_mask=fus_mask, ssum=tw[d + ".s"].view(B, HQ),
                                           dattc=dattc, vbias=P[p + ".ca.in.b"][2 * D:], hd=hd, drop=self._drop(f"dec.{l}" + ".ca_attn", pd),
-                                          n_split=n_split_b, part_dq=ws["part_o"])
+                                          n_split=n_split_b, part_dq=ws["part_o"], plan=wplan)
                 else:
                     tr.head_bias_bwd(dattc, tw[d + ".s"], P[p + ".ca.in.b"][2 * D:], G[p + ".ca.in.b"][2 * D:], tw["d_ds"], H)
                     d_ds = tw["d_ds"]
```

Result: faster. 14030 pairs/s, median of 6 (+1.7%).
